# isabella232/handel

Hardware: AMD Instinct MI355X
Metric: BN254 aggregate-sig verifications/sec (batch 4096) (higher is better)
Workload: dtype u32 (26-bit-limb Fp, 64-bit accumulators)

## Files before the change

### handel_amd/_lib.py

```python

from __future__ import annotations

import ctypes
import os
import threading

from . import build as _build

_lock = threading.Lock()
_lib = None

HG_OK = 0
HG_ERR_SIG_INVALID = 1
HG_ERR_HASH_EOF = 2
HG_ERR_LEVEL = 3
HG_ERR_PK_UNMARSHAL = 4
HG_ERR_SIG_UNMARSHAL = 5
HG_ERR_EMPTY_AGG = 6
HG_ERR_CF_EXCEEDS = 7
HG_ERR_CF_MALFORMED = 8
HG_ERR_CF_SHORT = 9
HG_ERR_SIG_CF_EXCEEDS = 10
HG_ERR_SIG_CF_MALFORMED = 11
HG_ERR_SIG_CF_SHORT = 12
HG_ERR_MULTI_SIZES = 13
HG_ERR_PKT_ORIGIN = 20
HG_ERR_PKT_LEVEL = 21
HG_ERR_PKT_EOF = 22
HG_ERR_PKT_UNEXPECTED_EOF = 23
HG_ERR_PKT_BITSET_SHORT = 24
HG_ERR_PKT_TYPE_MISMATCH = 25
HG_ERR_PKT_BITSET_SIZE = 26
HG_ERR_PKT_NO_SIG = 27
HG_ERR_PKT_ID_RANGE = 28
HG_PKT_NO_IND = 29
HG_PKT_HAS_IND = 1
HG_STORE_HAS_BEST = 1
HG_STORE_BEST_SIG = 2
HG_STORE_SIG_BEST = 0xFFFFFFFF
HG_STORE_LEVEL_FULL = 0xFFFFFFFF
HG_MERGE_SKIPPED = 0
HG_MERGE_STORED = 1
HG_MERGE_DISCARDED = 2
HG_MERGE_ERR_MISSING = 3
HG_MERGE_ERR_INDIVIDUAL = 4
HG_MERGE_ERR_ROW = 5
HG_COMBINED_EMPTY = 1
HG_COMBINED_ERR_MISSING = 2
HG_ERR_ARG = 100
HG_ERR_DEVICE = 101

HG_FLAVOR_GO = 0
HG_FLAVOR_CF = 1

HG_PHASE_VERIFY = 0
HG_PHASE_AGGREGATE = 1
HG_PHASE_SUBMIT = 2

_P = ctypes.c_void_p
_SZ = ctypes.c_size_t
_I = ctypes.c_int
SIGNATURES = {
    "hg_version": (_I, []),
    "hg_context_simds": (_I, [_P]),
    "hg_context_flavor": (_I, [_P]),
    "hg_create": (_I, [_I, _I, ctypes.POINTER(_P)]),
    "hg_destroy": (None, [_P]),
    "hg_last_error": (ctypes.c_char_p, [_P]),
    "hg_code_string": (ctypes.c_char_p, [_I, _I]),
    "hg_processing_error_string": (ctypes.c_char_p, [_I, _I]),
    "hg_registry_load": (_I, [_P, _P, _SZ, _P]),
    "hg_registry_size": (_SZ, [_P]),
    "hg_prepare_aggregate": (_I, [_P]),
    "hg_aggregate_tables": (_I, [_P]),
    "hg_prepare_aggregate_msg": (_I, [_P, _P, _SZ]),
    "hg_set_aggregate_level": (_I, [_P, _I]),
    "hg_set_table_budget": (_I, [_P, _SZ]),
    "hg_set_fold_overlap": (_I, [_P, _I]),
    "hg_set_verify_split": (_I, [_P, _I]),
    "hg_registry_non_g2": (_SZ, [_P]),
    "hg_set_message": (_I, [_P, _P, _SZ]),
    "hg_verify_batch": (_I, [_P, _P, _P, _SZ, _P]),
    "hg_verify_batch_msg": (_I, [_P, _P, _SZ, _P, _P, _SZ, _P]),
    "hg_verify_batch_device": (_I, [_P, _P, _P, _SZ, _P, _P]),
    "hg_pack_verdicts_device": (_I, [_P, _P, _SZ, _P, _P]),
    "hg_verify_aggregate": (_I, [_P, _P, _SZ, _P, _SZ, _P, _P, _P]),
    "hg_verify_aggregate_device": (_I, [_P, _P, _SZ, _P, _P, _P, _P, _P]),
    "hg_verify_aggregate_device_bits": (_I, [_P, _P, _SZ, _P, _P, _P, _P, _P]),
    "hg_verify_aggregate_msg": (_I, [_P, _P, _SZ, _P, _SZ, _P, _SZ, _P, _P, _P]),
    "hg_verify_multisig": (_I, [_P, _P, _P, _SZ, _P, _SZ, _P, _P]),
    "hg_aggregate_pk": (_I, [_P, _P, _SZ, _P, _SZ, _P, _P]),
    "hg_combine_g1": (_I, [_P, _P, _P, _SZ, _P, _P]),
    "hg_combine_g2": (_I, [_P, _P, _P, _SZ, _P, _P]),
    "hg_pair": (_I, [_P, _P, _P, _SZ, _P, _P]),
    "hg_keygen": (_I, [_P, _P, _SZ, _P]),
    "hg_sign": (_I, [_P, _P, _SZ, _P]),
    "hg_sign_msg": (_I, [_P, _P, _SZ, _P, _SZ, _P]),
    "hg_debug_fp_mul": (_I, [_P, _P, _P, _SZ, _P]),
    "hg_diag_read": (_I, [_P, _P, _SZ]),
    "hg_sig_pairing_device": (_I, [_P, _P, _SZ, _P, _I, _P]),
    "hg_debug_fp12": (_I, [_P, _I, _P, _P, _SZ, _P]),
    "hg_timing_enable": (_I, [_P, _I]),
    "hg_timing_read": (_I, [_P, ctypes.POINTER(ctypes.c_double), ctypes.POINTER(_I)]),
    "hg_timing_read_phase": (_I, [_P, _I, ctypes.POINTER(ctypes.c_double), ctypes.POINTER(_I)]),
    "hg_sync": (_I, [_P]),
    "hg_context_bytes": (_SZ, [_P]),
    "hg_packet_stride_words": (_SZ, [_P]),
    "hg_parse_packets": (_I, [_P, _P, _SZ, _P, _SZ, _SZ, _P, _P, _P, _P]),
    "hg_parse_packets_device": (_I, [_P, _P, _SZ, _P, _SZ, _SZ, _P, _P, _P, _P, _P]),
    "hg_packet_error": (_I, [_P, _I, _P, ctypes.c_char_p, _SZ]),
    "hg_stores_create": (_I, [_P, _P, _SZ, _SZ, ctypes.POINTER(_P)]),
    "hg_stores_destroy": (None, [_P]),
    "hg_stores_update": (_I, [_P, _P, _SZ, _P, _SZ]),
    "hg_stores_read": (_I, [_P, ctypes.c_uint32, ctypes.c_uint32, _P, _P, ctypes.POINTER(_I)]),
    "hg_stores_evaluate_device": (_I, [_P, _P, _SZ, _SZ, _P, _P, _P, _P, _P]),
    "hg_stores_evaluate": (_I, [_P, _P, _SZ, _SZ, _P, _P, _P, _P]),
    "hg_stores_select_capacity": (_SZ, [_P, _SZ, ctypes.c_uint32]),
    "hg_stores_select_device": (_I, [_P, _P, _SZ, _P, ctypes.c_uint32, _P, _P, _P, _P, _P, _P, _P]),
    "hg_stores_enable_merge": (_I, [_P]),
    "hg_stores_update_sigs": (_I, [_P, _P, _SZ, _P, _SZ]),
    "hg_stores_read_best": (_I, [_P, ctypes.c_uint32, ctypes.c_uint32, _P, _P, ctypes.POINTER(_I)]),
    "hg_stores_merge_device": (_I, [_P, _P, _SZ, _P, _P, _SZ, _P, _SZ, _P, _P, _P, _P, _P, _P]),
    "hg_stores_combined_device": (_I, [_P, _P, _SZ, _SZ, _P, _P, _P, _P, _P]),
    "hg_stores_combined": (_I, [_P, _P, _SZ, _SZ, _P, _P, _P, _P]),
    "hg_batcher_create": (_I, [_P, _SZ, ctypes.c_uint, ctypes.POINTER(_P)]),
    "hg_batcher_destroy": (None, [_P]),
    "hg_batcher_submit": (_I, [_P, _P, _SZ, _P, _P, _P, ctypes.POINTER(_P)]),
    "hg_batcher_wait": (_I, [_P, _P, _P]),
    "hg_batcher_verify_aggregate": (_I, [_P, _P, _SZ, _P, _P, _P, _P]),
    "hg_batcher_stats": (_I, [_P, _P, _P]),
    "hg_prepare_aggregate_level": (_I, [_P, _I]),
    "hg_lane_create": (_I, [_P, _SZ, _SZ, _I, ctypes.POINTER(_P)]),
    "hg_lane_destroy": (None, [_P]),
    "hg_lane_stage": (_I, [_P, _SZ, _SZ, ctypes.POINTER(_P), ctypes.POINTER(_P), ctypes.POINTER(_P)]),
    "hg_lane_submit": (_I, [_P]),
    "hg_lane_query": (_I, [_P]),
    "hg_lane_wait": (_I, [_P]),
    "hg_lane_codes": (ctypes.POINTER(ctypes.c_int32), [_P]),
    "hg_lane_submit_device": (_I, [_P, _P, _SZ, _P, _P, _P, _P, _P]),
    "hg_lane_set_pairing_padding": (_I, [_P, _I]),
    "hg_lane_set_latency_form": (_I, [_P, _I]),
    "hg_lane_stream": (_P, [_P]),
    "hg_service_config_init": (None, [_P]),
    "hg_service_create": (_I, [_P, ctypes.c_char_p, _P, ctypes.POINTER(_P)]),
    "hg_service_create_echo": (_I, [ctypes.c_char_p, _P, ctypes.c_uint32, ctypes.c_uint32, ctypes.POINTER(_P)]),
    "hg_service_destroy": (None, [_P]),
    "hg_service_stats": (_I, [_P, _P, _P, _P]),
}


class HandelGPUError(RuntimeError):
    pass


def load(build_if_missing: bool = True):
    global _lib
    with _lock:
# ... 18 lines not shown
```

### handel_amd/csrc/bn256_gt.h

```cpp
#pragma once
#include "bn256_kernels.h"
#include "bn256_sigform.h"

namespace hg {

struct Gt {
  uint32_t w[120];
};
static constexpr int kGtChunk = 8;
static constexpr int kGtChunkTeams = 5;

struct GtReq {
  int m;
  int chunks;
  int comp;
  int k;
  int term_off;
  int chunk_off;
};
struct alignas(8) GtHdr {
  int terms, chunks;
  int big, mid;
  int nlong, nshort;
};
struct GtBlockIndex {
  int base[24];
};
struct GtWork {
  GtReq* plan;
  GtHdr* hdr;
  uint32_t* terms;
  int2* ord;
  int cap;
  Gt* partial;
  int* multi;
  int chunk_grid;
  int chunk;
  int win_bits;
};

void launch_gt_keys(const PointG2* reg, int n, const LineCoef* tab, const PointG1* h, Gt* out, hipStream_t s);
void launch_gt_windows8(const Gt* key, int nreg, Gt* w8, int nwin8, hipStream_t s);
void launch_gt_windows16(const Gt* w8, int nwin8, Gt* w16, int nwin16, hipStream_t s);
void launch_gt_blocks(const Gt* src, int stride, int nsrc, Gt* dst, int ndst, hipStream_t s);
void launch_gt_fold(const AggRequest* reqs, int n, const uint64_t* words, int32_t* codes, int nreg, int levels,
                    const Gt* win, const Gt* blk, const GtBlockIndex& bi, GtWork w, Gt* y, bool zero_hdr,
                    hipStream_t s);
void launch_verify_sig(const PointG1* sigs, int n, const LineCoef* tab, const Gt* y, int32_t* codes, hipStream_t s);
const SigEnv& sig_env();
bool launch_sig_form(SigForm f, const uint8_t* sigs, int flavor, int n, const LineCoef* tab, uint8_t* ws, Gt* fe,
                     hipStream_t s);
size_t fe12_ws_bytes(int n);
bool launch_fe12(Gt* fe, int n, uint8_t* ws, hipStream_t s);
void launch_gt_compare(const Gt* fe, const Gt* y, int n, int32_t* codes, hipStream_t s);
void launch_gt_compare_bits(const Gt* fe, const Gt* y, int n, int32_t* codes, uint8_t* bits, hipStream_t s);

}
```

### handel_amd/csrc/bn256_gt.hip

```cpp
#include <hip/hip_runtime.h>

#include <cstdlib>

#include "bn256_agg.h"
#include "bn256_decode.h"
#include "bn256_gt.h"
#include "bn256_pairing.h"
#include "bn256_sigfe.h"
#include "bn256_sigteam.h"

namespace hg {
static inline int nblk(int n, int b) { return (n + b - 1) / b; }

static constexpr int kFoldWords = kFoldTeamElems * 10;
static_assert(kFoldWords % 2 == 0, "8-byte aligned team regions");

HG_DEV void fold_regs_init(const Team& T) {
  if (T.tl == 0) {
    Fp z, o;
    fp_zero(z);
    fp_one(o);
    st_fp_a8(T.base + (kFoldRegBase + 0) * 10, z.l);
    st_fp_a8(T.base + (kFoldRegBase + 1) * 10, o.l);
  }
// ... 380 lines not shown
    gt_put(T, S_B, v, false);
    c += 4;
    if (c < g.chunks) gt_read(nx, partial + g.chunk_off + c, T);
    fold_mul(T, S);
  }
  for (int d = 1; d < (g.chunks > 2 ? 4 : 2); d <<= 1) {
    team_sync();
    lds_fp12_copy(T, slot(T, S_B), lds + (team ^ d) * kFoldWords + S_A * kFp12Words);
    fold_mul(T, S);
  }
  team_sync();
  if (team == 0) gt_store(T, S_A, y + r);
}

template <int TEAMS, bool kStore, bool kPad = (TEAMS == 4)>
__global__ __launch_bounds__(64) void k_verify_sig(const PointG1* sigs, const uint8_t* sig_bytes, int flavor, int n,
                                                   const LineCoef* tab, const Gt* y, Gt* fe, int32_t* codes) {
  __shared__ __attribute__((aligned(16))) uint32_t lds[TEAMS * kSigTeamWords];
  if (kStore) __builtin_amdgcn_s_setprio(3);
  if constexpr (kPad) asm volatile("" ::: "v255", "a0");
  Team T = make_team(lds, kSigTeamWords);
  uint32_t* F = T.base + kSigRegBase * 10;
  const int idx = blockIdx.x * TEAMS + (threadIdx.x >> 4);
  const bool valid = idx < n;
  const int ci = valid ? idx : n - 1;
  PointG1 sg;
  if (kStore) (void)decode_g1_one(sig_bytes + (size_t)ci * 64, flavor, sg);
  else sg = sigs[ci];
  XStream S = x_stream();
  team_miller_sig(T, F, sg.x, sg.y, sg.inf == 0, tab, S, SigFE<SigProgs16>::final_exp_hint_s());
  SigFE<SigProgs16>::team_final_exp_fc_s(T, S);
  if (kStore) {
    team_sync();
    if (valid) gt_store(T, S_F, fe + idx);
    return;
  }
  gt_load(T, S_A, y + ci);
  team_sync();
  const bool ok = t12_equal(T, S_F, S_A);
  if (valid && T.tl == 0 && codes[idx] == HG_OK) codes[idx] = ok ? HG_OK : HG_ERR_SIG_INVALID;
}

__global__ __launch_bounds__(64) void k_gt_compare(const Gt* fe, const Gt* y, int n, int32_t* codes) {
  const int r = blockIdx.x;
  if (r >= n) return;
  const int l = threadIdx.x;
  bool eq = true;
  if (l < 60) {
    const uint2 a = reinterpret_cast<const uint2*>(fe[r].w)[l];
    const uint2 b = reinterpret_cast<const uint2*>(y[r].w)[l];
    eq = a.x == b.x && a.y == b.y;
  }
  const bool all = __ballot(!eq) == 0;
  if (l == 0 && codes[r] == HG_OK) codes[r] = all ? HG_OK : HG_ERR_SIG_INVALID;
}

__global__ __launch_bounds__(64) void k_gt_compare_bits(const Gt* fe, const Gt* y, int n, int32_t* codes,
                                                        uint8_t* bits) {
  const int b = blockIdx.x;
  const int l = threadIdx.x;
  uint2 a[8], v[8];
#pragma unroll
  for (int j = 0; j < 8; j++) {
    const int r = min(8 * b + j, n - 1);
    a[j] = l < 60 ? reinterpret_cast<const uint2*>(fe[r].w)[l] : make_uint2(0, 0);
    v[j] = l < 60 ? reinterpret_cast<const uint2*>(y[r].w)[l] : make_uint2(0, 0);
  }
  bool mine = false;
#pragma unroll
  for (int j = 0; j < 8; j++) {
    const bool all = __ballot(a[j].x != v[j].x || a[j].y != v[j].y) == 0;
    const int r = 8 * b + j;
    if (l == j && r < n) {
      int32_t c = codes[r];
      if (c == HG_OK) c = all ? HG_OK : HG_ERR_SIG_INVALID;
      codes[r] = c;
      mine = c == HG_OK;
    }
  }
  const uint64_t m = __ballot(mine);
  if (l == 0) bits[b] = (uint8_t)(m & 0xffu);
}

void launch_gt_keys(const PointG2* reg, int n, const LineCoef* tab, const PointG1* h, Gt* out, hipStream_t s) {
  if (n > 0) k_gt_keys<4><<<nblk(n, 4), 64, 0, s>>>(reg, n, tab, h, out);
}
void launch_gt_windows8(const Gt* key, int nreg, Gt* w8, int nwin8, hipStream_t s) {
  if (nwin8 <= 0) return;
  k_gt_nib<<<nblk(2 * nwin8, 4), 64, 0, s>>>(key, nreg, nwin8, w8);
  k_gt_cross<<<nblk(15 * nwin8, 4), 64, 0, s>>>(nwin8, w8);
}
void launch_gt_windows16(const Gt* w8, int nwin8, Gt* w16, int nwin16, hipStream_t s) {
  if (nwin16 <= 0) return;
  k_gt_win16<<<nblk(256 * nwin16, kTeams12), 64, 0, s>>>(w8, nwin8, nwin16, w16);
}
void launch_gt_blocks(const Gt* src, int stride, int nsrc, Gt* dst, int ndst, hipStream_t s) {
  if (ndst > 0) k_gt_blocks<<<nblk(ndst, 4), 64, 0, s>>>(src, stride, nsrc, dst, ndst);
}
void launch_gt_fold(const AggRequest* reqs, int n, const uint64_t* words, int32_t* codes, int nreg, int levels,
                    const Gt* win, const Gt* blk, const GtBlockIndex& bi, GtWork w, Gt* y, bool zero_hdr, hipStream_t s) {
  if (n <= 0) return;
  if (zero_hdr) (void)hipMemsetAsync(w.hdr, 0, sizeof(GtHdr), s);
  if (w.win_bits == 16)
    k_gt_plan<16><<<nblk(n, kPlanWaves), 64 * kPlanWaves, 0, s>>>(reqs, n, words, codes, nreg, levels, bi, w.plan,
                                                                  w.hdr, w.terms, w.ord, w.cap, w.chunk, w.multi);
  else
    k_gt_plan<8><<<nblk(n, kPlanWaves), 64 * kPlanWaves, 0, s>>>(reqs, n, words, codes, nreg, levels, bi, w.plan,
                                                                 w.hdr, w.terms, w.ord, w.cap, w.chunk, w.multi);
  k_gt_chunks<<<w.chunk_grid, 64, 0, s>>>(win, blk, w.terms, w.ord, w.cap, w.plan, w.hdr, w.chunk, w.partial, y);
  k_gt_combine<<<n, 64, 0, s>>>(n, w.hdr, w.multi, w.plan, w.partial, y);
}
void launch_verify_sig(const PointG1* sigs, int n, const LineCoef* tab, const Gt* y, int32_t* codes, hipStream_t s) {
  if (n > 0) k_verify_sig<4, false><<<nblk(n, 4), 64, 0, s>>>(sigs, nullptr, 0, n, tab, y, nullptr, codes);
}
const SigEnv& sig_env() {
  static const SigEnv env = [] {
    auto on = [](const char* name, bool def) {
      const char* e = getenv(name);
      return e ? atoi(e) != 0 : def;
    };
    SigEnv v;
    if (getenv("HG_SIG12")) v.sig12 = on("HG_SIG12", false) ? 1 : 0;
    v.sig12_split = on("HG_SIG12_SPLIT", true);
    v.w2 = on("HG_SIG_W2", true);
    if (const char* e = getenv("HG_SIG_W2_LANE_MAX")) v.w2_lane_max = atoi(e);
    if (const char* e = getenv("HG_VERIFY_SPLIT")) v.verify_split = atoi(e) == 1;
    return v;
  }();
  return env;
}
bool launch_sig12(bool pad, bool split, const uint8_t* sigs, int flavor, int n, const LineCoef* tab, uint8_t* ws,
                  Gt* fe, hipStream_t s);
void launch_sig_w2(const uint8_t* sigs, int flavor, int n, const LineCoef* tab, Gt* fe, hipStream_t s);
bool launch_sig_form(SigForm f, const uint8_t* sigs, int flavor, int n, const LineCoef* tab, uint8_t* ws, Gt* fe,
                     hipStream_t s) {
  switch (f) {
    case SigForm::W16Pad:
      if (n > 0) k_verify_sig<4, true><<<nblk(n, 4), 64, 0, s>>>(nullptr, sigs, flavor, n, tab, nullptr, fe, nullptr);
      return true;
    case SigForm::W16:
      if (n > 0)
        k_verify_sig<4, true, false><<<nblk(n, 4), 64, 0, s>>>(nullptr, sigs, flavor, n, tab, nullptr, fe, nullptr);
      return true;
    case SigForm::T12Pad:
    case SigForm::T12:
      return launch_sig12(f == SigForm::T12Pad, sig_form_split(sig_env(), f), sigs, flavor, n, tab, ws, fe, s);
    case SigForm::W2:
      launch_sig_w2(sigs, flavor, n, tab, fe, s);
      return true;
  }
  return false;
}
void launch_gt_compare(const Gt* fe, const Gt* y, int n, int32_t* codes, hipStream_t s) {
  if (n > 0) k_gt_compare<<<n, 64, 0, s>>>(fe, y, n, codes);
}
void launch_gt_compare_bits(const Gt* fe, const Gt* y, int n, int32_t* codes, uint8_t* bits, hipStream_t s) {
  if (n > 0) k_gt_compare_bits<<<(n + 7) / 8, 64, 0, s>>>(fe, y, n, codes, bits);
}

}
```

### handel_amd/csrc/bn256_xtab.h

```cpp
#pragma once
#include <stdint.h>
namespace hg {
#define HG_P2N 0x0422599cu, 0x04ac6c5du, 0x05678616u, 0x05120b5au, 0x07b96e22u, 0x0584dc20u, 0x07fb2e17u, 0x047f9aa5u, 0x078d2a8du, 0x008fb500u
enum XProg { XP_PDBL, XP_PADD_POS, XP_PADD_NEG, XP_PADD_F1, XP_PADD_F2, XP_MDBL_1, XP_MDBL_2, XP_PDBL_1, XP_PADD_POS_1, XP_MADD_POS_2, XP_PADD_POS_3, XP_PADD_NEG_1, XP_MADD_NEG_2, XP_PADD_NEG_3, XP_PADD_F1_1, XP_MADD_F1_2, XP_PADD_F1_3, XP_PADD_F2_1, XP_MADD_F2_2, XP_PADD_F2_3, XP_SQR12, XP_LINE_PK, XP_LINE_FIX, XP_CYC_SQR, XP_MUL12, XP_CYC_SQR_X, XP_FEVAL, XP_SDBL, XP_LFEV, XP_MUL12F, XP_SQR12_12, XP_LINE_FIX_12, XP_MUL12_12, XP_CYC_SQR_X_12, XP_LINE_FIX_S, XP_MUL12_S, XP_CYC_SQR_X_S, XP_FEVAL_S, XP_SDBL_S, XP_LFEV_S, XP_SQR12_12_T, XP_LINE_FIX_12_T, XP_MUL12_12_T, XP_CYC_SQR_X_12_T, XP_MDBL_1_V, XP_MDBL_2_V, XP_PDBL_1_V, XP_PADD_POS_1_V, XP_MADD_POS_2_V, XP_PADD_POS_3_V, XP_PADD_NEG_1_V, XP_MADD_NEG_2_V, XP_PADD_NEG_3_V, XP_PADD_F1_1_V, XP_MADD_F1_2_V, XP_PADD_F1_3_V, XP_PADD_F2_1_V, XP_MADD_F2_2_V, XP_PADD_F2_3_V, XP_LINE_PK_V };
__constant__ static const uint32_t kXTab[28288] = {
  0x240616d0u, 0x19509000u, 0x90002906u, 0x28ee1bd0u, 0x16d09000u, 0x16f805c8u, 0x172006b8u, 0x16801748u, 0x24fe1680u, 0x00000f00u, 0x2a1216f8u, 0x19789000u,
  0x900028fau, 0x29fa1bf8u, 0x16d09000u, 0x177006b8u, 0x16800690u, 0x16801680u, 0x2a021680u, 0x00000ff0u, 0x2a031720u, 0x19a02b03u, 0x25032403u, 0x9000ffffu,
  0x17989000u, 0x17c00618u, 0x17e80708u, 0x16801810u, 0x28fe1680u, 0x00000fa0u, 0x2aff1748u, 0x19c82b01u, 0x250124ffu, 0x9000ffffu, 0x17989000u, 0x18380708u,
  0x168006e0u, 0x16801680u, 0x2e021680u, 0x00001090u, 0x25061770u, 0x19f09000u, 0x2b092a09u, 0x9000ffffu, 0x18609000u, 0x18880668u, 0x18b00758u, 0x168018d8u,
  0x2cfe1680u, 0x00001040u, 0x26061798u, 0x1a189000u, 0x90002afau, 0x9000ffffu, 0x19009000u, 0x19280758u, 0x19500730u, 0x19780758u, 0x26020730u, 0x00000f50u,
  0x2c1217c0u, 0x1a409000u, 0x900024fau, 0x9000ffffu, 0x19a09000u, 0x19f019c8u, 0x1a181748u, 0x168006b8u, 0x25fe1680u, 0x00000f28u, 0x2c0317e8u, 0x1a682d03u,
  0x27032603u, 0x9000ffffu, 0x17709000u, 0x1a4006b8u, 0x16800690u, 0x16801680u, 0x2b021680u, 0x00001018u, 0x2cff1810u, 0x1a902d01u, 0x270126ffu, 0x9000ffffu,
  0x1a689000u, 0x1ab81a90u, 0x1ae01810u, 0x16800708u, 0x29fe1680u, 0x00000fc8u, 0x27061838u, 0x1ab89000u, 0x2d092c09u, 0x9000ffffu, 0x18389000u, 0x1b080708u,
  0x168006e0u, 0x16801680u, 0x2f021680u, 0x000010b8u, 0x28061860u, 0x1ae09000u, 0x90002cfau, 0x9000ffffu, 0x1b309000u, 0x1b801b58u, 0x1ba818d8u, 0x16800758u,
  0x2dfe1680u, 0x00001068u, 0x2e121888u, 0x1b089000u, 0x900026fau, 0x9000ffffu, 0x19289000u, 0x1bd00758u, 0x19780730u, 0x1bf80758u, 0x27020730u, 0x00000f78u,
  0x2e0318b0u, 0x1b302f03u, 0x29032803u, 0x9000ffffu, 0x16809000u, 0x16801680u, 0x16801680u, 0x16801680u, 0x90001680u, 0x0000ffffu, 0x2eff18d8u, 0x1b582f01u,
  0x290128ffu, 0x9000ffffu, 0x16809000u, 0x16801680u, 0x16801680u, 0x16801680u, 0x90001680u, 0x0000ffffu, 0x28121900u, 0x1b809000u, 0x2f092e09u, 0x9000ffffu,
  0x16809000u, 0x16801680u, 0x16801680u, 0x16801680u, 0x90001680u, 0x0000ffffu, 0x29121928u, 0x1ba89000u, 0x90002efau, 0x9000ffffu, 0x16809000u, 0x16801680u,
  0x16801680u, 0x16801680u, 0x90001680u, 0x0000ffffu, 0x0c0616d0u, 0x19509000u, 0x0f010effu, 0x020816d0u, 0x02f816f8u, 0x17481720u, 0x01e00cfeu, 0x121216f8u,
  0x19789000u, 0x900014fau, 0x17981770u, 0x02f817c0u, 0x174817e8u, 0x02080dfeu, 0x12031720u, 0x19a01303u, 0x15091409u, 0x03981810u, 0x03701838u, 0x16801680u,
  0x02300e02u, 0x12ff1748u, 0x19c81301u, 0x90000d06u, 0x03981838u, 0x18601810u, 0x16801680u, 0x02580f02u, 0x0c031770u, 0x19f00d03u, 0x90000cfau, 0x02581888u,
  0x034818b0u, 0x190018d8u, 0x028010feu, 0x0cff1798u, 0x1a180d01u, 0x90001006u, 0x19501928u, 0x03481978u, 0x190019a0u, 0x02a811feu, 0x12fa17c0u, 0x1a409000u,
  0x90001612u, 0x02f816d0u, 0x02d019c8u, 0x16801680u, 0x02d01202u, 0x120917e8u, 0x1a681309u, 0x17031603u, 0x02f819c8u, 0x02d019f0u, 0x16801680u, 0x02f81302u,
  0x10121810u, 0x1a901106u, 0x170116ffu, 0x02a81a18u, 0x03981a40u, 0x1a901a68u, 0x032014feu, 0x10fa1838u, 0x1ab81112u, 0x11031003u, 0x1ae01ab8u, 0x03981b08u,
  0x1a901b30u, 0x034815feu, 0x16ff1860u, 0x1ae09000u, 0x110110ffu, 0x03481888u, 0x03201b58u, 0x16801680u, 0x03701602u, 0x0e061888u, 0x1b089000u, 0x900016fau,
  0x03481b58u, 0x03201b80u, 0x16801680u, 0x03981702u, 0x141218b0u, 0x1b309000u, 0x17091609u, 0x16801680u, 0x16801680u, 0x16801680u, 0xffff9000u, 0x140318d8u,
  0x1b581503u, 0x90000f06u, 0x16801680u, 0x16801680u, 0x16801680u, 0xffff9000u, 0x14ff1900u, 0x1b801501u, 0x90000efau, 0x16801680u, 0x16801680u, 0x16801680u,
  0xffff9000u, 0x0e031928u, 0xffff0f03u, 0x90009000u, 0x16801680u, 0x16801680u, 0x16801680u, 0xffff9000u, 0x0c0616d0u, 0x19509000u, 0x0f010effu, 0x020816d0u,
  0x02f816f8u, 0x17481720u, 0x03c00cfeu, 0x121216f8u, 0x19789000u, 0x900014fau, 0x17981770u, 0x02f817c0u, 0x174817e8u, 0x03e80dfeu, 0x12031720u, 0x19a01303u,
  0x15091409u, 0x03981810u, 0x03701838u, 0x16801680u, 0x04100e02u, 0x12ff1748u, 0x19c81301u, 0x90000d06u, 0x03981838u, 0x18601810u, 0x16801680u, 0x04380f02u,
  0x0c031770u, 0x19f00d03u, 0x90000cfau, 0x02581888u, 0x034818b0u, 0x190018d8u, 0x046010feu, 0x0cff1798u, 0x1a180d01u, 0x90001006u, 0x19501928u, 0x03481978u,
  0x190019a0u, 0x048811feu, 0x12fa17c0u, 0x1a409000u, 0x90001612u, 0x02f816d0u, 0x02d019c8u, 0x16801680u, 0x04b01202u, 0x120917e8u, 0x1a681309u, 0x17031603u,
  0x02f819c8u, 0x02d019f0u, 0x16801680u, 0x04d81302u, 0x10121810u, 0x1a901106u, 0x170116ffu, 0x02a81a18u, 0x03981a40u, 0x1a901a68u, 0x050014feu, 0x10fa1838u,
  0x1ab81112u, 0x11031003u, 0x1ae01ab8u, 0x03981b08u, 0x1a901b30u, 0x052815feu, 0x16ff1860u, 0x1ae09000u, 0x110110ffu, 0x03481888u, 0x03201b58u, 0x16801680u,
  0x05501602u, 0x0e061888u, 0x1b089000u, 0x900016fau, 0x03481b58u, 0x03201b80u, 0x16801680u, 0x05781702u, 0x141218b0u, 0x1b309000u, 0x17091609u, 0x16801680u,
  0x16801680u, 0x16801680u, 0xffff9000u, 0x140318d8u, 0x1b581503u, 0x90000f06u, 0x16801680u, 0x16801680u, 0x16801680u, 0xffff9000u, 0x14ff1900u, 0x1b801501u,
  0x90000efau, 0x16801680u, 0x16801680u, 0x16801680u, 0xffff9000u, 0x0e031928u, 0xffff0f03u, 0x90009000u, 0x16801680u, 0x16801680u, 0x16801680u, 0xffff9000u,
  0x0c0616d0u, 0x19509000u, 0x0f010effu, 0x020816d0u, 0x02f816f8u, 0x17481720u, 0x00000cfeu, 0x121216f8u, 0x19789000u, 0x900014fau, 0x17981770u, 0x02f817c0u,
  0x174817e8u, 0x00280dfeu, 0x12031720u, 0x19a01303u, 0x15091409u, 0x03981810u, 0x03701838u, 0x16801680u, 0x00500e02u, 0x12ff1748u, 0x19c81301u, 0x90000d06u,
  0x03981838u, 0x18601810u, 0x16801680u, 0x00780f02u, 0x0c031770u, 0x19f00d03u, 0x90000cfau, 0x02581888u, 0x034818b0u, 0x190018d8u, 0x00a010feu, 0x0cff1798u,
  0x1a180d01u, 0x90001006u, 0x19501928u, 0x03481978u, 0x190019a0u, 0x00c811feu, 0x12fa17c0u, 0x1a409000u, 0x90001612u, 0x02f816d0u, 0x02d019c8u, 0x16801680u,
  0x00f01202u, 0x120917e8u, 0x1a681309u, 0x17031603u, 0x02f819c8u, 0x02d019f0u, 0x16801680u, 0x01181302u, 0x10121810u, 0x1a901106u, 0x170116ffu, 0x02a81a18u,
  0x03981a40u, 0x1a901a68u, 0x014014feu, 0x10fa1838u, 0x1ab81112u, 0x11031003u, 0x1ae01ab8u, 0x03981b08u, 0x1a901b30u, 0x016815feu, 0x16ff1860u, 0x1ae09000u,
  0x110110ffu, 0x03481888u, 0x03201b58u, 0x16801680u, 0x01901602u, 0x0e061888u, 0x1b089000u, 0x900016fau, 0x03481b58u, 0x03201b80u, 0x16801680u, 0x01b81702u,
  0x141218b0u, 0x1b309000u, 0x17091609u, 0x16801680u, 0x16801680u, 0x16801680u, 0xffff9000u, 0x140318d8u, 0x1b581503u, 0x90000f06u, 0x16801680u, 0x16801680u,
  0x16801680u, 0xffff9000u, 0x14ff1900u, 0x1b801501u, 0x90000efau, 0x16801680u, 0x16801680u, 0x16801680u, 0xffff9000u, 0x0e031928u, 0xffff0f03u, 0x90009000u,
  0x16801680u, 0x16801680u, 0x16801680u, 0xffff9000u, 0x000616d0u, 0x19509000u, 0x030102ffu, 0x002816d0u, 0x011816f8u, 0x17481720u, 0x000000feu, 0x061216f8u,
  0x19789000u, 0x900008fau, 0x17981770u, 0x011817c0u, 0x174817e8u, 0x002801feu, 0x06031720u, 0x19a00703u, 0x09090809u, 0x01b81810u, 0x01901838u, 0x16801680u,
  0x00500202u, 0x06ff1748u, 0x19c80701u, 0x90000106u, 0x01b81838u, 0x18601810u, 0x16801680u, 0x00780302u, 0x00031770u, 0x19f00103u, 0x900000fau, 0x00781888u,
  0x016818b0u, 0x190018d8u, 0x00a004feu, 0x00ff1798u, 0x1a180101u, 0x90000406u, 0x19501928u, 0x01681978u, 0x190019a0u, 0x00c805feu, 0x06fa17c0u, 0x1a409000u,
  0x90000a12u, 0x011816d0u, 0x00f019c8u, 0x16801680u, 0x00f00602u, 0x060917e8u, 0x1a680709u, 0x0b030a03u, 0x011819c8u, 0x00f019f0u, 0x16801680u, 0x01180702u,
  0x04121810u, 0x1a900506u, 0x0b010affu, 0x00c81a18u, 0x01b81a40u, 0x1a901a68u, 0x014008feu, 0x04fa1838u, 0x1ab80512u, 0x05030403u, 0x1ae01ab8u, 0x01b81b08u,
  0x1a901b30u, 0x016809feu, 0x0aff1860u, 0x1ae09000u, 0x050104ffu, 0x01681888u, 0x01401b58u, 0x16801680u, 0x01900a02u, 0x02061888u, 0x1b089000u, 0x90000afau,
  0x01681b58u, 0x01401b80u, 0x16801680u, 0x01b80b02u, 0x081218b0u, 0x1b309000u, 0x0b090a09u, 0x16801680u, 0x16801680u, 0x16801680u, 0xffff9000u, 0x080318d8u,
  0x1b580903u, 0x90000306u, 0x16801680u, 0x16801680u, 0x16801680u, 0xffff9000u, 0x08ff1900u, 0x1b800901u, 0x900002fau, 0x16801680u, 0x16801680u, 0x16801680u,
  0xffff9000u, 0x02031928u, 0xffff0303u, 0x90009000u, 0x16801680u, 0x16801680u, 0x16801680u, 0xffff9000u, 0x6c0616d0u, 0x19509000u, 0x6f016effu, 0x110816d0u,
  0x11f816f8u, 0x17481720u, 0x00006cfeu, 0x721216f8u, 0x19789000u, 0x900074fau, 0x17981770u, 0x11f817c0u, 0x174817e8u, 0x00286dfeu, 0x72031720u, 0x19a07303u,
  0x75097409u, 0x12981810u, 0x12701838u, 0x16801680u, 0x00506e02u, 0x72ff1748u, 0x19c87301u, 0x90006d06u, 0x12981838u, 0x18601810u, 0x16801680u, 0x00786f02u,
  0x6c031770u, 0x19f06d03u, 0x90006cfau, 0x11581888u, 0x124818b0u, 0x190018d8u, 0x00a070feu, 0x6cff1798u, 0x1a186d01u, 0x90007006u, 0x19501928u, 0x12481978u,
  0x190019a0u, 0x00c871feu, 0x72fa17c0u, 0x1a409000u, 0x90007612u, 0x11f816d0u, 0x11d019c8u, 0x16801680u, 0x00f07202u, 0x720917e8u, 0x1a687309u, 0x77037603u,
  0x11f819c8u, 0x11d019f0u, 0x16801680u, 0x01187302u, 0x70121810u, 0x1a907106u, 0x770176ffu, 0x11a81a18u, 0x12981a40u, 0x1a901a68u, 0x014074feu, 0x70fa1838u,
  0x1ab87112u, 0x71037003u, 0x1ae01ab8u, 0x12981b08u, 0x1a901b30u, 0x016875feu, 0x76ff1860u, 0x1ae09000u, 0x710170ffu, 0x12481888u, 0x12201b58u, 0x16801680u,
  0x01907602u, 0x6e061888u, 0x1b089000u, 0x900076fau, 0x12481b58u, 0x12201b80u, 0x16801680u, 0x01b87702u, 0x741218b0u, 0x1b309000u, 0x77097609u, 0x16801680u,
  0x16801680u, 0x16801680u, 0xffff9000u, 0x740318d8u, 0x1b587503u, 0x90006f06u, 0x16801680u, 0x16801680u, 0x16801680u, 0xffff9000u, 0x74ff1900u, 0x1b807501u,
  0x90006efau, 0x16801680u, 0x16801680u, 0x16801680u, 0xffff9000u, 0x6e031928u, 0xffff6f03u, 0x90009000u, 0x16801680u, 0x16801680u, 0x16801680u, 0xffff9000u,
  0x600616d0u, 0x19509000u, 0x630162ffu, 0x0f2816d0u, 0x101816f8u, 0x17481720u, 0x0f0060feu, 0x661216f8u, 0x19789000u, 0x900068fau, 0x17981770u, 0x101817c0u,
  0x174817e8u, 0x0f2861feu, 0x66031720u, 0x19a06703u, 0x69096809u, 0x10b81810u, 0x10901838u, 0x16801680u, 0x0f506202u, 0x66ff1748u, 0x19c86701u, 0x90006106u,
  0x10b81838u, 0x18601810u, 0x16801680u, 0x0f786302u, 0x60031770u, 0x19f06103u, 0x900060fau, 0x0f781888u, 0x106818b0u, 0x190018d8u, 0x0fa064feu, 0x60ff1798u,
  0x1a186101u, 0x90006406u, 0x19501928u, 0x10681978u, 0x190019a0u, 0x0fc865feu, 0x66fa17c0u, 0x1a409000u, 0x90006a12u, 0x101816d0u, 0x0ff019c8u, 0x16801680u,
  0x0ff06602u, 0x660917e8u, 0x1a686709u, 0x6b036a03u, 0x101819c8u, 0x0ff019f0u, 0x16801680u, 0x10186702u, 0x64121810u, 0x1a906506u, 0x6b016affu, 0x0fc81a18u,
  0x10b81a40u, 0x1a901a68u, 0x104068feu, 0x64fa1838u, 0x1ab86512u, 0x65036403u, 0x1ae01ab8u, 0x10b81b08u, 0x1a901b30u, 0x106869feu, 0x6aff1860u, 0x1ae09000u,
  0x650164ffu, 0x10681888u, 0x10401b58u, 0x16801680u, 0x10906a02u, 0x62061888u, 0x1b089000u, 0x90006afau, 0x10681b58u, 0x10401b80u, 0x16801680u, 0x10b86b02u,
  0x681218b0u, 0x1b309000u, 0x6b096a09u, 0x16801680u, 0x16801680u, 0x16801680u, 0xffff9000u, 0x680318d8u, 0x1b586903u, 0x90006306u, 0x16801680u, 0x16801680u,
  0x16801680u, 0xffff9000u, 0x68ff1900u, 0x1b806901u, 0x900062fau, 0x16801680u, 0x16801680u, 0x16801680u, 0xffff9000u, 0x62031928u, 0xffff6303u, 0x90009000u,
  0x16801680u, 0x16801680u, 0x16801680u, 0xffff9000u, 0x6c0616d0u, 0x19509000u, 0x6f016effu, 0x110816d0u, 0x11f816f8u, 0x17481720u, 0x0f006cfeu, 0x721216f8u,
  0x19789000u, 0x900074fau, 0x17981770u, 0x11f817c0u, 0x174817e8u, 0x0f286dfeu, 0x72031720u, 0x19a07303u, 0x75097409u, 0x12981810u, 0x12701838u, 0x16801680u,
  0x0f506e02u, 0x72ff1748u, 0x19c87301u, 0x90006d06u, 0x12981838u, 0x18601810u, 0x16801680u, 0x0f786f02u, 0x6c031770u, 0x19f06d03u, 0x90006cfau, 0x11581888u,
  0x124818b0u, 0x190018d8u, 0x0fa070feu, 0x6cff1798u, 0x1a186d01u, 0x90007006u, 0x19501928u, 0x12481978u, 0x190019a0u, 0x0fc871feu, 0x72fa17c0u, 0x1a409000u,
  0x90007612u, 0x11f816d0u, 0x11d019c8u, 0x16801680u, 0x0ff07202u, 0x720917e8u, 0x1a687309u, 0x77037603u, 0x11f819c8u, 0x11d019f0u, 0x16801680u, 0x10187302u,
  0x70121810u, 0x1a907106u, 0x770176ffu, 0x11a81a18u, 0x12981a40u, 0x1a901a68u, 0x104074feu, 0x70fa1838u, 0x1ab87112u, 0x71037003u, 0x1ae01ab8u, 0x12981b08u,
  0x1a901b30u, 0x106875feu, 0x76ff1860u, 0x1ae09000u, 0x710170ffu, 0x12481888u, 0x12201b58u, 0x16801680u, 0x10907602u, 0x6e061888u, 0x1b089000u, 0x900076fau,
  0x12481b58u, 0x12201b80u, 0x16801680u, 0x10b87702u, 0x741218b0u, 0x1b309000u, 0x77097609u, 0x16801680u, 0x16801680u, 0x16801680u, 0xffff9000u, 0x740318d8u,
  0x1b587503u, 0x90006f06u, 0x16801680u, 0x16801680u, 0x16801680u, 0xffff9000u, 0x74ff1900u, 0x1b807501u, 0x90006efau, 0x16801680u, 0x16801680u, 0x16801680u,
  0xffff9000u, 0x6e031928u, 0xffff6f03u, 0x90009000u, 0x16801680u, 0x16801680u, 0x16801680u, 0xffff9000u, 0x000616d0u, 0x19509000u, 0x030102ffu, 0x002816d0u,
  0x011816f8u, 0x17481720u, 0x10e000feu, 0x061216f8u, 0x19789000u, 0x900008fau, 0x17981770u, 0x011817c0u, 0x174817e8u, 0x110801feu, 0x06031720u, 0x19a00703u,
  0x09090809u, 0x01b81810u, 0x01901838u, 0x16801680u, 0x11300202u, 0x06ff1748u, 0x19c80701u, 0x90000106u, 0x01b81838u, 0x18601810u, 0x16801680u, 0x11580302u,
  0x00031770u, 0x19f00103u, 0x900000fau, 0x00781888u, 0x016818b0u, 0x190018d8u, 0x118004feu, 0x00ff1798u, 0x1a180101u, 0x90000406u, 0x19501928u, 0x01681978u,
  0x190019a0u, 0x11a805feu, 0x06fa17c0u, 0x1a409000u, 0x90000a12u, 0x011816d0u, 0x00f019c8u, 0x16801680u, 0x11d00602u, 0x060917e8u, 0x1a680709u, 0x0b030a03u,
// ... 2190 lines not shown
  0x11d01298u, 0x09b009b0u, 0x09b009b0u, 0x09b009b0u, 0x09b009b0u, 0x00000b40u, 0x720102a8u, 0x05287301u, 0x3e0071ffu, 0x11f81298u, 0x11d00488u, 0x09b009b0u,
  0x09b009b0u, 0x09b009b0u, 0x09b009b0u, 0x00000b68u, 0x72ff02d0u, 0xffff7301u, 0x3e003e00u, 0x0a281180u, 0x09b009b0u, 0x09b009b0u, 0x09b009b0u, 0x09b009b0u,
  0x09b009b0u, 0x00000f50u, 0x76fd02f8u, 0xffff77ffu, 0x3e003e00u, 0x0a2811a8u, 0x09b009b0u, 0x09b009b0u, 0x09b009b0u, 0x09b009b0u, 0x09b009b0u, 0x00000f78u,
  0x78020320u, 0xffff3e00u, 0x3e003e00u, 0x0a0004b0u, 0x09b009b0u, 0x09b009b0u, 0x09b009b0u, 0x09b009b0u, 0x09b009b0u, 0x00000f00u, 0x73ff0348u, 0xffff7903u,
  0x3e003e00u, 0x0a0004d8u, 0x09b009b0u, 0x09b009b0u, 0x09b009b0u, 0x09b009b0u, 0x09b009b0u, 0x00000f28u, 0x72ff0370u, 0xffff7803u, 0x3e003e00u, 0x0ca81130u,
  0x0c801158u, 0x0cf80500u, 0x0cd00528u, 0x09b009b0u, 0x09b009b0u, 0x00000eb0u, 0x7cfd0398u, 0xffff7dffu, 0x3e003e00u, 0x0ca81158u, 0x0c8004b0u, 0x0cf80528u,
  0x0cd01180u, 0x09b009b0u, 0x09b009b0u, 0x00000ed8u, 0x7c0103c0u, 0xffff7dfdu, 0x3e003e00u, 0x09b009b0u, 0x09b009b0u, 0x09b009b0u, 0x09b009b0u, 0x09b009b0u,
  0x09b009b0u, 0x0000ffffu, 0x7eff03e8u, 0xffff3e00u, 0x3e003e00u, 0x09b009b0u, 0x09b009b0u, 0x09b009b0u, 0x09b009b0u, 0x09b009b0u, 0x09b009b0u, 0x0000ffffu,
  0x7fff0410u, 0xffff3e00u, 0x3e003e00u, 0x09b009b0u, 0x09b009b0u, 0x09b009b0u, 0x09b009b0u, 0x09b009b0u, 0x09b009b0u, 0x0000ffffu, 0x7aff0438u, 0xffff3e00u,
  0x3e003e00u, 0x09b009b0u, 0x09b009b0u, 0x09b009b0u, 0x09b009b0u, 0x09b009b0u, 0x09b009b0u, 0x0000ffffu, 0x4cff01e0u, 0x01e03e00u, 0x02300208u, 0x46010258u,
  0x00001130u, 0x48ff0208u, 0x02304903u, 0x0be00208u, 0x47010258u, 0x00001158u, 0x4dff0230u, 0x02803e00u, 0x02a80208u, 0x44010258u, 0x00001180u, 0x48030258u,
  0x02a84901u, 0x0d200208u, 0x45010258u, 0x000011a8u, 0x54ff0280u, 0x0d703e00u, 0x09b00a50u, 0x3e0009b0u, 0x00000e10u, 0x55ff02a8u, 0x0d983e00u, 0x09b00a50u,
  0x3e0009b0u, 0x00000e38u, 0x3e00ffffu, 0x0dc03e00u, 0x09b00a78u, 0x3e0009b0u, 0x00000e60u, 0x3e00ffffu, 0x0de83e00u, 0x09b00a78u, 0x3e0009b0u, 0x00000e88u,
  0x3e00ffffu, 0x09b03e00u, 0x09b009b0u, 0x3e0009b0u, 0x0000ffffu, 0x3e00ffffu, 0x09b03e00u, 0x09b009b0u, 0x3e0009b0u, 0x0000ffffu, 0x3e00ffffu, 0x09b03e00u,
  0x09b009b0u, 0x3e0009b0u, 0x0000ffffu, 0x3e00ffffu, 0x09b03e00u, 0x09b009b0u, 0x3e0009b0u, 0x0000ffffu, 0x3e00ffffu, 0x09b03e00u, 0x09b009b0u, 0x3e0009b0u,
  0x0000ffffu, 0x3e00ffffu, 0x09b03e00u, 0x09b009b0u, 0x3e0009b0u, 0x0000ffffu, 0x3e00ffffu, 0x09b03e00u, 0x09b009b0u, 0x3e0009b0u, 0x0000ffffu, 0x3e00ffffu,
  0x09b03e00u, 0x09b009b0u, 0x3e0009b0u, 0x0000ffffu, 0x720201e0u, 0x04603e00u, 0x7d017c03u, 0x11f801e0u, 0x12480208u, 0x12200230u, 0x11f80258u, 0x11d00280u,
  0x09b009b0u, 0x00000aa0u, 0x76030208u, 0x04887701u, 0x3e0076ffu, 0x02d002a8u, 0x12480230u, 0x122002f8u, 0x11f80280u, 0x11d00320u, 0x09b009b0u, 0x00000ac8u,
  0x76ff0230u, 0x04b07703u, 0x3e006effu, 0x03481310u, 0x03701338u, 0x12480398u, 0x122003c0u, 0x11f803e8u, 0x11d00410u, 0x00000af0u, 0x78fe0258u, 0x04d83e00u,
  0x3e006fffu, 0x03481338u, 0x03700438u, 0x124803c0u, 0x12200460u, 0x11f80410u, 0x11d013b0u, 0x00000b18u, 0x79fe0280u, 0x05003e00u, 0x3e0070ffu, 0x11f81270u,
  0x11d01298u, 0x09b009b0u, 0x09b009b0u, 0x09b009b0u, 0x09b009b0u, 0x00000b40u, 0x720102a8u, 0x05287301u, 0x3e0071ffu, 0x11f81298u, 0x11d00488u, 0x09b009b0u,
  0x09b009b0u, 0x09b009b0u, 0x09b009b0u, 0x00000b68u, 0x72ff02d0u, 0xffff7301u, 0x3e003e00u, 0x0a281180u, 0x09b009b0u, 0x09b009b0u, 0x09b009b0u, 0x09b009b0u,
  0x09b009b0u, 0x00000f50u, 0x76fd02f8u, 0xffff77ffu, 0x3e003e00u, 0x0a2811a8u, 0x09b009b0u, 0x09b009b0u, 0x09b009b0u, 0x09b009b0u, 0x09b009b0u, 0x00000f78u,
  0x78020320u, 0xffff3e00u, 0x3e003e00u, 0x0a0004b0u, 0x09b009b0u, 0x09b009b0u, 0x09b009b0u, 0x09b009b0u, 0x09b009b0u, 0x00000f00u, 0x73ff0348u, 0xffff7903u,
  0x3e003e00u, 0x0a0004d8u, 0x09b009b0u, 0x09b009b0u, 0x09b009b0u, 0x09b009b0u, 0x09b009b0u, 0x00000f28u, 0x72ff0370u, 0xffff7803u, 0x3e003e00u, 0x0d481130u,
  0x0d201158u, 0x0c080500u, 0x0be00528u, 0x09b009b0u, 0x09b009b0u, 0x00000eb0u, 0x7cfd0398u, 0xffff7dffu, 0x3e003e00u, 0x0d481158u, 0x0d2004b0u, 0x0c080528u,
  0x0be01180u, 0x09b009b0u, 0x09b009b0u, 0x00000ed8u, 0x7c0103c0u, 0xffff7dfdu, 0x3e003e00u, 0x09b009b0u, 0x09b009b0u, 0x09b009b0u, 0x09b009b0u, 0x09b009b0u,
  0x09b009b0u, 0x0000ffffu, 0x7eff03e8u, 0xffff3e00u, 0x3e003e00u, 0x09b009b0u, 0x09b009b0u, 0x09b009b0u, 0x09b009b0u, 0x09b009b0u, 0x09b009b0u, 0x0000ffffu,
  0x7fff0410u, 0xffff3e00u, 0x3e003e00u, 0x09b009b0u, 0x09b009b0u, 0x09b009b0u, 0x09b009b0u, 0x09b009b0u, 0x09b009b0u, 0x0000ffffu, 0x7aff0438u, 0xffff3e00u,
  0x3e003e00u, 0x09b009b0u, 0x09b009b0u, 0x09b009b0u, 0x09b009b0u, 0x09b009b0u, 0x09b009b0u, 0x0000ffffu, 0x5aff01e0u, 0x00005b03u, 0x00280e88u, 0x01900e60u,
  0x01b801e0u, 0x06030208u, 0x00000701u, 0x11a802a8u, 0x09b009b0u, 0x000011d0u, 0x5a030208u, 0x00285b01u, 0x00000e88u, 0x01b80230u, 0x019001e0u, 0x07030258u,
  0x002806ffu, 0x02f802d0u, 0x09b009b0u, 0x000011f8u, 0x5cff0230u, 0x00503e00u, 0x00780e88u, 0x00000e60u, 0x00280e38u, 0x08030e10u, 0x00500901u, 0x11580320u,
  0x09b009b0u, 0x00001220u, 0x5afd0258u, 0x00785bffu, 0x00500e88u, 0x00280230u, 0x00000e38u, 0x09030280u, 0x007808ffu, 0x03700348u, 0x09b009b0u, 0x00001248u,
  0x5aff0280u, 0x00a03e00u, 0x00c80e88u, 0x00500e60u, 0x00780e38u, 0x0a030e10u, 0x00a00b01u, 0x11a80b40u, 0x11800b68u, 0x00001270u, 0x700202a8u, 0x00c83e00u,
  0x00a00e88u, 0x00780230u, 0x00500e38u, 0x0b030280u, 0x00c80affu, 0x11a80b68u, 0x11800398u, 0x00001298u, 0x700102d0u, 0x00f07101u, 0x01180e88u, 0x00a00e60u,
  0x00c80e38u, 0x00010e10u, 0x00f03e00u, 0x11a80aa0u, 0x11800ac8u, 0x000012c0u, 0x70ff02f8u, 0x01187101u, 0x00f00e88u, 0x00c80230u, 0x00a00e38u, 0x01010280u,
  0x01183e00u, 0x11a80ac8u, 0x118003c0u, 0x000012e8u, 0x6e020320u, 0x01403e00u, 0x01680e88u, 0x00f00e60u, 0x01180e38u, 0x02010e10u, 0x01403e00u, 0x11a81130u,
  0x11801158u, 0x00001310u, 0x6e010348u, 0x01686f01u, 0x01400e88u, 0x01180230u, 0x00f00e38u, 0x03010280u, 0x01683e00u, 0x11a81158u, 0x118003e8u, 0x00001338u,
  0x6eff0370u, 0x01906f01u, 0x01b80e88u, 0x01400e60u, 0x01680e38u, 0x04010e10u, 0x01903e00u, 0x11580b40u, 0x11300b68u, 0x00001360u, 0x48ff0398u, 0x01b83e00u,
  0x01900e88u, 0x01680230u, 0x01400e38u, 0x05010280u, 0x01b83e00u, 0x11580b68u, 0x11300398u, 0x00001388u, 0x44ff03c0u, 0x09b03e00u, 0x09b009b0u, 0x09b009b0u,
  0x09b009b0u, 0x3e0009b0u, 0xffff3e00u, 0x11a80af0u, 0x11800b18u, 0x000013b0u, 0x6eff03e8u, 0x09b03e00u, 0x09b009b0u, 0x09b009b0u, 0x09b009b0u, 0x3e0009b0u,
  0xffff3e00u, 0x11a80b18u, 0x11800410u, 0x000013d8u, 0x46ff0410u, 0x09b03e00u, 0x09b009b0u, 0x09b009b0u, 0x09b009b0u, 0x3e0009b0u, 0xffff3e00u, 0x09b009b0u,
  0x09b009b0u, 0x0000ffffu, 0x3e00ffffu, 0x09b03e00u, 0x09b009b0u, 0x09b009b0u, 0x09b009b0u, 0x3e0009b0u, 0xffff3e00u, 0x09b009b0u, 0x09b009b0u, 0x0000ffffu,
  0x5aff01e0u, 0x00005b03u, 0x00280e88u, 0x01900e60u, 0x01b801e0u, 0x06030208u, 0x00000701u, 0x11a802a8u, 0x09b009b0u, 0x000011d0u, 0x5a030208u, 0x00285b01u,
  0x00000e88u, 0x01b80230u, 0x019001e0u, 0x07030258u, 0x002806ffu, 0x02f802d0u, 0x09b009b0u, 0x000011f8u, 0x5cff0230u, 0x00503e00u, 0x00780e88u, 0x00000e60u,
  0x00280e38u, 0x08030e10u, 0x00500901u, 0x11580320u, 0x09b009b0u, 0x00001220u, 0x5afd0258u, 0x00785bffu, 0x00500e88u, 0x00280230u, 0x00000e38u, 0x09030280u,
  0x007808ffu, 0x03700348u, 0x09b009b0u, 0x00001248u, 0x5aff0280u, 0x00a03e00u, 0x00c80e88u, 0x00500e60u, 0x00780e38u, 0x0a030e10u, 0x00a00b01u, 0x11a80b40u,
  0x11800b68u, 0x00001270u, 0x700202a8u, 0x00c83e00u, 0x00a00e88u, 0x00780230u, 0x00500e38u, 0x0b030280u, 0x00c80affu, 0x11a80b68u, 0x11800398u, 0x00001298u,
  0x700102d0u, 0x00f07101u, 0x01180e88u, 0x00a00e60u, 0x00c80e38u, 0x00010e10u, 0x00f03e00u, 0x11a80aa0u, 0x11800ac8u, 0x000012c0u, 0x70ff02f8u, 0x01187101u,
  0x00f00e88u, 0x00c80230u, 0x00a00e38u, 0x01010280u, 0x01183e00u, 0x11a80ac8u, 0x118003c0u, 0x000012e8u, 0x6e020320u, 0x01403e00u, 0x01680e88u, 0x00f00e60u,
  0x01180e38u, 0x02010e10u, 0x01403e00u, 0x11a81130u, 0x11801158u, 0x00001310u, 0x6e010348u, 0x01686f01u, 0x01400e88u, 0x01180230u, 0x00f00e38u, 0x03010280u,
  0x01683e00u, 0x11a81158u, 0x118003e8u, 0x00001338u, 0x6eff0370u, 0x01906f01u, 0x01b80e88u, 0x01400e60u, 0x01680e38u, 0x04010e10u, 0x01903e00u, 0x11580b40u,
  0x11300b68u, 0x00001360u, 0x48ff0398u, 0x01b83e00u, 0x01900e88u, 0x01680230u, 0x01400e38u, 0x05010280u, 0x01b83e00u, 0x11580b68u, 0x11300398u, 0x00001388u,
  0x44ff03c0u, 0x09b03e00u, 0x09b009b0u, 0x09b009b0u, 0x09b009b0u, 0x3e0009b0u, 0xffff3e00u, 0x11a80af0u, 0x11800b18u, 0x000013b0u, 0x6eff03e8u, 0x09b03e00u,
  0x09b009b0u, 0x09b009b0u, 0x09b009b0u, 0x3e0009b0u, 0xffff3e00u, 0x11a80b18u, 0x11800410u, 0x000013d8u, 0x46ff0410u, 0x09b03e00u, 0x09b009b0u, 0x09b009b0u,
  0x09b009b0u, 0x3e0009b0u, 0xffff3e00u, 0x09b009b0u, 0x09b009b0u, 0x0000ffffu, 0x3e00ffffu, 0x09b03e00u, 0x09b009b0u, 0x09b009b0u, 0x09b009b0u, 0x3e0009b0u,
  0xffff3e00u, 0x09b009b0u, 0x09b009b0u, 0x0000ffffu, 0x5aff01e0u, 0x00005b03u, 0x00280e88u, 0x01900e60u, 0x01b801e0u, 0x06030208u, 0x00000701u, 0x11a802a8u,
  0x09b009b0u, 0x000011d0u, 0x5a030208u, 0x00285b01u, 0x00000e88u, 0x01b80230u, 0x019001e0u, 0x07030258u, 0x002806ffu, 0x02f802d0u, 0x09b009b0u, 0x000011f8u,
  0x5cff0230u, 0x00503e00u, 0x00780e88u, 0x00000e60u, 0x00280e38u, 0x08030e10u, 0x00500901u, 0x11580320u, 0x09b009b0u, 0x00001220u, 0x5afd0258u, 0x00785bffu,
  0x00500e88u, 0x00280230u, 0x00000e38u, 0x09030280u, 0x007808ffu, 0x03700348u, 0x09b009b0u, 0x00001248u, 0x5aff0280u, 0x00a03e00u, 0x00c80e88u, 0x00500e60u,
  0x00780e38u, 0x0a030e10u, 0x00a00b01u, 0x11a80b40u, 0x11800b68u, 0x00001270u, 0x700202a8u, 0x00c83e00u, 0x00a00e88u, 0x00780230u, 0x00500e38u, 0x0b030280u,
  0x00c80affu, 0x11a80b68u, 0x11800398u, 0x00001298u, 0x700102d0u, 0x00f07101u, 0x01180e88u, 0x00a00e60u, 0x00c80e38u, 0x00010e10u, 0x00f03e00u, 0x11a80aa0u,
  0x11800ac8u, 0x000012c0u, 0x70ff02f8u, 0x01187101u, 0x00f00e88u, 0x00c80230u, 0x00a00e38u, 0x01010280u, 0x01183e00u, 0x11a80ac8u, 0x118003c0u, 0x000012e8u,
  0x6e020320u, 0x01403e00u, 0x01680e88u, 0x00f00e60u, 0x01180e38u, 0x02010e10u, 0x01403e00u, 0x11a81130u, 0x11801158u, 0x00001310u, 0x6e010348u, 0x01686f01u,
  0x01400e88u, 0x01180230u, 0x00f00e38u, 0x03010280u, 0x01683e00u, 0x11a81158u, 0x118003e8u, 0x00001338u, 0x6eff0370u, 0x01906f01u, 0x01b80e88u, 0x01400e60u,
  0x01680e38u, 0x04010e10u, 0x01903e00u, 0x11580b40u, 0x11300b68u, 0x00001360u, 0x48ff0398u, 0x01b83e00u, 0x01900e88u, 0x01680230u, 0x01400e38u, 0x05010280u,
  0x01b83e00u, 0x11580b68u, 0x11300398u, 0x00001388u, 0x44ff03c0u, 0x09b03e00u, 0x09b009b0u, 0x09b009b0u, 0x09b009b0u, 0x3e0009b0u, 0xffff3e00u, 0x11a80af0u,
  0x11800b18u, 0x000013b0u, 0x6eff03e8u, 0x09b03e00u, 0x09b009b0u, 0x09b009b0u, 0x09b009b0u, 0x3e0009b0u, 0xffff3e00u, 0x11a80b18u, 0x11800410u, 0x000013d8u,
  0x46ff0410u, 0x09b03e00u, 0x09b009b0u, 0x09b009b0u, 0x09b009b0u, 0x3e0009b0u, 0xffff3e00u, 0x09b009b0u, 0x09b009b0u, 0x0000ffffu, 0x3e00ffffu, 0x09b03e00u,
  0x09b009b0u, 0x09b009b0u, 0x09b009b0u, 0x3e0009b0u, 0xffff3e00u, 0x09b009b0u, 0x09b009b0u, 0x0000ffffu, 0x5aff01e0u, 0x00005b03u, 0x00280e88u, 0x01900e60u,
  0x01b801e0u, 0x06030208u, 0x00000701u, 0x11a802a8u, 0x09b009b0u, 0x000011d0u, 0x5a030208u, 0x00285b01u, 0x00000e88u, 0x01b80230u, 0x019001e0u, 0x07030258u,
  0x002806ffu, 0x02f802d0u, 0x09b009b0u, 0x000011f8u, 0x5cff0230u, 0x00503e00u, 0x00780e88u, 0x00000e60u, 0x00280e38u, 0x08030e10u, 0x00500901u, 0x11580320u,
  0x09b009b0u, 0x00001220u, 0x5afd0258u, 0x00785bffu, 0x00500e88u, 0x00280230u, 0x00000e38u, 0x09030280u, 0x007808ffu, 0x03700348u, 0x09b009b0u, 0x00001248u,
  0x5aff0280u, 0x00a03e00u, 0x00c80e88u, 0x00500e60u, 0x00780e38u, 0x0a030e10u, 0x00a00b01u, 0x11a80b40u, 0x11800b68u, 0x00001270u, 0x700202a8u, 0x00c83e00u,
  0x00a00e88u, 0x00780230u, 0x00500e38u, 0x0b030280u, 0x00c80affu, 0x11a80b68u, 0x11800398u, 0x00001298u, 0x700102d0u, 0x00f07101u, 0x01180e88u, 0x00a00e60u,
  0x00c80e38u, 0x00010e10u, 0x00f03e00u, 0x11a80aa0u, 0x11800ac8u, 0x000012c0u, 0x70ff02f8u, 0x01187101u, 0x00f00e88u, 0x00c80230u, 0x00a00e38u, 0x01010280u,
  0x01183e00u, 0x11a80ac8u, 0x118003c0u, 0x000012e8u, 0x6e020320u, 0x01403e00u, 0x01680e88u, 0x00f00e60u, 0x01180e38u, 0x02010e10u, 0x01403e00u, 0x11a81130u,
  0x11801158u, 0x00001310u, 0x6e010348u, 0x01686f01u, 0x01400e88u, 0x01180230u, 0x00f00e38u, 0x03010280u, 0x01683e00u, 0x11a81158u, 0x118003e8u, 0x00001338u,
  0x6eff0370u, 0x01906f01u, 0x01b80e88u, 0x01400e60u, 0x01680e38u, 0x04010e10u, 0x01903e00u, 0x11580b40u, 0x11300b68u, 0x00001360u, 0x48ff0398u, 0x01b83e00u,
  0x01900e88u, 0x01680230u, 0x01400e38u, 0x05010280u, 0x01b83e00u, 0x11580b68u, 0x11300398u, 0x00001388u, 0x44ff03c0u, 0x09b03e00u, 0x09b009b0u, 0x09b009b0u,
  0x09b009b0u, 0x3e0009b0u, 0xffff3e00u, 0x11a80af0u, 0x11800b18u, 0x000013b0u, 0x6eff03e8u, 0x09b03e00u, 0x09b009b0u, 0x09b009b0u, 0x09b009b0u, 0x3e0009b0u,
  0xffff3e00u, 0x11a80b18u, 0x11800410u, 0x000013d8u, 0x46ff0410u, 0x09b03e00u, 0x09b009b0u, 0x09b009b0u, 0x09b009b0u, 0x3e0009b0u, 0xffff3e00u, 0x09b009b0u,
  0x09b009b0u, 0x0000ffffu, 0x3e00ffffu, 0x09b03e00u, 0x09b009b0u, 0x09b009b0u, 0x09b009b0u, 0x3e0009b0u, 0xffff3e00u, 0x09b009b0u, 0x09b009b0u, 0x0000ffffu,
  0x00000000u, 0x00000000u, 0x00000000u, 0x00000000u, 0x00000000u, 0x00000000u, 0x00000000u, 0x00000000u, 0x00000000u, 0x00000000u, 0x00000000u, 0x00000000u,
  0x00000000u, 0x00000000u, 0x00000000u, 0x00000000u,
};
static constexpr int kXFetchWords = 16;
static constexpr int kFoldRegBase = 36;
static constexpr int kFoldTeamElems = 60;
static constexpr int kSigRegBase = 84;
static constexpr int kSigTeamElems = 118;
static constexpr int kSigTRegBase = 60;
static constexpr int kSigTTeamElems = 92;
static constexpr int kVRegBase = 62;
static constexpr int kVTeamElems = 128;
template <int PROG, int D = -1, int A = -1, int B = -1> struct XInst;
template <> struct XInst<XP_CYC_SQR, S_I, S_C> { static constexpr int kOff = 0, kW = 10; HG_DEV static void run(const Team& T, XStream& S, XHint h) { x_round<3, 2, 4, 1, 10, 0, 0, -1, -1, -1, 1, 0, 0, 0, 1>(T, S, 0, h); } };
template <> struct XInst<XP_CYC_SQR_X, S_A, S_A> { static constexpr int kOff = 160, kW = 7; HG_DEV static void run(const Team& T, XStream& S, XHint h) { x_round<2, 2, 3, 1, 7, 0, 0, 6, 2, 0, 0, 0, 1, 0, 1>(T, S, 160, h); } };
template <> struct XInst<XP_CYC_SQR_X, S_B, S_A> { static constexpr int kOff = 272, kW = 7; HG_DEV static void run(const Team& T, XStream& S, XHint h) { x_round<2, 2, 3, 1, 7, 0, 0, 6, 2, 0, 0, 0, 1, 0, 1>(T, S, 272, h); } };
template <> struct XInst<XP_CYC_SQR_X, S_F, S_A> { static constexpr int kOff = 384, kW = 7; HG_DEV static void run(const Team& T, XStream& S, XHint h) { x_round<2, 2, 3, 1, 7, 0, 0, 6, 2, 0, 0, 0, 1, 0, 1>(T, S, 384, h); } };
template <> struct XInst<XP_CYC_SQR_X, S_F, S_F> { static constexpr int kOff = 496, kW = 7; HG_DEV static void run(const Team& T, XStream& S, XHint h) { x_round<2, 2, 3, 1, 7, 0, 0, 6, 2, 0, 0, 0, 1, 0, 1>(T, S, 496, h); } };
template <> struct XInst<XP_CYC_SQR_X, S_F, S_J> { static constexpr int kOff = 608, kW = 7; HG_DEV static void run(const Team& T, XStream& S, XHint h) { x_round<2, 2, 3, 1, 7, 0, 0, 6, 2, 0, 0, 0, 1, 0, 1>(T, S, 608, h); } };
template <> struct XInst<XP_CYC_SQR_X, S_I, S_I> { static constexpr int kOff = 720, kW = 7; HG_DEV static void run(const Team& T, XStream& S, XHint h) { x_round<2, 2, 3, 1, 7, 0, 0, 6, 2, 0, 0, 0, 1, 0, 1>(T, S, 720, h); } };
template <> struct XInst<XP_CYC_SQR_X, S_I, S_J> { static constexpr int kOff = 832, kW = 7; HG_DEV static void run(const Team& T, XStream& S, XHint h) { x_round<2, 2, 3, 1, 7, 0, 0, 6, 2, 0, 0, 0, 1, 0, 1>(T, S, 832, h); } };
template <> struct XInst<XP_CYC_SQR_X, S_J, S_F> { static constexpr int kOff = 944, kW = 7; HG_DEV static void run(const Team& T, XStream& S, XHint h) { x_round<2, 2, 3, 1, 7, 0, 0, 6, 2, 0, 0, 0, 1, 0, 1>(T, S, 944, h); } };
template <> struct XInst<XP_CYC_SQR_X, S_J, S_I> { static constexpr int kOff = 1056, kW = 7; HG_DEV static void run(const Team& T, XStream& S, XHint h) { x_round<2, 2, 3, 1, 7, 0, 0, 6, 2, 0, 0, 0, 1, 0, 1>(T, S, 1056, h); } };
template <> struct XInst<XP_CYC_SQR_X, S_J, S_J> { static constexpr int kOff = 1168, kW = 7; HG_DEV static void run(const Team& T, XStream& S, XHint h) { x_round<2, 2, 3, 1, 7, 0, 0, 6, 2, 0, 0, 0, 1, 0, 1>(T, S, 1168, h); } };
template <> struct XInst<XP_CYC_SQR_X, S_K, S_I> { static constexpr int kOff = 1280, kW = 7; HG_DEV static void run(const Team& T, XStream& S, XHint h) { x_round<2, 2, 3, 1, 7, 0, 0, 6, 2, 0, 0, 0, 1, 0, 1>(T, S, 1280, h); } };
template <> struct XInst<XP_CYC_SQR_X, S_K, S_K> { static constexpr int kOff = 1392, kW = 7; HG_DEV static void run(const Team& T, XStream& S, XHint h) { x_round<2, 2, 3, 1, 7, 0, 0, 6, 2, 0, 0, 0, 1, 0, 1>(T, S, 1392, h); } };
template <> struct XInst<XP_LINE_FIX, S_F, S_F> { static constexpr int kOff = 1504, kW = 7; HG_DEV static void run(const Team& T, XStream& S, XHint h) { x_round<1, 2, 4, 2, 7, 0, 0, 4, 1, 0, 1, 0, 0, 1, 1>(T, S, 1504, h); } };
template <> struct XInst<XP_LINE_PK, S_A, S_A> { static constexpr int kOff = 1616, kW = 8; HG_DEV static void run(const Team& T, XStream& S, XHint h) { x_round<1, 2, 6, 0, 8, 0, 0, 4, 0, 0, 1, 0, 0, 1, 0>(T, S, 1616, h); } };
template <> struct XInst<XP_LINE_PK, S_F, S_F> { static constexpr int kOff = 1744, kW = 8; HG_DEV static void run(const Team& T, XStream& S, XHint h) { x_round<1, 2, 6, 0, 8, 0, 0, 4, 0, 0, 1, 0, 0, 1, 0>(T, S, 1744, h); } };
template <> struct XInst<XP_MADD_F1_2, S_F, S_F> { static constexpr int kOff = 1872, kW = 10; HG_DEV static void run(const Team& T, XStream& S, XHint h) { x_round<1, 2, 4, 2, 10, 2, 0, 4, 1, 0, 1, 0, 0, 0, 0>(T, S, 1872, h); } };
template <> struct XInst<XP_MADD_F2_2, S_F, S_F> { static constexpr int kOff = 2032, kW = 10; HG_DEV static void run(const Team& T, XStream& S, XHint h) { x_round<1, 2, 4, 2, 10, 2, 0, 4, 1, 0, 1, 0, 0, 0, 0>(T, S, 2032, h); } };
template <> struct XInst<XP_MADD_NEG_2, S_F, S_F> { static constexpr int kOff = 2192, kW = 10; HG_DEV static void run(const Team& T, XStream& S, XHint h) { x_round<1, 2, 4, 2, 10, 2, 0, 4, 1, 0, 1, 0, 0, 0, 0>(T, S, 2192, h); } };
template <> struct XInst<XP_MADD_POS_2, S_F, S_F> { static constexpr int kOff = 2352, kW = 10; HG_DEV static void run(const Team& T, XStream& S, XHint h) { x_round<1, 2, 4, 2, 10, 2, 0, 4, 1, 0, 1, 0, 0, 0, 0>(T, S, 2352, h); } };
template <> struct XInst<XP_MDBL_1, S_F, S_F> { static constexpr int kOff = 2512, kW = 16; HG_DEV static void run(const Team& T, XStream& S, XHint h) { x_round<4, 2, 7, 0, 16, 2, 0, -1, -1, -1, 1, 0, 0, 0, 0>(T, S, 2512, h); } };
template <> struct XInst<XP_MDBL_2, S_F, S_F> { static constexpr int kOff = 2768, kW = 14; HG_DEV static void run(const Team& T, XStream& S, XHint h) { x_round<2, 4, 4, 2, 14, 2, 2, -1, -1, -1, 1, 0, 0, 0, 0>(T, S, 2768, h); } };
template <> struct XInst<XP_MUL12, S_A, S_A, S_B> { static constexpr int kOff = 2992, kW = 16; HG_DEV static void run(const Team& T, XStream& S, XHint h) { x_round<2, 2, 12, 0, 16, 0, 0, 4, 0, 0, 1, 0, 0, 1, 1>(T, S, 2992, h); } };
template <> struct XInst<XP_MUL12, S_A, S_C, S_E> { static constexpr int kOff = 3248, kW = 16; HG_DEV static void run(const Team& T, XStream& S, XHint h) { x_round<2, 2, 12, 0, 16, 0, 0, 4, 0, 0, 1, 0, 0, 1, 1>(T, S, 3248, h); } };
template <> struct XInst<XP_MUL12, S_A, S_F, S_A> { static constexpr int kOff = 3504, kW = 16; HG_DEV static void run(const Team& T, XStream& S, XHint h) { x_round<2, 2, 12, 0, 16, 0, 0, 4, 0, 0, 1, 0, 0, 1, 1>(T, S, 3504, h); } };
template <> struct XInst<XP_MUL12, S_A, S_G, S_A> { static constexpr int kOff = 3760, kW = 16; HG_DEV static void run(const Team& T, XStream& S, XHint h) { x_round<2, 2, 12, 0, 16, 0, 0, 4, 0, 0, 1, 0, 0, 1, 1>(T, S, 3760, h); } };
template <> struct XInst<XP_MUL12, S_A, S_K, S_L> { static constexpr int kOff = 4016, kW = 16; HG_DEV static void run(const Team& T, XStream& S, XHint h) { x_round<2, 2, 12, 0, 16, 0, 0, 4, 0, 0, 1, 0, 0, 1, 1>(T, S, 4016, h); } };
template <> struct XInst<XP_MUL12, S_B, S_A, S_B> { static constexpr int kOff = 4272, kW = 16; HG_DEV static void run(const Team& T, XStream& S, XHint h) { x_round<2, 2, 12, 0, 16, 0, 0, 4, 0, 0, 1, 0, 0, 1, 1>(T, S, 4272, h); } };
template <> struct XInst<XP_MUL12, S_B, S_C, S_D> { static constexpr int kOff = 4528, kW = 16; HG_DEV static void run(const Team& T, XStream& S, XHint h) { x_round<2, 2, 12, 0, 16, 0, 0, 4, 0, 0, 1, 0, 0, 1, 1>(T, S, 4528, h); } };
template <> struct XInst<XP_MUL12, S_D, S_A, S_E> { static constexpr int kOff = 4784, kW = 16; HG_DEV static void run(const Team& T, XStream& S, XHint h) { x_round<2, 2, 12, 0, 16, 0, 0, 4, 0, 0, 1, 0, 0, 1, 1>(T, S, 4784, h); } };
template <> struct XInst<XP_MUL12, S_E, S_B, S_J> { static constexpr int kOff = 5040, kW = 16; HG_DEV static void run(const Team& T, XStream& S, XHint h) { x_round<2, 2, 12, 0, 16, 0, 0, 4, 0, 0, 1, 0, 0, 1, 1>(T, S, 5040, h); } };
template <> struct XInst<XP_MUL12, S_F, S_A, S_B> { static constexpr int kOff = 5296, kW = 16; HG_DEV static void run(const Team& T, XStream& S, XHint h) { x_round<2, 2, 12, 0, 16, 0, 0, 4, 0, 0, 1, 0, 0, 1, 1>(T, S, 5296, h); } };
template <> struct XInst<XP_MUL12, S_F, S_B, S_A> { static constexpr int kOff = 5552, kW = 16; HG_DEV static void run(const Team& T, XStream& S, XHint h) { x_round<2, 2, 12, 0, 16, 0, 0, 4, 0, 0, 1, 0, 0, 1, 1>(T, S, 5552, h); } };
template <> struct XInst<XP_MUL12, S_F, S_F, S_A> { static constexpr int kOff = 5808, kW = 16; HG_DEV static void run(const Team& T, XStream& S, XHint h) { x_round<2, 2, 12, 0, 16, 0, 0, 4, 0, 0, 1, 0, 0, 1, 1>(T, S, 5808, h); } };
template <> struct XInst<XP_MUL12, S_F, S_F, S_J> { static constexpr int kOff = 6064, kW = 16; HG_DEV static void run(const Team& T, XStream& S, XHint h) { x_round<2, 2, 12, 0, 16, 0, 0, 4, 0, 0, 1, 0, 0, 1, 1>(T, S, 6064, h); } };
template <> struct XInst<XP_MUL12, S_F, S_F, S_K> { static constexpr int kOff = 6320, kW = 16; HG_DEV static void run(const Team& T, XStream& S, XHint h) { x_round<2, 2, 12, 0, 16, 0, 0, 4, 0, 0, 1, 0, 0, 1, 1>(T, S, 6320, h); } };
template <> struct XInst<XP_MUL12, S_F, S_G, S_A> { static constexpr int kOff = 6576, kW = 16; HG_DEV static void run(const Team& T, XStream& S, XHint h) { x_round<2, 2, 12, 0, 16, 0, 0, 4, 0, 0, 1, 0, 0, 1, 1>(T, S, 6576, h); } };
template <> struct XInst<XP_MUL12, S_F, S_K, S_J> { static constexpr int kOff = 6832, kW = 16; HG_DEV static void run(const Team& T, XStream& S, XHint h) { x_round<2, 2, 12, 0, 16, 0, 0, 4, 0, 0, 1, 0, 0, 1, 1>(T, S, 6832, h); } };
template <> struct XInst<XP_MUL12, S_F, S_K, S_L> { static constexpr int kOff = 7088, kW = 16; HG_DEV static void run(const Team& T, XStream& S, XHint h) { x_round<2, 2, 12, 0, 16, 0, 0, 4, 0, 0, 1, 0, 0, 1, 1>(T, S, 7088, h); } };
template <> struct XInst<XP_MUL12, S_G, S_G, S_D> { static constexpr int kOff = 7344, kW = 16; HG_DEV static void run(const Team& T, XStream& S, XHint h) { x_round<2, 2, 12, 0, 16, 0, 0, 4, 0, 0, 1, 0, 0, 1, 1>(T, S, 7344, h); } };
template <> struct XInst<XP_MUL12, S_H, S_C, S_H> { static constexpr int kOff = 7600, kW = 16; HG_DEV static void run(const Team& T, XStream& S, XHint h) { x_round<2, 2, 12, 0, 16, 0, 0, 4, 0, 0, 1, 0, 0, 1, 1>(T, S, 7600, h); } };
template <> struct XInst<XP_MUL12, S_I, S_E, S_I> { static constexpr int kOff = 7856, kW = 16; HG_DEV static void run(const Team& T, XStream& S, XHint h) { x_round<2, 2, 12, 0, 16, 0, 0, 4, 0, 0, 1, 0, 0, 1, 1>(T, S, 7856, h); } };
template <> struct XInst<XP_MUL12, S_I, S_I, S_J> { static constexpr int kOff = 8112, kW = 16; HG_DEV static void run(const Team& T, XStream& S, XHint h) { x_round<2, 2, 12, 0, 16, 0, 0, 4, 0, 0, 1, 0, 0, 1, 1>(T, S, 8112, h); } };
template <> struct XInst<XP_MUL12, S_I, S_I, S_K> { static constexpr int kOff = 8368, kW = 16; HG_DEV static void run(const Team& T, XStream& S, XHint h) { x_round<2, 2, 12, 0, 16, 0, 0, 4, 0, 0, 1, 0, 0, 1, 1>(T, S, 8368, h); } };
template <> struct XInst<XP_MUL12, S_J, S_G, S_D> { static constexpr int kOff = 8624, kW = 16; HG_DEV static void run(const Team& T, XStream& S, XHint h) { x_round<2, 2, 12, 0, 16, 0, 0, 4, 0, 0, 1, 0, 0, 1, 1>(T, S, 8624, h); } };
template <> struct XInst<XP_MUL12, S_J, S_J, S_A> { static constexpr int kOff = 8880, kW = 16; HG_DEV static void run(const Team& T, XStream& S, XHint h) { x_round<2, 2, 12, 0, 16, 0, 0, 4, 0, 0, 1, 0, 0, 1, 1>(T, S, 8880, h); } };
template <> struct XInst<XP_MUL12, S_J, S_J, S_F> { static constexpr int kOff = 9136, kW = 16; HG_DEV static void run(const Team& T, XStream& S, XHint h) { x_round<2, 2, 12, 0, 16, 0, 0, 4, 0, 0, 1, 0, 0, 1, 1>(T, S, 9136, h); } };
template <> struct XInst<XP_MUL12, S_J, S_J, S_I> { static constexpr int kOff = 9392, kW = 16; HG_DEV static void run(const Team& T, XStream& S, XHint h) { x_round<2, 2, 12, 0, 16, 0, 0, 4, 0, 0, 1, 0, 0, 1, 1>(T, S, 9392, h); } };
template <> struct XInst<XP_MUL12, S_J, S_J, S_K> { static constexpr int kOff = 9648, kW = 16; HG_DEV static void run(const Team& T, XStream& S, XHint h) { x_round<2, 2, 12, 0, 16, 0, 0, 4, 0, 0, 1, 0, 0, 1, 1>(T, S, 9648, h); } };
template <> struct XInst<XP_MUL12, S_K, S_J, S_L> { static constexpr int kOff = 9904, kW = 16; HG_DEV static void run(const Team& T, XStream& S, XHint h) { x_round<2, 2, 12, 0, 16, 0, 0, 4, 0, 0, 1, 0, 0, 1, 1>(T, S, 9904, h); } };
template <> struct XInst<XP_MUL12, S_K, S_K, S_C> { static constexpr int kOff = 10160, kW = 16; HG_DEV static void run(const Team& T, XStream& S, XHint h) { x_round<2, 2, 12, 0, 16, 0, 0, 4, 0, 0, 1, 0, 0, 1, 1>(T, S, 10160, h); } };
template <> struct XInst<XP_MUL12, S_K, S_K, S_D> { static constexpr int kOff = 10416, kW = 16; HG_DEV static void run(const Team& T, XStream& S, XHint h) { x_round<2, 2, 12, 0, 16, 0, 0, 4, 0, 0, 1, 0, 0, 1, 1>(T, S, 10416, h); } };
template <> struct XInst<XP_MUL12, S_K, S_K, S_H> { static constexpr int kOff = 10672, kW = 16; HG_DEV static void run(const Team& T, XStream& S, XHint h) { x_round<2, 2, 12, 0, 16, 0, 0, 4, 0, 0, 1, 0, 0, 1, 1>(T, S, 10672, h); } };
template <> struct XInst<XP_MUL12, S_L, S_A, S_K> { static constexpr int kOff = 10928, kW = 16; HG_DEV static void run(const Team& T, XStream& S, XHint h) { x_round<2, 2, 12, 0, 16, 0, 0, 4, 0, 0, 1, 0, 0, 1, 1>(T, S, 10928, h); } };
template <> struct XInst<XP_MUL12, S_L, S_F, S_K> { static constexpr int kOff = 11184, kW = 16; HG_DEV static void run(const Team& T, XStream& S, XHint h) { x_round<2, 2, 12, 0, 16, 0, 0, 4, 0, 0, 1, 0, 0, 1, 1>(T, S, 11184, h); } };
template <> struct XInst<XP_MUL12F, S_A, S_A, S_B> { static constexpr int kOff = 11440, kW = 16; HG_DEV static void run(const Team& T, XStream& S, XHint h) { x_round<2, 2, 12, 0, 16, 0, 0, 4, 0, 0, 1, 0, 0, 1, 0>(T, S, 11440, h); } };
template <> struct XInst<XP_PADD_F1> { static constexpr int kOff = 11696, kW = 5; HG_DEV static void run(const Team& T, XStream& S, XHint h) { x_round<1, 2, 2, 1, 5, 0, 0, 1, 0, 0, 0, 0, 0, 0, 0>(T, S, 11696, XHint{11776, 4}); x_round<1, 2, 2, 0, 4, 0, 0, 1, 0, 0, 0, 0, 0, 0, 0>(T, S, 11776, XHint{11840, 10}); x_round<2, 2, 6, 0, 10, 0, 0, 4, 0, 0, 1, 0, 0, 0, 0>(T, S, 11840, h); } };
template <> struct XInst<XP_PADD_F1_1> { static constexpr int kOff = 12000, kW = 5; HG_DEV static void run(const Team& T, XStream& S, XHint h) { x_round<1, 2, 2, 1, 5, 0, 0, 1, 0, 0, 0, 0, 0, 0, 0>(T, S, 12000, h); } };
template <> struct XInst<XP_PADD_F1_3> { static constexpr int kOff = 12080, kW = 10; HG_DEV static void run(const Team& T, XStream& S, XHint h) { x_round<2, 2, 6, 0, 10, 0, 0, 4, 0, 0, 1, 0, 0, 0, 0>(T, S, 12080, h); } };
template <> struct XInst<XP_PADD_F2> { static constexpr int kOff = 12240, kW = 5; HG_DEV static void run(const Team& T, XStream& S, XHint h) { x_round<1, 2, 2, 1, 5, 0, 0, 1, 0, 0, 0, 0, 0, 0, 0>(T, S, 12240, XHint{12320, 4}); x_round<1, 2, 2, 0, 4, 0, 0, 1, 0, 0, 0, 0, 0, 0, 0>(T, S, 12320, XHint{12384, 10}); x_round<2, 2, 6, 0, 10, 0, 0, 4, 0, 0, 1, 0, 0, 0, 0>(T, S, 12384, h); } };
template <> struct XInst<XP_PADD_F2_1> { static constexpr int kOff = 12544, kW = 5; HG_DEV static void run(const Team& T, XStream& S, XHint h) { x_round<1, 2, 2, 1, 5, 0, 0, 1, 0, 0, 0, 0, 0, 0, 0>(T, S, 12544, h); } };
template <> struct XInst<XP_PADD_F2_3> { static constexpr int kOff = 12624, kW = 10; HG_DEV static void run(const Team& T, XStream& S, XHint h) { x_round<2, 2, 6, 0, 10, 0, 0, 4, 0, 0, 1, 0, 0, 0, 0>(T, S, 12624, h); } };
template <> struct XInst<XP_PADD_NEG> { static constexpr int kOff = 12784, kW = 5; HG_DEV static void run(const Team& T, XStream& S, XHint h) { x_round<1, 2, 2, 1, 5, 0, 0, 1, 0, 0, 0, 0, 0, 0, 0>(T, S, 12784, XHint{12864, 4}); x_round<1, 2, 2, 0, 4, 0, 0, 1, 0, 0, 0, 0, 0, 0, 0>(T, S, 12864, XHint{12928, 10}); x_round<2, 2, 6, 0, 10, 0, 0, 4, 0, 0, 1, 0, 0, 0, 0>(T, S, 12928, h); } };
template <> struct XInst<XP_PADD_NEG_1> { static constexpr int kOff = 13088, kW = 5; HG_DEV static void run(const Team& T, XStream& S, XHint h) { x_round<1, 2, 2, 1, 5, 0, 0, 1, 0, 0, 0, 0, 0, 0, 0>(T, S, 13088, h); } };
template <> struct XInst<XP_PADD_NEG_3> { static constexpr int kOff = 13168, kW = 10; HG_DEV static void run(const Team& T, XStream& S, XHint h) { x_round<2, 2, 6, 0, 10, 0, 0, 4, 0, 0, 1, 0, 0, 0, 0>(T, S, 13168, h); } };
template <> struct XInst<XP_PADD_POS> { static constexpr int kOff = 13328, kW = 5; HG_DEV static void run(const Team& T, XStream& S, XHint h) { x_round<1, 2, 2, 1, 5, 0, 0, 1, 0, 0, 0, 0, 0, 0, 0>(T, S, 13328, XHint{13408, 4}); x_round<1, 2, 2, 0, 4, 0, 0, 1, 0, 0, 0, 0, 0, 0, 0>(T, S, 13408, XHint{13472, 10}); x_round<2, 2, 6, 0, 10, 0, 0, 4, 0, 0, 1, 0, 0, 0, 0>(T, S, 13472, h); } };
template <> struct XInst<XP_PADD_POS_1> { static constexpr int kOff = 13632, kW = 5; HG_DEV static void run(const Team& T, XStream& S, XHint h) { x_round<1, 2, 2, 1, 5, 0, 0, 1, 0, 0, 0, 0, 0, 0, 0>(T, S, 13632, h); } };
template <> struct XInst<XP_PADD_POS_3> { static constexpr int kOff = 13712, kW = 10; HG_DEV static void run(const Team& T, XStream& S, XHint h) { x_round<2, 2, 6, 0, 10, 0, 0, 4, 0, 0, 1, 0, 0, 0, 0>(T, S, 13712, h); } };
template <> struct XInst<XP_PDBL> { static constexpr int kOff = 13872, kW = 4; HG_DEV static void run(const Team& T, XStream& S, XHint h) { x_round<1, 2, 2, 0, 4, 0, 0, -1, -1, -1, 0, 0, 0, 0, 0>(T, S, 13872, XHint{13936, 9}); x_round<2, 4, 2, 2, 9, 0, 0, -1, -1, -1, 0, 0, 0, 0, 0>(T, S, 13936, h); } };
template <> struct XInst<XP_PDBL_1> { static constexpr int kOff = 14080, kW = 4; HG_DEV static void run(const Team& T, XStream& S, XHint h) { x_round<1, 2, 2, 0, 4, 0, 0, -1, -1, -1, 0, 0, 0, 0, 0>(T, S, 14080, h); } };
template <> struct XInst<XP_SQR12, S_A, S_A> { static constexpr int kOff = 14144, kW = 12; HG_DEV static void run(const Team& T, XStream& S, XHint h) { x_round<3, 2, 7, 0, 12, 0, 0, 8, 0, 0, 1, 0, 0, 0, 0>(T, S, 14144, h); } };
template <> struct XInst<XP_SQR12, S_F, S_A> { static constexpr int kOff = 14336, kW = 12; HG_DEV static void run(const Team& T, XStream& S, XHint h) { x_round<3, 2, 7, 0, 12, 0, 0, 8, 0, 0, 1, 0, 0, 0, 0>(T, S, 14336, h); } };
template <> struct XInst<XP_SQR12, S_F, S_F> { static constexpr int kOff = 14528, kW = 12; HG_DEV static void run(const Team& T, XStream& S, XHint h) { x_round<3, 2, 7, 0, 12, 0, 0, 8, 0, 0, 1, 0, 0, 0, 0>(T, S, 14528, h); } };
template <> struct XInst<XP_CYC_SQR_X_S, S_A, S_A> { static constexpr int kOff = 14720, kW = 7; HG_DEV static void run(const Team& T, XStream& S, XHint h) { x_round<2, 2, 3, 1, 7, 0, 0, 6, 2, 0, 0, 0, 1, 0, 1>(T, S, 14720, h); } };
template <> struct XInst<XP_CYC_SQR_X_S, S_B, S_A> { static constexpr int kOff = 14832, kW = 7; HG_DEV static void run(const Team& T, XStream& S, XHint h) { x_round<2, 2, 3, 1, 7, 0, 0, 6, 2, 0, 0, 0, 1, 0, 1>(T, S, 14832, h); } };
template <> struct XInst<XP_CYC_SQR_X_S, S_D, S_D> { static constexpr int kOff = 14944, kW = 7; HG_DEV static void run(const Team& T, XStream& S, XHint h) { x_round<2, 2, 3, 1, 7, 0, 0, 6, 2, 0, 0, 0, 1, 0, 1>(T, S, 14944, h); } };
template <> struct XInst<XP_CYC_SQR_X_S, S_D, S_E> { static constexpr int kOff = 15056, kW = 7; HG_DEV static void run(const Team& T, XStream& S, XHint h) { x_round<2, 2, 3, 1, 7, 0, 0, 6, 2, 0, 0, 0, 1, 0, 1>(T, S, 15056, h); } };
template <> struct XInst<XP_CYC_SQR_X_S, S_E, S_D> { static constexpr int kOff = 15168, kW = 7; HG_DEV static void run(const Team& T, XStream& S, XHint h) { x_round<2, 2, 3, 1, 7, 0, 0, 6, 2, 0, 0, 0, 1, 0, 1>(T, S, 15168, h); } };
template <> struct XInst<XP_CYC_SQR_X_S, S_E, S_E> { static constexpr int kOff = 15280, kW = 7; HG_DEV static void run(const Team& T, XStream& S, XHint h) { x_round<2, 2, 3, 1, 7, 0, 0, 6, 2, 0, 0, 0, 1, 0, 1>(T, S, 15280, h); } };
template <> struct XInst<XP_FEVAL_S> { static constexpr int kOff = 15392, kW = 2; HG_DEV static void run(const Team& T, XStream& S, XHint h) { x_round<0, 0, 1, 0, 2, 0, 0, 0, 0, 0, 0, 0, 0, 1, 1>(T, S, 15392, h); } };
template <> struct XInst<XP_LFEV_S, S_F, S_F> { static constexpr int kOff = 15424, kW = 7; HG_DEV static void run(const Team& T, XStream& S, XHint h) { x_round<1, 2, 4, 2, 7, 0, 0, 4, 1, 0, 1, 0, 0, 1, 1>(T, S, 15424, h); } };
template <> struct XInst<XP_LINE_FIX_S, S_F, S_F> { static constexpr int kOff = 15536, kW = 7; HG_DEV static void run(const Team& T, XStream& S, XHint h) { x_round<1, 2, 4, 2, 7, 0, 0, 4, 1, 0, 1, 0, 0, 1, 1>(T, S, 15536, h); } };
template <> struct XInst<XP_MUL12_S, S_A, S_C, S_G> { static constexpr int kOff = 15648, kW = 16; HG_DEV static void run(const Team& T, XStream& S, XHint h) { x_round<2, 2, 12, 0, 16, 0, 0, 4, 0, 0, 1, 0, 0, 1, 1>(T, S, 15648, h); } };
template <> struct XInst<XP_MUL12_S, S_A, S_D, S_A> { static constexpr int kOff = 15904, kW = 16; HG_DEV static void run(const Team& T, XStream& S, XHint h) { x_round<2, 2, 12, 0, 16, 0, 0, 4, 0, 0, 1, 0, 0, 1, 1>(T, S, 15904, h); } };
template <> struct XInst<XP_MUL12_S, S_A, S_D, S_E> { static constexpr int kOff = 16160, kW = 16; HG_DEV static void run(const Team& T, XStream& S, XHint h) { x_round<2, 2, 12, 0, 16, 0, 0, 4, 0, 0, 1, 0, 0, 1, 1>(T, S, 16160, h); } };
template <> struct XInst<XP_MUL12_S, S_A, S_F, S_A> { static constexpr int kOff = 16416, kW = 16; HG_DEV static void run(const Team& T, XStream& S, XHint h) { x_round<2, 2, 12, 0, 16, 0, 0, 4, 0, 0, 1, 0, 0, 1, 1>(T, S, 16416, h); } };
template <> struct XInst<XP_MUL12_S, S_B, S_A, S_B> { static constexpr int kOff = 16672, kW = 16; HG_DEV static void run(const Team& T, XStream& S, XHint h) { x_round<2, 2, 12, 0, 16, 0, 0, 4, 0, 0, 1, 0, 0, 1, 1>(T, S, 16672, h); } };
template <> struct XInst<XP_MUL12_S, S_B, S_A, S_G> { static constexpr int kOff = 16928, kW = 16; HG_DEV static void run(const Team& T, XStream& S, XHint h) { x_round<2, 2, 12, 0, 16, 0, 0, 4, 0, 0, 1, 0, 0, 1, 1>(T, S, 16928, h); } };
template <> struct XInst<XP_MUL12_S, S_B, S_C, S_G> { static constexpr int kOff = 17184, kW = 16; HG_DEV static void run(const Team& T, XStream& S, XHint h) { x_round<2, 2, 12, 0, 16, 0, 0, 4, 0, 0, 1, 0, 0, 1, 1>(T, S, 17184, h); } };
template <> struct XInst<XP_MUL12_S, S_D, S_C, S_C> { static constexpr int kOff = 17440, kW = 16; HG_DEV static void run(const Team& T, XStream& S, XHint h) { x_round<2, 2, 12, 0, 16, 0, 0, 4, 0, 0, 1, 0, 0, 1, 1>(T, S, 17440, h); } };
template <> struct XInst<XP_MUL12_S, S_D, S_D, S_B> { static constexpr int kOff = 17696, kW = 16; HG_DEV static void run(const Team& T, XStream& S, XHint h) { x_round<2, 2, 12, 0, 16, 0, 0, 4, 0, 0, 1, 0, 0, 1, 1>(T, S, 17696, h); } };
template <> struct XInst<XP_MUL12_S, S_D, S_D, S_E> { static constexpr int kOff = 17952, kW = 16; HG_DEV static void run(const Team& T, XStream& S, XHint h) { x_round<2, 2, 12, 0, 16, 0, 0, 4, 0, 0, 1, 0, 0, 1, 1>(T, S, 17952, h); } };
template <> struct XInst<XP_MUL12_S, S_D, S_D, S_G> { static constexpr int kOff = 18208, kW = 16; HG_DEV static void run(const Team& T, XStream& S, XHint h) { x_round<2, 2, 12, 0, 16, 0, 0, 4, 0, 0, 1, 0, 0, 1, 1>(T, S, 18208, h); } };
template <> struct XInst<XP_MUL12_S, S_E, S_E, S_D> { static constexpr int kOff = 18464, kW = 16; HG_DEV static void run(const Team& T, XStream& S, XHint h) { x_round<2, 2, 12, 0, 16, 0, 0, 4, 0, 0, 1, 0, 0, 1, 1>(T, S, 18464, h); } };
template <> struct XInst<XP_MUL12_S, S_E, S_E, S_G> { static constexpr int kOff = 18720, kW = 16; HG_DEV static void run(const Team& T, XStream& S, XHint h) { x_round<2, 2, 12, 0, 16, 0, 0, 4, 0, 0, 1, 0, 0, 1, 1>(T, S, 18720, h); } };
template <> struct XInst<XP_MUL12_S, S_E, S_F, S_D> { static constexpr int kOff = 18976, kW = 16; HG_DEV static void run(const Team& T, XStream& S, XHint h) { x_round<2, 2, 12, 0, 16, 0, 0, 4, 0, 0, 1, 0, 0, 1, 1>(T, S, 18976, h); } };
template <> struct XInst<XP_MUL12_S, S_F, S_B, S_A> { static constexpr int kOff = 19232, kW = 16; HG_DEV static void run(const Team& T, XStream& S, XHint h) { x_round<2, 2, 12, 0, 16, 0, 0, 4, 0, 0, 1, 0, 0, 1, 1>(T, S, 19232, h); } };
template <> struct XInst<XP_MUL12_S, S_F, S_D, S_A> { static constexpr int kOff = 19488, kW = 16; HG_DEV static void run(const Team& T, XStream& S, XHint h) { x_round<2, 2, 12, 0, 16, 0, 0, 4, 0, 0, 1, 0, 0, 1, 1>(T, S, 19488, h); } };
template <> struct XInst<XP_MUL12_S, S_F, S_F, S_A> { static constexpr int kOff = 19744, kW = 16; HG_DEV static void run(const Team& T, XStream& S, XHint h) { x_round<2, 2, 12, 0, 16, 0, 0, 4, 0, 0, 1, 0, 0, 1, 1>(T, S, 19744, h); } };
template <> struct XInst<XP_MUL12_S, S_G, S_B, S_E> { static constexpr int kOff = 20000, kW = 16; HG_DEV static void run(const Team& T, XStream& S, XHint h) { x_round<2, 2, 12, 0, 16, 0, 0, 4, 0, 0, 1, 0, 0, 1, 1>(T, S, 20000, h); } };
template <> struct XInst<XP_SDBL_S, S_F, S_F> { static constexpr int kOff = 20256, kW = 12; HG_DEV static void run(const Team& T, XStream& S, XHint h) { x_round<3, 2, 7, 0, 12, 0, 0, 8, 0, 0, 1, 0, 0, 0, 1>(T, S, 20256, h); } };
template <> struct XInst<XP_CYC_SQR_X_12_T, S_A, S_A> { static constexpr int kOff = 20448, kW = 7; HG_DEV static void run(const Team& T, XStream& S, XHint h) { XQ<13>::x_round<2, 2, 3, 1, 7, 0, 0, 4, 2, 0, 1, 0, 1, 0, 0>(T, S, 20448, h); } };
template <> struct XInst<XP_CYC_SQR_X_12_T, S_B, S_A> { static constexpr int kOff = 20560, kW = 7; HG_DEV static void run(const Team& T, XStream& S, XHint h) { XQ<13>::x_round<2, 2, 3, 1, 7, 0, 0, 4, 2, 0, 1, 0, 1, 0, 0>(T, S, 20560, h); } };
template <> struct XInst<XP_CYC_SQR_X_12_T, S_C, S_B> { static constexpr int kOff = 20672, kW = 7; HG_DEV static void run(const Team& T, XStream& S, XHint h) { XQ<13>::x_round<2, 2, 3, 1, 7, 0, 0, 4, 2, 0, 1, 0, 1, 0, 0>(T, S, 20672, h); } };
template <> struct XInst<XP_CYC_SQR_X_12_T, S_C, S_C> { static constexpr int kOff = 20784, kW = 7; HG_DEV static void run(const Team& T, XStream& S, XHint h) { XQ<13>::x_round<2, 2, 3, 1, 7, 0, 0, 4, 2, 0, 1, 0, 1, 0, 0>(T, S, 20784, h); } };
template <> struct XInst<XP_CYC_SQR_X_12_T, S_C, S_D> { static constexpr int kOff = 20896, kW = 7; HG_DEV static void run(const Team& T, XStream& S, XHint h) { XQ<13>::x_round<2, 2, 3, 1, 7, 0, 0, 4, 2, 0, 1, 0, 1, 0, 0>(T, S, 20896, h); } };
template <> struct XInst<XP_CYC_SQR_X_12_T, S_C, S_F> { static constexpr int kOff = 21008, kW = 7; HG_DEV static void run(const Team& T, XStream& S, XHint h) { XQ<13>::x_round<2, 2, 3, 1, 7, 0, 0, 4, 2, 0, 1, 0, 1, 0, 0>(T, S, 21008, h); } };
template <> struct XInst<XP_CYC_SQR_X_12_T, S_D, S_C> { static constexpr int kOff = 21120, kW = 7; HG_DEV static void run(const Team& T, XStream& S, XHint h) { XQ<13>::x_round<2, 2, 3, 1, 7, 0, 0, 4, 2, 0, 1, 0, 1, 0, 0>(T, S, 21120, h); } };
template <> struct XInst<XP_CYC_SQR_X_12_T, S_D, S_D> { static constexpr int kOff = 21232, kW = 7; HG_DEV static void run(const Team& T, XStream& S, XHint h) { XQ<13>::x_round<2, 2, 3, 1, 7, 0, 0, 4, 2, 0, 1, 0, 1, 0, 0>(T, S, 21232, h); } };
template <> struct XInst<XP_LINE_FIX_12_T, S_F, S_F> { static constexpr int kOff = 21344, kW = 7; HG_DEV static void run(const Team& T, XStream& S, XHint h) { XQ<13>::x_round<1, 2, 4, 2, 7, 0, 0, 4, 1, 0, 1, 0, 0, 1, 0>(T, S, 21344, h); } };
template <> struct XInst<XP_MUL12_12_T, S_A, S_D, S_B> { static constexpr int kOff = 21456, kW = 16; HG_DEV static void run(const Team& T, XStream& S, XHint h) { x_round<2, 2, 12, 0, 16, 0, 0, 4, 0, 0, 1, 0, 0, 1, 0>(T, S, 21456, h); } };
template <> struct XInst<XP_MUL12_12_T, S_B, S_A, S_B> { static constexpr int kOff = 21712, kW = 16; HG_DEV static void run(const Team& T, XStream& S, XHint h) { x_round<2, 2, 12, 0, 16, 0, 0, 4, 0, 0, 1, 0, 0, 1, 0>(T, S, 21712, h); } };
template <> struct XInst<XP_MUL12_12_T, S_B, S_A, S_F> { static constexpr int kOff = 21968, kW = 16; HG_DEV static void run(const Team& T, XStream& S, XHint h) { x_round<2, 2, 12, 0, 16, 0, 0, 4, 0, 0, 1, 0, 0, 1, 0>(T, S, 21968, h); } };
template <> struct XInst<XP_MUL12_12_T, S_B, S_F, S_D> { static constexpr int kOff = 22224, kW = 16; HG_DEV static void run(const Team& T, XStream& S, XHint h) { x_round<2, 2, 12, 0, 16, 0, 0, 4, 0, 0, 1, 0, 0, 1, 0>(T, S, 22224, h); } };
template <> struct XInst<XP_MUL12_12_T, S_C, S_C, S_B> { static constexpr int kOff = 22480, kW = 16; HG_DEV static void run(const Team& T, XStream& S, XHint h) { x_round<2, 2, 12, 0, 16, 0, 0, 4, 0, 0, 1, 0, 0, 1, 0>(T, S, 22480, h); } };
template <> struct XInst<XP_MUL12_12_T, S_C, S_C, S_D> { static constexpr int kOff = 22736, kW = 16; HG_DEV static void run(const Team& T, XStream& S, XHint h) { x_round<2, 2, 12, 0, 16, 0, 0, 4, 0, 0, 1, 0, 0, 1, 0>(T, S, 22736, h); } };
template <> struct XInst<XP_MUL12_12_T, S_C, S_C, S_F> { static constexpr int kOff = 22992, kW = 16; HG_DEV static void run(const Team& T, XStream& S, XHint h) { x_round<2, 2, 12, 0, 16, 0, 0, 4, 0, 0, 1, 0, 0, 1, 0>(T, S, 22992, h); } };
template <> struct XInst<XP_MUL12_12_T, S_D, S_A, S_A> { static constexpr int kOff = 23248, kW = 16; HG_DEV static void run(const Team& T, XStream& S, XHint h) { x_round<2, 2, 12, 0, 16, 0, 0, 4, 0, 0, 1, 0, 0, 1, 0>(T, S, 23248, h); } };
template <> struct XInst<XP_MUL12_12_T, S_D, S_B, S_C> { static constexpr int kOff = 23504, kW = 16; HG_DEV static void run(const Team& T, XStream& S, XHint h) { x_round<2, 2, 12, 0, 16, 0, 0, 4, 0, 0, 1, 0, 0, 1, 0>(T, S, 23504, h); } };
template <> struct XInst<XP_MUL12_12_T, S_D, S_D, S_B> { static constexpr int kOff = 23760, kW = 16; HG_DEV static void run(const Team& T, XStream& S, XHint h) { x_round<2, 2, 12, 0, 16, 0, 0, 4, 0, 0, 1, 0, 0, 1, 0>(T, S, 23760, h); } };
template <> struct XInst<XP_MUL12_12_T, S_D, S_D, S_C> { static constexpr int kOff = 24016, kW = 16; HG_DEV static void run(const Team& T, XStream& S, XHint h) { x_round<2, 2, 12, 0, 16, 0, 0, 4, 0, 0, 1, 0, 0, 1, 0>(T, S, 24016, h); } };
template <> struct XInst<XP_MUL12_12_T, S_D, S_D, S_F> { static constexpr int kOff = 24272, kW = 16; HG_DEV static void run(const Team& T, XStream& S, XHint h) { x_round<2, 2, 12, 0, 16, 0, 0, 4, 0, 0, 1, 0, 0, 1, 0>(T, S, 24272, h); } };
template <> struct XInst<XP_MUL12_12_T, S_F, S_A, S_D> { static constexpr int kOff = 24528, kW = 16; HG_DEV static void run(const Team& T, XStream& S, XHint h) { x_round<2, 2, 12, 0, 16, 0, 0, 4, 0, 0, 1, 0, 0, 1, 0>(T, S, 24528, h); } };
template <> struct XInst<XP_MUL12_12_T, S_F, S_A, S_F> { static constexpr int kOff = 24784, kW = 16; HG_DEV static void run(const Team& T, XStream& S, XHint h) { x_round<2, 2, 12, 0, 16, 0, 0, 4, 0, 0, 1, 0, 0, 1, 0>(T, S, 24784, h); } };
template <> struct XInst<XP_MUL12_12_T, S_F, S_B, S_A> { static constexpr int kOff = 25040, kW = 16; HG_DEV static void run(const Team& T, XStream& S, XHint h) { x_round<2, 2, 12, 0, 16, 0, 0, 4, 0, 0, 1, 0, 0, 1, 0>(T, S, 25040, h); } };
template <> struct XInst<XP_MUL12_12_T, S_F, S_C, S_F> { static constexpr int kOff = 25296, kW = 16; HG_DEV static void run(const Team& T, XStream& S, XHint h) { x_round<2, 2, 12, 0, 16, 0, 0, 4, 0, 0, 1, 0, 0, 1, 0>(T, S, 25296, h); } };
template <> struct XInst<XP_MUL12_12_T, S_F, S_F, S_A> { static constexpr int kOff = 25552, kW = 16; HG_DEV static void run(const Team& T, XStream& S, XHint h) { x_round<2, 2, 12, 0, 16, 0, 0, 4, 0, 0, 1, 0, 0, 1, 0>(T, S, 25552, h); } };
template <> struct XInst<XP_SQR12_12_T, S_F, S_F> { static constexpr int kOff = 25808, kW = 12; HG_DEV static void run(const Team& T, XStream& S, XHint h) { x_round<3, 2, 7, 0, 12, 0, 0, 8, 0, 0, 1, 0, 0, 0, 0>(T, S, 25808, h); } };
template <> struct XInst<XP_MDBL_1_V, S_F, S_F> { static constexpr int kOff = 26000, kW = 16; HG_DEV static void run(const Team& T, XStream& S, XHint h) { x_round<4, 2, 7, 0, 16, 2, 0, -1, -1, -1, 1, 0, 0, 0, 0>(T, S, 26000, h); } };
template <> struct XInst<XP_MDBL_2_V, S_F, S_F> { static constexpr int kOff = 26256, kW = 14; HG_DEV static void run(const Team& T, XStream& S, XHint h) { x_round<2, 4, 4, 2, 14, 2, 2, -1, -1, -1, 1, 0, 0, 0, 0>(T, S, 26256, h); } };
template <> struct XInst<XP_PDBL_1_V> { static constexpr int kOff = 26480, kW = 4; HG_DEV static void run(const Team& T, XStream& S, XHint h) { x_round<1, 2, 2, 0, 4, 0, 0, -1, -1, -1, 0, 0, 0, 0, 0>(T, S, 26480, h); } };
template <> struct XInst<XP_LINE_PK_V, S_F, S_F> { static constexpr int kOff = 26544, kW = 8; HG_DEV static void run(const Team& T, XStream& S, XHint h) { x_round<1, 2, 6, 0, 8, 0, 0, 4, 0, 0, 1, 0, 0, 1, 0>(T, S, 26544, h); } };
template <> struct XInst<XP_PADD_POS_1_V> { static constexpr int kOff = 26672, kW = 5; HG_DEV static void run(const Team& T, XStream& S, XHint h) { x_round<1, 2, 2, 1, 5, 0, 0, 1, 0, 0, 0, 0, 0, 0, 0>(T, S, 26672, h); } };
template <> struct XInst<XP_PADD_POS_3_V> { static constexpr int kOff = 26752, kW = 10; HG_DEV static void run(const Team& T, XStream& S, XHint h) { x_round<2, 2, 6, 0, 10, 0, 0, 4, 0, 0, 1, 0, 0, 0, 0>(T, S, 26752, h); } };
template <> struct XInst<XP_PADD_NEG_1_V> { static constexpr int kOff = 26912, kW = 5; HG_DEV static void run(const Team& T, XStream& S, XHint h) { x_round<1, 2, 2, 1, 5, 0, 0, 1, 0, 0, 0, 0, 0, 0, 0>(T, S, 26912, h); } };
template <> struct XInst<XP_PADD_NEG_3_V> { static constexpr int kOff = 26992, kW = 10; HG_DEV static void run(const Team& T, XStream& S, XHint h) { x_round<2, 2, 6, 0, 10, 0, 0, 4, 0, 0, 1, 0, 0, 0, 0>(T, S, 26992, h); } };
template <> struct XInst<XP_PADD_F1_1_V> { static constexpr int kOff = 27152, kW = 5; HG_DEV static void run(const Team& T, XStream& S, XHint h) { x_round<1, 2, 2, 1, 5, 0, 0, 1, 0, 0, 0, 0, 0, 0, 0>(T, S, 27152, h); } };
template <> struct XInst<XP_PADD_F1_3_V> { static constexpr int kOff = 27232, kW = 10; HG_DEV static void run(const Team& T, XStream& S, XHint h) { x_round<2, 2, 6, 0, 10, 0, 0, 4, 0, 0, 1, 0, 0, 0, 0>(T, S, 27232, h); } };
template <> struct XInst<XP_PADD_F2_1_V> { static constexpr int kOff = 27392, kW = 5; HG_DEV static void run(const Team& T, XStream& S, XHint h) { x_round<1, 2, 2, 1, 5, 0, 0, 1, 0, 0, 0, 0, 0, 0, 0>(T, S, 27392, h); } };
template <> struct XInst<XP_PADD_F2_3_V> { static constexpr int kOff = 27472, kW = 10; HG_DEV static void run(const Team& T, XStream& S, XHint h) { x_round<2, 2, 6, 0, 10, 0, 0, 4, 0, 0, 1, 0, 0, 0, 0>(T, S, 27472, h); } };
template <> struct XInst<XP_MADD_POS_2_V, S_F, S_F> { static constexpr int kOff = 27632, kW = 10; HG_DEV static void run(const Team& T, XStream& S, XHint h) { x_round<1, 2, 4, 2, 10, 2, 0, 4, 1, 0, 1, 0, 0, 0, 0>(T, S, 27632, h); } };
template <> struct XInst<XP_MADD_NEG_2_V, S_F, S_F> { static constexpr int kOff = 27792, kW = 10; HG_DEV static void run(const Team& T, XStream& S, XHint h) { x_round<1, 2, 4, 2, 10, 2, 0, 4, 1, 0, 1, 0, 0, 0, 0>(T, S, 27792, h); } };
template <> struct XInst<XP_MADD_F1_2_V, S_F, S_F> { static constexpr int kOff = 27952, kW = 10; HG_DEV static void run(const Team& T, XStream& S, XHint h) { x_round<1, 2, 4, 2, 10, 2, 0, 4, 1, 0, 1, 0, 0, 0, 0>(T, S, 27952, h); } };
template <> struct XInst<XP_MADD_F2_2_V, S_F, S_F> { static constexpr int kOff = 28112, kW = 10; HG_DEV static void run(const Team& T, XStream& S, XHint h) { x_round<1, 2, 4, 2, 10, 2, 0, 4, 1, 0, 1, 0, 0, 0, 0>(T, S, 28112, h); } };
}
```

### handel_amd/csrc/hg_aggregate.cpp

```cpp
#include <cstring>

#include "hg_ctx.h"

namespace {

__global__ void k_agg_codes(const int32_t* sig_codes, const int32_t* lvl_codes, int hash_eof, int n, int32_t* out) {
  int i = blockIdx.x * blockDim.x + threadIdx.x;
  if (i >= n) return;
  int32_t c = sig_codes[i];
  if (c == HG_OK && lvl_codes[i] == HG_ERR_LEVEL) c = HG_ERR_LEVEL;
  if (c == HG_OK && hash_eof) c = HG_ERR_HASH_EOF;
  if (c == HG_OK) c = lvl_codes[i];
  out[i] = c;
}
}

static void level_codes(hg_ctx* c, const hg_request* reqs, size_t n, std::vector<int32_t>& out) {
  out.resize(n);
  for (size_t i = 0; i < n; i++) {
    const hg_request& r = reqs[i];
    bool ok = r.bitlen == r.level_size && (size_t)r.offset + r.bitlen <= c->nreg;
    out[i] = ok ? HG_OK : HG_ERR_LEVEL;
  }
}

static constexpr size_t kGtMaxRegistry = 16384;
static constexpr size_t kGtLevel1Requests = 16384;
static constexpr size_t kGtLevel2Requests = (size_t)1 << 20;
static constexpr int kNoMem = -1;
static constexpr int kOverBudget = -2;
int gt_forced_level() {
  static const int lvl = [] {
    const char* p = getenv("HG_AGG_PATH");
    if (p && strcmp(p, "g2") == 0) return 0;
    const char* e = getenv("HG_GT_LEVEL");
    if (!e) return -1;
    const int v = atoi(e);
    return v >= 0 && v <= 2 ? v : -1;
  }();
  return lvl;
}
static int resolve_subgroup(hg_ctx* c) {
  if (!c->sub_pending) return HG_OK;
  int cnt = 0;
  HG_CHECK(c, hipEventSynchronize(c->ev_sub));
  HG_CHECK(c, hipMemcpy(&cnt, c->sub_count.p, sizeof cnt, hipMemcpyDeviceToHost));
  c->reg_non_g2 = (size_t)cnt;
  c->sub_pending = false;
  return HG_OK;
}
static int gt_max_level(const hg_ctx* c) {
  if (c->reg_non_g2 || c->sub_pending) return 0;
  const int top = c->nreg <= kGtMaxRegistry ? 2 : 1;
  return top < c->gt_cap ? top : c->gt_cap;
}

#define HG_GT_ALLOC(ctx, expr)                                                     \
  do {                                                                             \
    hipError_t e_ = (expr);                                                        \
    if (e_ == hipErrorOutOfMemory) {                                               \
      (void)hipGetLastError();        \
      return kNoMem;                                                               \
    }                                                                              \
    if (e_ != hipSuccess) {                                                        \
      (ctx)->err = std::string(#expr) + ": " + hipGetErrorString(e_);              \
      return HG_ERR_DEVICE;                                                        \
    }                                                                              \
  } while (0)

static size_t gt_block_count(const hg_ctx* c, int* cnt) {
  size_t total = 0;
  for (int k = 4; k <= c->block_levels && k < 24; k++) {
    const size_t v = (c->nreg + ((size_t)1 << k) - 1) >> k;
    if (cnt) cnt[k] = (int)v;
    total += v;
  }
  return total;
}
static size_t gt_table_bytes(const hg_ctx* c, int level) {
  const size_t n = c->nreg, nwin8 = (n + 7) / 8, nwin16 = (n + 15) / 16;
  size_t b = 0;
  if (level >= 1) b += (n + nwin8 * 256 + gt_block_count(c, nullptr)) * sizeof(Gt);
  if (level >= 2) b += nwin16 * 65536 * sizeof(Gt);
  return b;
}

static int build_gt_locked(hg_ctx* c, hipStream_t s, int level) {
  const int n = (int)c->nreg;
  const int nwin8 = (n + 7) / 8, nwin16 = (n + 15) / 16;
  if (c->cur.gt_level < 1 && level >= 1) {
    if (gt_table_bytes(c, 1) + c->alt.table_bytes() > c->table_budget) return kOverBudget;
    int cnt[24] = {0};
    const size_t total = gt_block_count(c, cnt);
    int base = 0;
    for (int k = 4; k <= c->block_levels && k < 24; k++) {
      c->gt_bi.base[k] = base;
      base += cnt[k];
    }
    HG_GT_ALLOC(c, c->cur.gt_key.ensure(n));
    HG_GT_ALLOC(c, c->cur.gt_w8.ensure((size_t)nwin8 * 256));
    if (total) HG_GT_ALLOC(c, c->cur.gt_blk.ensure(total));
    launch_gt_keys(c->reg.p, n, c->d_lines.p, c->cur.d_h.p, c->cur.gt_key.p, s);
    launch_gt_windows8(c->cur.gt_key.p, n, c->cur.gt_w8.p, nwin8, s);
    for (int k = 4; k <= c->block_levels && k < 24; k++) {
      if (k == 4) launch_gt_blocks(c->cur.gt_w8.p + 255, 256, nwin8, c->cur.gt_blk.p + c->gt_bi.base[4], cnt[4], s);
      else launch_gt_blocks(c->cur.gt_blk.p + c->gt_bi.base[k - 1], 1, cnt[k - 1], c->cur.gt_blk.p + c->gt_bi.base[k], cnt[k], s);
    }
    int rc = check_launch(c);
    if (rc) return rc;
    c->cur.gt_level = 1;
  }
  if (c->cur.gt_level < 2 && level >= 2) {
    if (gt_table_bytes(c, 2) + c->alt.table_bytes() > c->table_budget) return kOverBudget;
    HG_GT_ALLOC(c, c->cur.gt_win.ensure((size_t)nwin16 * 65536));
    launch_gt_windows16(c->cur.gt_w8.p, nwin8, c->cur.gt_win.p, nwin16, s);
    int rc = check_launch(c);
    if (rc) return rc;
    c->cur.gt_level = 2;
  }
  return HG_OK;
}

static void gt_lower_cap(hg_ctx* c, int cap, bool oom) {
  if (cap < 0) cap = 0;
  if (cap < c->gt_cap) c->gt_cap = cap;
  if (oom && cap < c->oom_cap) c->oom_cap = cap;
  if (c->gt_cap < 2) c->cur.gt_win.reset();
  if (c->gt_cap < 1) c->cur.drop_tables();
  if (c->cur.gt_level > c->gt_cap) c->cur.gt_level = c->gt_cap;
}

static int build_fitting_locked(hg_ctx* c, hipStream_t s, int& level) {
  while (level > c->cur.gt_level) {
    int rc = build_gt_locked(c, s, level);
    if (rc == kNoMem || rc == kOverBudget) {
      if (c->alt.drop_tables()) continue;
      gt_lower_cap(c, c->cur.gt_level < level ? c->cur.gt_level : level - 1, rc == kNoMem);
      level = level < c->gt_cap ? level : c->gt_cap;
      continue;
    }
    if (rc) return rc;
  }
  return HG_OK;
}

static int gt_submission_level(hg_ctx* c, size_t n) {
  if (c->cur.hash_eof || c->nreg == 0) return 0;
  const bool wants_gt = c->pinned_level > 0 || c->cur.gt_level > 0 || c->cur.gt_requests + n >= kGtLevel1Requests;
  if (wants_gt && resolve_subgroup(c) != HG_OK) return 0;
  const int top = gt_max_level(c);
  if (c->pinned_level >= 0) return c->pinned_level < top ? c->pinned_level : top;
  c->cur.gt_requests += n;
  int want = c->cur.gt_requests >= kGtLevel2Requests ? 2 : (c->cur.gt_requests >= kGtLevel1Requests ? 1 : 0);
  if (want < c->cur.gt_level) want = c->cur.gt_level;
  return want < top ? want : top;
}

static int gt_chunk() {
  static const int chunk = env_int("HG_GT_CHUNK", kGtChunk, 1, 64);
  return chunk;
}
static size_t fold_terms_bound(size_t bitlen) { return 8 * ((bitlen + 7 + 63) / 64) + 1; }
struct FoldCaps {
  size_t terms = 0, chunks = 0;
  void add(size_t bitlen) {
    const size_t m = fold_terms_bound(bitlen);
    terms += m;
    chunks += (m + gt_chunk() - 1) / gt_chunk();
  }
};
static FoldCaps fold_caps_worst(const hg_ctx* c, size_t n) {
  FoldCaps one;
  one.add(c->nreg);
  return FoldCaps{one.terms * n, one.chunks * n};
}
static FoldCaps fold_caps_lane(size_t n, size_t max_words) {
  const size_t terms = 8 * (max_words + n) + n;
  return FoldCaps{terms, terms / (size_t)gt_chunk() + n};
}

enum : unsigned { kWsVerify = 1, kWsLevel = 2, kWsG2Fold = 4, kWsAggOut = 8, kWsGtFold = 16, kWsPairing = 32, kWsSide = 64 };
static hipError_t ws_ensure(Ws& ws, size_t n, unsigned parts, const FoldCaps& caps = {}, size_t sig_bytes = 0) {
  hipError_t e = hipSuccess;
  auto grow = [&e](auto& buf, size_t count) {
    if (e == hipSuccess) e = buf.ensure(count);
  };
  if (parts & kWsVerify) grow(ws.pts1, n), grow(ws.codes_b, n);
  if (parts & kWsLevel) grow(ws.codes_c, n);
  if (parts & kWsG2Fold) grow(ws.checks, n), grow(ws.order, n), grow(ws.agg_ws, n * agg_partial_bytes() + agg_fixed_bytes());
  if (parts & kWsAggOut) grow(ws.pts2, n);
  if (parts & kWsGtFold) {
    grow(ws.gt_plan, n), grow(ws.gt_hdr, 1), grow(ws.gt_terms, caps.terms), grow(ws.gt_ord, caps.chunks);
    grow(ws.gt_multi, 2 * n), grow(ws.gt_partial, caps.chunks), grow(ws.gt_y, n);
  }
  if (parts & kWsPairing) grow(ws.gt_fe, n), grow(ws.sig_lines, sig_bytes);
  if ((parts & kWsSide) && e == hipSuccess) e = ensure_side(ws);
  return e;
}

static int ensure_gt_fold(hg_ctx* c, Ws& ws, size_t n, const FoldCaps& caps, GtWork& w) {
  static const int grid = env_int("HG_GT_GRID", 4096, 64, 65536);
  if (caps.chunks > (size_t)INT32_MAX || caps.terms > (size_t)INT32_MAX) return kNoMem;
  HG_GT_ALLOC(c, ws_ensure(ws, n, kWsGtFold, caps));
  w.plan = ws.gt_plan.p;
  w.hdr = ws.gt_hdr.p;
  w.terms = ws.gt_terms.p;
  w.ord = ws.gt_ord.p;
  w.cap = (int)caps.chunks;
  w.multi = ws.gt_multi.p;
  w.partial = ws.gt_partial.p;
  const size_t per_wg = kGtChunkTeams;
  const size_t need = (caps.chunks + per_wg - 1) / per_wg;
  w.chunk_grid = (int)(need < (size_t)grid ? (need ? need : 1) : (size_t)grid);
  w.chunk = gt_chunk();
  return HG_OK;
}

static int gt_acquire(hg_ctx* c, Ws& ws, hipStream_t s, size_t n, const FoldCaps& caps, int& level, GtWork& w,
                      bool may_build = true) {
  if (!may_build && level > c->cur.gt_level) level = c->cur.gt_level;
  if (level > 0 && c->cur.gt_level < level) {
    int rc = build_fitting_locked(c, s, level);
    if (rc) return rc;
  }
  if (level > 0) {
    int rc = ensure_gt_fold(c, ws, n, caps, w);
    if (rc == kNoMem) level = 0;
    else if (rc) return rc;
  }
  return HG_OK;
}

bool gt_overlap() {
  static const bool on = env_int("HG_GT_OVERLAP", 1, 0, 1) != 0;
  return on;
}

__global__ void k_level_codes(const hg_request* r, int n, uint32_t nreg, int32_t* out) {
  int i = blockIdx.x * blockDim.x + threadIdx.x;
  if (i >= n) return;
  bool ok = r[i].bitlen == r[i].level_size && (uint64_t)r[i].offset + r[i].bitlen <= nreg;
  out[i] = ok ? HG_OK : HG_ERR_LEVEL;
}

struct AggBatch {
  const hg_request* reqs;
  size_t n;
  const uint64_t* words;
  const uint8_t* sigs;
  int32_t* codes;
  uint8_t* agg = nullptr;
  int32_t* lvl = nullptr;
  uint8_t* bits = nullptr;
  const FoldCaps* caps = nullptr;
};

static void gt_prologue(hg_ctx* c, const AggBatch& b, Ws& ws, const GtWork& gw, hipStream_t s) {
  launch_agg_prologue(b.reqs, (int)b.n, (uint32_t)c->nreg, b.sigs, c->flavor, ws.pts1.p, b.codes, (int*)gw.hdr,
                      (int)(sizeof(GtHdr) / sizeof(int)), s);
}
static void gt_fold(hg_ctx* c, const AggBatch& b, Ws& ws, const GtWork& gw, int32_t* codes, bool zero_hdr,
                    hipStream_t s) {
  launch_gt_fold(b.reqs, (int)b.n, b.words, codes, (int)c->nreg, c->block_levels,
                 gw.win_bits == 16 ? c->cur.gt_win.p : c->cur.gt_w8.p, c->cur.gt_blk.p, c->gt_bi, gw, ws.gt_y.p, zero_hdr,
                 s);
}

static int flow_gt_beside(hg_ctx* c, const AggBatch& b, Ws& ws, SigForm form, const GtWork& gw, hipStream_t s) {
  const int n = (int)b.n;
  HG_CHECK(c, hipEventRecord(ws.ev_fork, s));
  PhaseTimer t(c, HG_PHASE_VERIFY, s);
  const bool ran = launch_sig_form(form, b.sigs, c->flavor, n, c->d_lines.p, ws.sig_lines.p, ws.gt_fe.p, s);
  t.stop();
  if (!ran) {
    c->err = "aggregate batch too large for its pairing form";
    return HG_ERR_ARG;
  }
  HG_CHECK(c, hipStreamWaitEvent(ws.side, ws.ev_fork, 0));
  gt_prologue(c, b, ws, gw, ws.side);
  PhaseTimer fold(c, HG_PHASE_AGGREGATE, ws.side);
  gt_fold(c, b, ws, gw, b.codes, false, ws.side);
  fold.stop();
  HG_CHECK(c, hipEventRecord(ws.ev_join, ws.side));
  HG_CHECK(c, hipStreamWaitEvent(s, ws.ev_join, 0));
  if (b.bits) launch_gt_compare_bits(ws.gt_fe.p, ws.gt_y.p, n, b.codes, b.bits, s);
  else launch_gt_compare(ws.gt_fe.p, ws.gt_y.p, n, b.codes, s);
  return HG_OK;
}

static int flow_gt_sequence(hg_ctx* c, const AggBatch& b, Ws& ws, const GtWork& gw, hipStream_t s) {
  const int n = (int)b.n;
  gt_prologue(c, b, ws, gw, s);
  PhaseTimer fold(c, HG_PHASE_AGGREGATE, s);
  gt_fold(c, b, ws, gw, b.codes, false, s);
  fold.stop();
  PhaseTimer t(c, HG_PHASE_VERIFY, s);
  launch_verify_sig(ws.pts1.p, n, c->d_lines.p, ws.gt_y.p, b.codes, s);
  t.stop();
  if (b.bits) launch_pack_verdicts(b.codes, n, b.bits, s);
  return HG_OK;
}

static int flow_g2_or_mixed(hg_ctx* c, const AggBatch& b, Ws& ws, bool verify, bool use_gt, bool g2_fold,
                            const GtWork& gw, hipStream_t s) {
  const int n = (int)b.n;
  int32_t* d_lvl = b.lvl;
  if (!d_lvl) {
    d_lvl = ws.codes_c.p;
    k_level_codes<<<nb(b.n), 256, 0, s>>>(b.reqs, n, (uint32_t)c->nreg, d_lvl);
  }
  PhaseTimer fold(c, HG_PHASE_AGGREGATE, s);
  if (g2_fold)
    launch_aggregate(c->wsum.p, (int)c->nreg, c->blocks.p, c->block_base.data(), c->block_levels, b.reqs, n, b.words,
                     ws.order.p, ws.agg_ws.p, ws.checks.p, d_lvl, s);
  if (use_gt) gt_fold(c, b, ws, gw, d_lvl, true, s);
  fold.stop();
  if (b.agg) {
    launch_extract_pk(ws.checks.p, n, ws.pts2.p, s);
    launch_encode_g2(ws.pts2.p, n, b.agg, s);
  }
  if (verify) {
    launch_decode_g1(b.sigs, n, c->flavor, ws.pts1.p, ws.codes_b.p, s);
    k_agg_codes<<<nb(b.n), 256, 0, s>>>(ws.codes_b.p, d_lvl, c->cur.hash_eof ? 1 : 0, n, b.codes);
    if (use_gt) {
      PhaseTimer t(c, HG_PHASE_VERIFY, s);
      launch_verify_sig(ws.pts1.p, n, c->d_lines.p, ws.gt_y.p, b.codes, s);
      t.stop();
    } else if (!c->cur.hash_eof) {
      launch_sig_into_checks(ws.pts1.p, n, ws.checks.p, s);
      PhaseTimer t(c, HG_PHASE_VERIFY, s);
      launch_verify(ws.checks.p, n, c->d_lines.p, c->cur.d_h.p, b.codes, s);
      t.stop();
    }
  }
  if (b.bits) launch_pack_verdicts(b.codes, n, b.bits, s);
  return HG_OK;
}

static int aggregate_device_locked(hg_ctx* c, const AggBatch& b, bool verify, hipStream_t s, Ws& ws,
                                   const SigPolicy& pol, bool is_lane) {
  if (verify && !c->cur.has_msg) {
    c->err = "hg_set_message was not called";
    return HG_ERR_ARG;
  }
  const size_t n = b.n;
  Submission sub(c, s);
  if (!is_lane) HG_CHECK(c, sub.start());
  int level = verify ? gt_submission_level(c, n) : 0;
  GtWork gw{};
  if (level > 0) {
    int rc = gt_acquire(c, ws, s, n, b.caps ? *b.caps : fold_caps_worst(c, n), level, gw, !is_lane);
    if (rc) return rc;
  }
  gw.win_bits = level == 2 ? 16 : 8;
  const bool use_gt = level > 0;
  const bool g2_fold = !use_gt || b.agg;
  const bool beside = use_gt && !g2_fold && pol.overlap;
  const SigForm form = sig_form(sig_env(), pol, n);
  const unsigned parts = (g2_fold ? kWsG2Fold : 0) | (b.agg ? kWsAggOut : 0) | (b.lvl ? 0 : kWsLevel) |
                         (verify ? kWsVerify : 0) | (beside ? kWsPairing | kWsSide : 0);
  HG_CHECK(c, ws_ensure(ws, n, parts, {}, sig_form_ws_bytes(form, (int)n)));
  PhaseTimer all(c, HG_PHASE_SUBMIT, s);
  int rc;
  if (beside) rc = flow_gt_beside(c, b, ws, form, gw, s);
  else if (use_gt && !g2_fold) rc = flow_gt_sequence(c, b, ws, gw, s);
  else rc = flow_g2_or_mixed(c, b, ws, verify, use_gt, g2_fold, gw, s);
  if (rc) return rc;
  all.stop();
  rc = check_launch(c);
  if (rc) return rc;
  if (!is_lane) HG_CHECK(c, sub.finish());
  return HG_OK;
}

static int aggregate_host_locked(hg_ctx* c, const hg_request* reqs, size_t n, const uint64_t* words, size_t nwords,
                                 const uint8_t* sigs, int32_t* codes, uint8_t* agg_out, bool verify) {
  HG_CHECK(c, hipSetDevice(c->device));
  std::vector<int32_t> lvl;
  level_codes(c, reqs, n, lvl);
  FoldCaps caps;
  for (size_t i = 0; i < n; i++) {
    if (lvl[i] != HG_OK) continue;
    if ((size_t)reqs[i].word_offset + (reqs[i].bitlen + 63) / 64 > nwords) {
      c->err = "request words out of range";
      return HG_ERR_ARG;
    }
    caps.add(reqs[i].bitlen);
  }
  HG_CHECK(c, c->reqs.ensure(n));
  HG_CHECK(c, c->words.ensure(nwords ? nwords : 1));
  HG_CHECK(c, c->codes_a.ensure(n));
  HG_CHECK(c, c->ws.codes_c.ensure(n));
  uint8_t* d_agg = nullptr;
  if (agg_out) {
    HG_CHECK(c, c->bytes_a.ensure(n * 128));
    d_agg = c->bytes_a.p;
  }
  if (verify) HG_CHECK(c, c->bytes_b.ensure(n * 64));
  Submission sub(c, c->stream);
  HG_CHECK(c, sub.start());
  HG_CHECK(c, hipMemcpyAsync(c->reqs.p, reqs, n * sizeof(hg_request), hipMemcpyHostToDevice, c->stream));
  if (nwords) HG_CHECK(c, hipMemcpyAsync(c->words.p, words, nwords * 8, hipMemcpyHostToDevice, c->stream));
  HG_CHECK(c, hipMemcpyAsync(c->ws.codes_c.p, lvl.data(), n * 4, hipMemcpyHostToDevice, c->stream));
  if (verify) HG_CHECK(c, hipMemcpyAsync(c->bytes_b.p, sigs, n * 64, hipMemcpyHostToDevice, c->stream));
  const AggBatch b{c->reqs.p, n, c->words.p, verify ? c->bytes_b.p : nullptr, c->codes_a.p, d_agg, c->ws.codes_c.p,
                   nullptr, &caps};
  int rc = aggregate_device_locked(c, b, verify, c->stream, c->ws, c->pol, false);
  if (rc) return rc;
  if (agg_out) HG_CHECK(c, hipMemcpyAsync(agg_out, d_agg, n * 128, hipMemcpyDeviceToHost, c->stream));
  HG_CHECK(c, hipMemcpyAsync(codes, verify ? c->codes_a.p : c->ws.codes_c.p, n * 4, hipMemcpyDeviceToHost, c->stream));
  HG_CHECK(c, sub.finish());
  HG_CHECK(c, hipStreamSynchronize(c->stream));
  if (agg_out) {
    for (size_t i = 0; i < n; i++)
      if (lvl[i] != HG_OK || codes[i] == HG_ERR_EMPTY_AGG) memset(agg_out + 128 * i, 0, 128);
  }
  return HG_OK;
}

static int prepare_aggregate_locked(hg_ctx* c, int want = -1) {
  if (!c->cur.has_msg || c->nreg == 0) {
    c->err = "hg_prepare_aggregate: needs a message and a registry";
    return HG_ERR_ARG;
  }
  if (c->cur.hash_eof) return HG_ERR_HASH_EOF;
  int src = resolve_subgroup(c);
  if (src) return src;
  int level = gt_max_level(c);
  if (c->pinned_level >= 0 && c->pinned_level < level) level = c->pinned_level;
  if (want >= 0 && want < level) level = want;
  if (c->cur.gt_level >= level) return HG_OK;
  HG_CHECK(c, hipSetDevice(c->device));
  Submission sub(c, c->stream);
  HG_CHECK(c, sub.start());
  int rc = build_fitting_locked(c, c->stream, level);
  if (rc) return rc;
  HG_CHECK(c, sub.finish());
  HG_CHECK(c, hipStreamSynchronize(c->stream));
  return HG_OK;
}

extern "C" {

int hg_prepare_aggregate(hg_ctx* c) {
  if (!c) return HG_ERR_ARG;
  std::lock_guard<std::mutex> g(c->mu);
  return prepare_aggregate_locked(c);
}

int hg_prepare_aggregate_msg(hg_ctx* c, const uint8_t* msg, size_t len) {
  if (!c || (!msg && len)) return HG_ERR_ARG;
  std::lock_guard<std::mutex> g(c->mu);
  int rc = set_message_locked(c, msg, len);
  if (rc) return rc;
  return prepare_aggregate_locked(c);
}

int hg_set_aggregate_level(hg_ctx* c, int level) {
  if (!c || level < -1 || level > 2) return HG_ERR_ARG;
  std::lock_guard<std::mutex> g(c->mu);
  c->pinned_level = level;
  return HG_OK;
}

int hg_set_fold_overlap(hg_ctx* c, int on) {
  if (!c) return HG_ERR_ARG;
  std::lock_guard<std::mutex> g(c->mu);
  c->pol.overlap = on != 0;
  return HG_OK;
}

int hg_set_verify_split(hg_ctx* c, int on) {
  if (!c) return HG_ERR_ARG;
  std::lock_guard<std::mutex> g(c->mu);
  c->verify_split = on != 0;
  return HG_OK;
}

int hg_set_table_budget(hg_ctx* c, size_t bytes) {
  if (!c) return HG_ERR_ARG;
  std::lock_guard<std::mutex> g(c->mu);
  c->table_budget = bytes;
  if (gt_table_bytes(c, c->cur.gt_level) + c->alt.table_bytes() > bytes) c->alt.drop_tables();
  if (c->cur.gt_level >= 1 && gt_table_bytes(c, c->cur.gt_level) > bytes)
    gt_lower_cap(c, gt_table_bytes(c, 1) <= bytes ? 1 : 0, false);
  c->gt_cap = c->oom_cap;
  return HG_OK;
}

size_t hg_registry_non_g2(hg_ctx* c) {
  if (!c) return 0;
  std::lock_guard<std::mutex> g(c->mu);
  if (resolve_subgroup(c) != HG_OK) return 0;
  return c->reg_non_g2;
}

int hg_aggregate_tables(hg_ctx* c) {
  if (!c) return 0;
  std::lock_guard<std::mutex> g(c->mu);
  return c->cur.gt_level;
}

int hg_verify_aggregate_device(hg_ctx* c, const hg_request* d_reqs, size_t n, const uint64_t* d_words,
                               const uint8_t* d_sigs, int32_t* d_codes, uint8_t* d_agg_pk_out, void* stream) {
  if (!c || (n && (!d_reqs || !d_sigs || !d_codes)) || n > (size_t)INT32_MAX) return HG_ERR_ARG;
  if (n == 0) return HG_OK;
  std::lock_guard<std::mutex> g(c->mu);
  HG_CHECK(c, hipSetDevice(c->device));
  hipStream_t s = stream ? (hipStream_t)stream : c->stream;
  return aggregate_device_locked(c, AggBatch{d_reqs, n, d_words, d_sigs, d_codes, d_agg_pk_out}, true, s, c->ws, c->pol,
                                 false);
}

int hg_verify_aggregate_device_bits(hg_ctx* c, const hg_request* d_reqs, size_t n, const uint64_t* d_words,
                                    const uint8_t* d_sigs, int32_t* d_codes, uint8_t* d_bits, void* stream) {
  if (!c || (n && (!d_reqs || !d_sigs || !d_codes || !d_bits)) || n > (size_t)INT32_MAX) return HG_ERR_ARG;
  if (n == 0) return HG_OK;
  std::lock_guard<std::mutex> g(c->mu);
  HG_CHECK(c, hipSetDevice(c->device));
  hipStream_t s = stream ? (hipStream_t)stream : c->stream;
  return aggregate_device_locked(c, AggBatch{d_reqs, n, d_words, d_sigs, d_codes, nullptr, nullptr, d_bits}, true, s,
                                 c->ws, c->pol, false);
}

int hg_verify_aggregate(hg_ctx* c, const hg_request* reqs, size_t n, const uint64_t* words, size_t nwords,
                        const uint8_t* sigs, int32_t* codes, uint8_t* agg_pk_out) {
  if (!c || (n && (!reqs || !sigs || !codes)) || n > (size_t)INT32_MAX) return HG_ERR_ARG;
  if (n == 0) return HG_OK;
  std::lock_guard<std::mutex> g(c->mu);
  return aggregate_host_locked(c, reqs, n, words, nwords, sigs, codes, agg_pk_out, true);
}

int hg_verify_aggregate_msg(hg_ctx* c, const uint8_t* msg, size_t len, const hg_request* reqs, size_t n,
                            const uint64_t* words, size_t nwords, const uint8_t* sigs, int32_t* codes,
                            uint8_t* agg_pk_out) {
  if (!c || (!msg && len) || (n && (!reqs || !sigs || !codes)) || n > (size_t)INT32_MAX) return HG_ERR_ARG;
  std::lock_guard<std::mutex> g(c->mu);
  int rc = set_message_locked(c, msg, len);
  if (rc != HG_OK && rc != HG_ERR_HASH_EOF) return rc;
  if (n == 0) return HG_OK;
  return aggregate_host_locked(c, reqs, n, words, nwords, sigs, codes, agg_pk_out, true);
}

int hg_verify_multisig(hg_ctx* c, const uint32_t* bitlens, const uint32_t* word_offsets, size_t n,
                       const uint64_t* words, size_t nwords, const uint8_t* sigs, int32_t* codes) {
  if (!c || (n && (!bitlens || !word_offsets || !sigs || !codes)) || n > (size_t)INT32_MAX) return HG_ERR_ARG;
  if (n == 0) return HG_OK;
  std::lock_guard<std::mutex> g(c->mu);
  std::vector<hg_request> reqs(n);
  for (size_t i = 0; i < n; i++) reqs[i] = hg_request{0u, bitlens[i], (uint32_t)c->nreg, word_offsets[i]};
  int rc = aggregate_host_locked(c, reqs.data(), n, words, nwords, sigs, codes, nullptr, true);
  if (rc) return rc;
  for (size_t i = 0; i < n; i++)
    if (bitlens[i] != c->nreg) codes[i] = HG_ERR_MULTI_SIZES;
  return HG_OK;
}

int hg_aggregate_pk(hg_ctx* c, const hg_request* reqs, size_t n, const uint64_t* words, size_t nwords,
                    uint8_t* agg_pk_out, int32_t* codes) {
  if (!c || (n && (!reqs || !agg_pk_out || !codes)) || n > (size_t)INT32_MAX) return HG_ERR_ARG;
  if (n == 0) return HG_OK;
  std::lock_guard<std::mutex> g(c->mu);
  return aggregate_host_locked(c, reqs, n, words, nwords, nullptr, codes, agg_pk_out, false);
}

int hg_prepare_aggregate_level(hg_ctx* c, int level) {
  if (!c || level < 0 || level > 2) return HG_ERR_ARG;
  std::lock_guard<std::mutex> g(c->mu);
  return prepare_aggregate_locked(c, level);
}

int hg_lane_create(hg_ctx* c, size_t max_batch, size_t max_words, int overlap, hg_lane** out) {
  if (!c || !out || max_batch == 0 || max_batch > (size_t)INT32_MAX || max_words > ((size_t)1 << 40))
    return HG_ERR_ARG;
  *out = nullptr;
  std::lock_guard<std::mutex> g(c->mu);
  HG_CHECK(c, hipSetDevice(c->device));
  hg_lane* l = new hg_lane();
  l->c = c;
  l->pol.overlap = overlap != 0;
  l->max_batch = max_batch;
  l->max_words = max_words;
  const size_t bytes = ((max_batch * sizeof(hg_request) + 255) & ~(size_t)255) +
// ... 142 lines not shown
```

### handel_amd/csrc/hg_ctx.h

```cpp
#pragma once
#include <hip/hip_runtime.h>

#include <cstdint>
#include <cstdlib>
#include <mutex>
#include <string>
#include <utility>
#include <vector>

#include "bn256_gt.h"
#include "bn256_kernels.h"
#include "hg_codes.h"
#include "hg_dev.h"
#include "hg_packets.h"
#include "hg_stores.h"

namespace hg {

struct Ws {
  DevBuf<PointG2> pts2;
  DevBuf<PointG1> pts1;
  DevBuf<CheckIn> checks;
  DevBuf<int32_t> codes_b, codes_c;
  DevBuf<int> order;
  DevBuf<uint8_t> agg_ws;
  DevBuf<GtReq> gt_plan;
  DevBuf<GtHdr> gt_hdr;
  DevBuf<uint32_t> gt_terms;
  DevBuf<int2> gt_ord;
  DevBuf<int> gt_multi;
  DevBuf<Gt> gt_partial, gt_y;
  Stream side;
  Event ev_fork, ev_join;
  DevBuf<Gt> gt_fe;
  DevBuf<uint8_t> sig_lines;
  size_t bytes() const {
    return pts2.bytes() + pts1.bytes() + checks.bytes() + codes_b.bytes() + codes_c.bytes() + order.bytes() +
           agg_ws.bytes() + gt_plan.bytes() + gt_hdr.bytes() + gt_terms.bytes() + gt_ord.bytes() + gt_multi.bytes() +
           gt_partial.bytes() + gt_y.bytes() + gt_fe.bytes() + sig_lines.bytes();
  }
};

struct TableSet {
  std::vector<uint8_t> msg;
  bool has_msg = false, hash_eof = false;
  DevBuf<PointG1> d_h;
  DevBuf<Gt> gt_key, gt_w8, gt_win, gt_blk;
  int gt_level = 0;
  size_t gt_requests = 0;
  size_t table_bytes() const { return gt_key.bytes() + gt_w8.bytes() + gt_win.bytes() + gt_blk.bytes(); }
  bool drop_tables() {
    if (table_bytes() == 0) return false;
    gt_key.reset();
    gt_w8.reset();
    gt_win.reset();
    gt_blk.reset();
    gt_level = 0;
    return true;
  }
};

}

using namespace hg;

struct hg_ctx {
  int device = 0;
  int flavor = HG_FLAVOR_GO;
  Stream stream;
  std::mutex mu;
  std::string err;
  DevBuf<LineCoef> d_lines;
  DevBuf<uint32_t> d_k;
  TableSet cur, alt;
  DevBuf<PointG2> reg;
  size_t nreg = 0;
  uint64_t reg_gen = 0;
  DevBuf<PointG2> blocks;
  DevBuf<PointG2> wsum;
  std::vector<int> block_base = std::vector<int>(24, 0);
  int block_levels = 0;
  Ws ws;
  DevBuf<uint8_t> bytes_a, bytes_b;
  DevBuf<PointG1> pts1b;
  DevBuf<int32_t> codes_a;
  DevBuf<hg_request> reqs;
  DevBuf<hg_packet> pkts;
  DevBuf<uint64_t> words;
  int pinned_level = -1;
  int gt_cap = 2;
  size_t table_budget = SIZE_MAX;
  size_t reg_non_g2 = 0;
  bool sub_pending = false;
  Event ev_sub;
  DevBuf<int> sub_count;
  GtBlockIndex gt_bi{};
  int oom_cap = 2;
  SigPolicy pol;
  bool verify_split = false;
  Event last_ev;
  hipStream_t last_s = nullptr;
  std::vector<hg_lane*> lanes;
  bool timing = false;
  std::vector<std::pair<Event, Event>> events[HG_NUM_PHASES];
};

struct hg_lane {
  hg_ctx* c = nullptr;
  Ws ws;
  Stream s;
  Event done;
  bool recorded = false;
  SigPolicy pol{true, sig_env().w2_lane_max, true};
  Event ev_in;
  size_t max_batch = 0, max_words = 0;
  HostBuf<uint8_t> h_in;
  HostBuf<int32_t> h_codes;
  DevBuf<uint8_t> d_in;
  DevBuf<int32_t> d_codes;
  size_t n = 0, nwords = 0, off_sigs = 0, off_words = 0, in_bytes = 0;
  size_t bytes() const { return ws.bytes() + d_in.bytes() + d_codes.bytes(); }
};

struct hg_stores {
  hg_ctx* c = nullptr;
  uint64_t reg_gen = 0;
  size_t nreg = 0, max_packets = 0;
  int levels = 0, stride = 0;
  std::vector<uint32_t> receivers;
  std::vector<int32_t> map;
  DevBuf<uint64_t> tab;
  DevBuf<uint32_t> flags;
  DevBuf<int32_t> d_map;
  DevBuf<hg_store_update> ups;
  DevBuf<uint64_t> up_words;
  DevBuf<hg_packet> pkts;
  DevBuf<uint64_t> words;
  DevBuf<int32_t> codes, scores;
  DevBuf<uint8_t> live;
  DevBuf<uint64_t> keys_a, keys_b;
// ... 115 lines not shown
```

### handel_amd/engine.py

```python

from __future__ import annotations

import ctypes
import weakref
from typing import Optional, Sequence, Tuple

import numpy as np

from . import _lib
from ._lib import HandelGPUError

FLAVORS = {"go": _lib.HG_FLAVOR_GO, "bn256/go": _lib.HG_FLAVOR_GO,
           "cf": _lib.HG_FLAVOR_CF, "bn256/cf": _lib.HG_FLAVOR_CF, "bn256": _lib.HG_FLAVOR_CF}

REQ_DTYPE = np.dtype([("offset", "<u4"), ("bitlen", "<u4"), ("level_size", "<u4"), ("word_offset", "<u4")])
PACKET_DTYPE = np.dtype([("origin", "<i4"), ("receiver", "<u4"), ("level", "<u4"), ("flags", "<u4"),
                         ("ms_off", "<u4"), ("ms_len", "<u4"), ("ind_off", "<u4"), ("ind_len", "<u4")])
STORE_UPDATE_DTYPE = np.dtype([("receiver", "<u4"), ("level", "<u4"), ("flags", "<u4"), ("best_off", "<u4"),
                               ("indiv_off", "<u4")])
STORE_SIG_DTYPE = np.dtype([("receiver", "<u4"), ("level", "<u4"), ("index", "<u4"), ("sig_off", "<u4")])
STORE_QUERY_DTYPE = np.dtype([("receiver", "<u4"), ("level", "<u4")])


def _ptr(a) -> Optional[int]:
# ... 4 lines not shown
    return a.ctypes.data


def _u8(b) -> np.ndarray:
    if isinstance(b, np.ndarray):
        return np.ascontiguousarray(b, dtype=np.uint8)
    return np.frombuffer(bytes(b), dtype=np.uint8).copy()


class Engine:

    def __init__(self, device: int = 0, flavor: str = "go"):
        self.L = _lib.load()
        self.flavor_name = flavor
        self.flavor = FLAVORS[flavor]
        h = ctypes.c_void_p()
        rc = self.L.hg_create(device, self.flavor, ctypes.byref(h))
        if rc != 0:
            raise HandelGPUError(f"hg_create failed: code {rc}")
        self.ctx = h
        self.device = device

    def close(self):
        if getattr(self, "ctx", None):
            for ref in getattr(self, "_stores", []):
                st = ref()
                if st is not None:
                    st.close()
            self.L.hg_destroy(self.ctx)
            self.ctx = None

    def __del__(self):
        try:
            self.close()
        except Exception:
            pass

    def _check(self, rc: int, what: str, ok=(0,)):
        if rc not in ok:
            err = self.L.hg_last_error(self.ctx)
            raise HandelGPUError(f"{what}: code {rc}: {err.decode() if err else ''}")
        return rc

    def code_string(self, code: int) -> str:
        return self.L.hg_code_string(int(code), self.flavor).decode()

    def processing_error_string(self, code: int) -> str:
        return self.L.hg_processing_error_string(int(code), self.flavor).decode()

    def set_message(self, msg: bytes) -> int:
        m = _u8(msg)
        return self._check(self.L.hg_set_message(self.ctx, _ptr(m) if len(m) else None, len(m)),
                           "hg_set_message", ok=(0, _lib.HG_ERR_HASH_EOF))

    def prepare_aggregate(self) -> int:
        return self._check(self.L.hg_prepare_aggregate(self.ctx), "hg_prepare_aggregate",
                           ok=(0, _lib.HG_ERR_HASH_EOF))

    def prepare_aggregate_msg(self, msg: bytes) -> int:
        m = _u8(msg)
        return self._check(self.L.hg_prepare_aggregate_msg(self.ctx, _ptr(m) if len(m) else None, len(m)),
                           "hg_prepare_aggregate_msg", ok=(0, _lib.HG_ERR_HASH_EOF))

    def set_aggregate_level(self, level: int) -> None:
        self._check(self.L.hg_set_aggregate_level(self.ctx, int(level)), "hg_set_aggregate_level")

    def set_fold_overlap(self, on: bool) -> None:
        self._check(self.L.hg_set_fold_overlap(self.ctx, int(bool(on))), "hg_set_fold_overlap")

    def set_verify_split(self, on: bool) -> None:
        self._check(self.L.hg_set_verify_split(self.ctx, int(bool(on))), "hg_set_verify_split")

    def set_table_budget(self, nbytes: int) -> None:
        self._check(self.L.hg_set_table_budget(self.ctx, int(nbytes)), "hg_set_table_budget")

    def registry_non_g2(self) -> int:
        return int(self.L.hg_registry_non_g2(self.ctx))

    def context_bytes(self) -> int:
        return int(self.L.hg_context_bytes(self.ctx))

    def aggregate_tables(self) -> int:
        return int(self.L.hg_aggregate_tables(self.ctx))

    def registry_load(self, pks: bytes) -> np.ndarray:
        a = _u8(pks)
        n = len(a) // 128
        codes = np.zeros(n, dtype=np.int32)
        rc = self.L.hg_registry_load(self.ctx, _ptr(a), n, _ptr(codes))
        self._check(rc, "hg_registry_load", ok=(0, _lib.HG_ERR_PK_UNMARSHAL))
        return codes

    def verify_batch(self, pks: bytes, sigs: bytes) -> np.ndarray:
        a, b = _u8(pks), _u8(sigs)
        n = len(b) // 64
        if len(a) != 128 * n:
            raise ValueError("pks must hold 128 bytes per signature")
        codes = np.zeros(n, dtype=np.int32)
        self._check(self.L.hg_verify_batch(self.ctx, _ptr(a), _ptr(b), n, _ptr(codes)), "hg_verify_batch")
        return codes

    def verify_batch_msg(self, msg: bytes, pks: bytes, sigs: bytes) -> np.ndarray:
        m, a, b = _u8(msg), _u8(pks), _u8(sigs)
        n = len(b) // 64
        if len(a) != 128 * n:
            raise ValueError("pks must hold 128 bytes per signature")
        codes = np.zeros(n, dtype=np.int32)
        rc = self.L.hg_verify_batch_msg(self.ctx, _ptr(m) if len(m) else None, len(m), _ptr(a) if n else None,
                                        _ptr(b) if n else None, n, _ptr(codes) if n else None)
        self._check(rc, "hg_verify_batch_msg")
        return codes

    def verify_batch_device(self, d_pks: int, d_sigs: int, n: int, d_codes: int, stream: int = 0):
        self._check(self.L.hg_verify_batch_device(self.ctx, d_pks, d_sigs, n, d_codes, stream or None),
                    "hg_verify_batch_device")

    def pack_verdicts_device(self, d_codes: int, n: int, d_bits: int, stream: int = 0):
        self._check(self.L.hg_pack_verdicts_device(self.ctx, d_codes, n, d_bits, stream or None),
                    "hg_pack_verdicts_device")

    SIG_K16_PAD, SIG_K16, SIG_K12_PAD, SIG_K12, SIG_W2 = 0, 1, 2, 3, 4

    def sig_pairing_device(self, d_sigs: int, n: int, d_fe: int, kernel: int, stream: int = 0):
        self._check(self.L.hg_sig_pairing_device(self.ctx, d_sigs, n, d_fe, int(kernel), stream or None),
                    "hg_sig_pairing_device")

    def verify_aggregate(self, reqs: np.ndarray, words: np.ndarray, sigs: bytes, want_agg: bool = False):
        reqs = np.ascontiguousarray(reqs, dtype=REQ_DTYPE)
        words = np.ascontiguousarray(words, dtype=np.uint64)
        s = _u8(sigs)
        n = len(reqs)
        codes = np.zeros(n, dtype=np.int32)
        agg = np.zeros(n * 128, dtype=np.uint8) if want_agg else None
        self._check(self.L.hg_verify_aggregate(self.ctx, _ptr(reqs), n, _ptr(words) if len(words) else None,
                                               len(words), _ptr(s), _ptr(codes), _ptr(agg)),
                    "hg_verify_aggregate")
        return (codes, agg.tobytes()) if want_agg else codes

    def packet_stride_words(self) -> int:
        return int(self.L.hg_packet_stride_words(self.ctx))

    def parse_packets(self, pool, pkts: np.ndarray, stride: Optional[int] = None):
        pkts = np.ascontiguousarray(pkts, dtype=PACKET_DTYPE)
        pool = _u8(pool)
        n = len(pkts)
        stride = self.packet_stride_words() if stride is None else int(stride)
        reqs, words, sigs, codes = _parse_outputs(n, stride)
        self._check(self.L.hg_parse_packets(self.ctx, _ptr(pool) if len(pool) else None, len(pool), _ptr(pkts), n,
                                            stride, _ptr(reqs), _ptr(words), _ptr(sigs), _ptr(codes)),
                    "hg_parse_packets")
        return reqs, words, sigs.tobytes(), codes

    def parse_packets_device(self, d_pool: int, pool_len: int, d_pkts: int, n: int, stride: int, d_reqs: int,
                             d_words: int, d_sigs: int, d_codes: int, stream: int = 0) -> None:
        self._check(self.L.hg_parse_packets_device(self.ctx, d_pool or None, pool_len, d_pkts, n, stride, d_reqs,
                                                   d_words, d_sigs, d_codes, stream or None),
                    "hg_parse_packets_device")

    def packet_error(self, code: int, pkt) -> str:
        p = np.ascontiguousarray(np.asarray(pkt, dtype=PACKET_DTYPE).reshape(1))
        buf = ctypes.create_string_buffer(256)
        self.L.hg_packet_error(self.ctx, int(code), _ptr(p), buf, 256)
        return buf.value.decode()

    def verify_aggregate_msg(self, msg: bytes, reqs: np.ndarray, words: np.ndarray, sigs: bytes):
        reqs = np.ascontiguousarray(reqs, dtype=REQ_DTYPE)
# ... 353 lines not shown
```

### include/handel_gpu.h

```cpp
#ifndef HANDEL_GPU_H
#define HANDEL_GPU_H

#include <stddef.h>
#include <stdint.h>

#ifdef __cplusplus
extern "C" {
#endif

enum hg_code {
  HG_OK = 0,
  HG_ERR_SIG_INVALID = 1,
  HG_ERR_HASH_EOF = 2,
  HG_ERR_LEVEL = 3,
  HG_ERR_PK_UNMARSHAL = 4,
  HG_ERR_SIG_UNMARSHAL = 5,
  HG_ERR_EMPTY_AGG = 6,
  HG_ERR_CF_EXCEEDS = 7,
  HG_ERR_CF_MALFORMED = 8,
  HG_ERR_CF_SHORT = 9,
  HG_ERR_SIG_CF_EXCEEDS = 10,
  HG_ERR_SIG_CF_MALFORMED = 11,
  HG_ERR_SIG_CF_SHORT = 12,
  HG_ERR_MULTI_SIZES = 13,
  HG_ERR_PKT_ORIGIN = 20,
  HG_ERR_PKT_LEVEL = 21,
  HG_ERR_PKT_EOF = 22,
  HG_ERR_PKT_UNEXPECTED_EOF = 23,
  HG_ERR_PKT_BITSET_SHORT = 24,
  HG_ERR_PKT_TYPE_MISMATCH = 25,
  HG_ERR_PKT_BITSET_SIZE = 26,
  HG_ERR_PKT_NO_SIG = 27,
  HG_ERR_PKT_ID_RANGE = 28,
  HG_PKT_NO_IND = 29,
  HG_ERR_ARG = 100,
  HG_ERR_DEVICE = 101
};

enum hg_flavor {
  HG_FLAVOR_GO = 0,
  HG_FLAVOR_CF = 1
};

typedef struct hg_ctx hg_ctx;

typedef struct {
  uint32_t offset;
  uint32_t bitlen;
  uint32_t level_size;
  uint32_t word_offset;
} hg_request;

int hg_create(int device, int flavor, hg_ctx** out);
void hg_destroy(hg_ctx* ctx);
const char* hg_last_error(hg_ctx* ctx);
const char* hg_code_string(int code, int flavor);
const char* hg_processing_error_string(int code, int flavor);
int hg_version(void);
int hg_context_flavor(hg_ctx* ctx);
int hg_context_simds(hg_ctx* ctx);

int hg_registry_load(hg_ctx* ctx, const uint8_t* pks, size_t n, int32_t* codes);
size_t hg_registry_size(hg_ctx* ctx);

int hg_set_message(hg_ctx* ctx, const uint8_t* msg, size_t len);

int hg_verify_batch_msg(hg_ctx* ctx, const uint8_t* msg, size_t len, const uint8_t* pks, const uint8_t* sigs,
                        size_t n, int32_t* codes);

int hg_verify_batch(hg_ctx* ctx, const uint8_t* pks, const uint8_t* sigs, size_t n, int32_t* codes);

int hg_verify_batch_device(hg_ctx* ctx, const uint8_t* d_pks, const uint8_t* d_sigs, size_t n, int32_t* d_codes,
                           void* stream);

int hg_pack_verdicts_device(hg_ctx* ctx, const int32_t* d_codes, size_t n, uint8_t* d_bits, void* stream);

int hg_verify_aggregate(hg_ctx* ctx, const hg_request* reqs, size_t n, const uint64_t* words, size_t nwords,
                        const uint8_t* sigs, int32_t* codes, uint8_t* agg_pk_out);

int hg_verify_aggregate_msg(hg_ctx* ctx, const uint8_t* msg, size_t len, const hg_request* reqs, size_t n,
                            const uint64_t* words, size_t nwords, const uint8_t* sigs, int32_t* codes,
                            uint8_t* agg_pk_out);

int hg_verify_multisig(hg_ctx* ctx, const uint32_t* bitlens, const uint32_t* word_offsets, size_t n,
                       const uint64_t* words, size_t nwords, const uint8_t* sigs, int32_t* codes);

int hg_prepare_aggregate(hg_ctx* ctx);
int hg_prepare_aggregate_msg(hg_ctx* ctx, const uint8_t* msg, size_t len);
int hg_aggregate_tables(hg_ctx* ctx);
int hg_set_aggregate_level(hg_ctx* ctx, int level);
int hg_set_fold_overlap(hg_ctx* ctx, int on);
int hg_set_verify_split(hg_ctx* ctx, int on);
int hg_set_table_budget(hg_ctx* ctx, size_t bytes);
size_t hg_registry_non_g2(hg_ctx* ctx);

int hg_verify_aggregate_device(hg_ctx* ctx, const hg_request* d_reqs, size_t n, const uint64_t* d_words,
                               const uint8_t* d_sigs, int32_t* d_codes, uint8_t* d_agg_pk_out, void* stream);

int hg_verify_aggregate_device_bits(hg_ctx* ctx, const hg_request* d_reqs, size_t n, const uint64_t* d_words,
                                    const uint8_t* d_sigs, int32_t* d_codes, uint8_t* d_bits, void* stream);

int hg_aggregate_pk(hg_ctx* ctx, const hg_request* reqs, size_t n, const uint64_t* words, size_t nwords,
                    uint8_t* agg_pk_out, int32_t* codes);

int hg_combine_g1(hg_ctx* ctx, const uint8_t* a, const uint8_t* b, size_t n, uint8_t* out, int32_t* codes);

int hg_combine_g2(hg_ctx* ctx, const uint8_t* a, const uint8_t* b, size_t n, uint8_t* out, int32_t* codes);

int hg_pair(hg_ctx* ctx, const uint8_t* g1s, const uint8_t* g2s, size_t n, uint8_t* gt_out, int32_t* codes);

int hg_keygen(hg_ctx* ctx, const uint8_t* scalars_be, size_t n, uint8_t* pks_out);
int hg_sign(hg_ctx* ctx, const uint8_t* scalars_be, size_t n, uint8_t* sigs_out);
int hg_sign_msg(hg_ctx* ctx, const uint8_t* msg, size_t len, const uint8_t* scalars_be, size_t n,
                uint8_t* sigs_out);

int hg_debug_fp_mul(hg_ctx* ctx, const uint32_t* a, const uint32_t* b, size_t n, uint32_t* out);

enum hg_phase { HG_PHASE_VERIFY = 0, HG_PHASE_AGGREGATE = 1, HG_PHASE_SUBMIT = 2, HG_NUM_PHASES = 3 };
int hg_timing_enable(hg_ctx* ctx, int on);
int hg_timing_read(hg_ctx* ctx, double* total_ms, int* launches);
int hg_timing_read_phase(hg_ctx* ctx, int phase, double* total_ms, int* launches);

int hg_debug_fp12(hg_ctx* ctx, int op, const uint8_t* a, const uint8_t* b, size_t n, uint8_t* out);

int hg_sig_pairing_device(hg_ctx* ctx, const uint8_t* d_sigs, size_t n, uint8_t* d_fe, int kernel, void* stream);

int hg_diag_read(hg_ctx* ctx, uint64_t* out, size_t n);

int hg_sync(hg_ctx* ctx);

size_t hg_context_bytes(hg_ctx* ctx);

typedef struct {
  int32_t origin;
  uint32_t receiver;
  uint32_t level;
  uint32_t flags;
  uint32_t ms_off, ms_len;
  uint32_t ind_off, ind_len;
} hg_packet;
#define HG_PKT_HAS_IND 1u
size_t hg_packet_stride_words(hg_ctx* ctx);
int hg_parse_packets(hg_ctx* ctx, const uint8_t* pool, size_t pool_len, const hg_packet* pkts, size_t n,
                     size_t stride_words, hg_request* reqs, uint64_t* words, uint8_t* sigs, int32_t* codes);
int hg_parse_packets_device(hg_ctx* ctx, const uint8_t* d_pool, size_t pool_len, const hg_packet* d_pkts, size_t n,
                            size_t stride_words, hg_request* d_reqs, uint64_t* d_words, uint8_t* d_sigs,
                            int32_t* d_codes, void* stream);
int hg_packet_error(hg_ctx* ctx, int code, const hg_packet* p, char* buf, size_t cap);

typedef struct hg_stores hg_stores;
typedef struct {
  uint32_t receiver;
  uint32_t level;
  uint32_t flags;
  uint32_t best_off, indiv_off;
} hg_store_update;
#define HG_STORE_HAS_BEST 1u
int hg_stores_create(hg_ctx* ctx, const uint32_t* receivers, size_t n_receivers, size_t max_packets, hg_stores** out);
void hg_stores_destroy(hg_stores* st);
int hg_stores_update(hg_stores* st, const hg_store_update* ups, size_t n, const uint64_t* words, size_t nwords);
int hg_stores_read(hg_stores* st, uint32_t receiver, uint32_t level, uint64_t* best, uint64_t* indiv, int* has_best);
int hg_stores_evaluate_device(hg_stores* st, const hg_packet* d_pkts, size_t n, size_t stride_words,
                              const uint64_t* d_words, const int32_t* d_codes, const uint8_t* d_live,
                              int32_t* d_scores, void* stream);
int hg_stores_evaluate(hg_stores* st, const hg_packet* pkts, size_t n, size_t stride_words, const uint64_t* words,
                       const int32_t* codes, const uint8_t* live, int32_t* scores);
size_t hg_stores_select_capacity(hg_stores* st, size_t n, uint32_t k);
int hg_stores_select_device(hg_stores* st, const hg_packet* d_pkts, size_t n, const int32_t* d_scores, uint32_t k,
                            const hg_request* d_reqs, const uint8_t* d_sigs, uint32_t* d_sel, uint32_t* d_count,
                            hg_request* d_out_reqs, uint8_t* d_out_sigs, void* stream);

#define HG_STORE_BEST_SIG 2u
// ... 86 lines not shown
```

Baseline: 6.735 million.

## Store level-2 GT tables in compressed torus form and fold with cheaper multiply

After building the 16-bit window GT tables, a one-time pass converts each Fp12 entry into a compressed torus (Fp6-ratio) representation using batched Montgomery-style inversion, zeroing the upper half. The fold kernel then reads only half the words per term and uses a new cheaper torus multiply program, and the final check compares the pairing output against the torus element via a dedicated compare kernel. This is meant to cut memory traffic and multiply cost in the aggregate fold. In exchange it adds a host sync at table build, a degenerate-entry scan fallback, and a different verification path that always runs the full pairing form.

Result: faster. 6.812 million (median of 6 runs) (+1.1%).

```diff
diff --git a/handel_amd/_lib.py b/handel_amd/_lib.py
--- a/handel_amd/_lib.py
+++ b/handel_amd/_lib.py
@@ -73,6 +73,7 @@
     "hg_registry_size": (_SZ, [_P]),
     "hg_prepare_aggregate": (_I, [_P]),
     "hg_aggregate_tables": (_I, [_P]),
+    "hg_aggregate_tables_torus": (_I, [_P]),
     "hg_prepare_aggregate_msg": (_I, [_P, _P, _SZ]),
     "hg_set_aggregate_level": (_I, [_P, _I]),
     "hg_set_table_budget": (_I, [_P, _SZ]),
diff --git a/handel_amd/csrc/bn256_gt.h b/handel_amd/csrc/bn256_gt.h
--- a/handel_amd/csrc/bn256_gt.h
+++ b/handel_amd/csrc/bn256_gt.h
@@ -37,6 +37,7 @@
   int chunk_grid;
   int chunk;
   int win_bits;
+  bool torus;
 };
 
 void launch_gt_keys(const PointG2* reg, int n, const LineCoef* tab, const PointG1* h, Gt* out, hipStream_t s);
@@ -52,6 +53,9 @@
                      hipStream_t s);
 size_t fe12_ws_bytes(int n);
 bool launch_fe12(Gt* fe, int n, uint8_t* ws, hipStream_t s);
+void launch_tor_scan(Gt* win, size_t nwin, Gt* blk, size_t nblk, int nreg, int* flag, hipStream_t s);
+void launch_tor_convert(Gt* win, size_t nwin, Gt* blk, size_t nblk, int nreg, hipStream_t s);
+void launch_tor_compare(const Gt* fe, const Gt* x, int n, int32_t* codes, uint8_t* bits, hipStream_t s);
 void launch_gt_compare(const Gt* fe, const Gt* y, int n, int32_t* codes, hipStream_t s);
 void launch_gt_compare_bits(const Gt* fe, const Gt* y, int n, int32_t* codes, uint8_t* bits, hipStream_t s);
 
diff --git a/handel_amd/csrc/bn256_gt.hip b/handel_amd/csrc/bn256_gt.hip
--- a/handel_amd/csrc/bn256_gt.hip
+++ b/handel_amd/csrc/bn256_gt.hip
@@ -486,6 +486,286 @@
   if (l == 0) bits[b] = (uint8_t)(m & 0xffu);
 }
 
+struct Fp6 {
+  Fp2 c[3];
+};
+HG_DEV void f6_mul(Fp6& r, const Fp6& a, const Fp6& b) {
+  Fp2 t0, t1, t2, s, u, w;
+  Fp6 o;
+  f2_mul(t0, a.c[0], b.c[0]);
+  f2_mul(t1, a.c[1], b.c[1]);
+  f2_mul(t2, a.c[2], b.c[2]);
+  f2_add(s, a.c[1], a.c[2]);
+  f2_add(u, b.c[1], b.c[2]);
+  f2_mul(w, s, u);
+  f2_sub(w, w, t1);
+  f2_sub(w, w, t2);
+  f2_mul_xi(w, w);
+  f2_add(o.c[0], t0, w);
+  f2_add(s, a.c[0], a.c[1]);
+  f2_add(u, b.c[0], b.c[1]);
+  f2_mul(w, s, u);
+  f2_sub(w, w, t0);
+  f2_sub(w, w, t1);
+  f2_mul_xi(s, t2);
+  f2_add(o.c[1], w, s);
+  f2_add(s, a.c[0], a.c[2]);
+  f2_add(u, b.c[0], b.c[2]);
+  f2_mul(w, s, u);
+  f2_sub(w, w, t0);
+  f2_sub(w, w, t2);
+  f2_add(o.c[2], w, t1);
+  r = o;
+}
+HG_DEV void f6_adj_norm(Fp6& adj, Fp2& n, const Fp6& a) {
+  Fp2 A, B, C, t;
+  f2_sqr(A, a.c[0]);
+  f2_mul(t, a.c[1], a.c[2]);
+  f2_mul_xi(t, t);
+  f2_sub(A, A, t);
+  f2_sqr(B, a.c[2]);
+  f2_mul_xi(B, B);
+  f2_mul(t, a.c[0], a.c[1]);
+  f2_sub(B, B, t);
+  f2_sqr(C, a.c[1]);
+  f2_mul(t, a.c[0], a.c[2]);
+  f2_sub(C, C, t);
+  f2_mul(n, a.c[2], B);
+  f2_mul(t, a.c[1], C);
+  f2_add(n, n, t);
+  f2_mul_xi(n, n);
+  f2_mul(t, a.c[0], A);
+  f2_add(n, n, t);
+  adj.c[0] = A;
+  adj.c[1] = B;
+  adj.c[2] = C;
+}
+HG_DEV void tor_ld(Fp& v, const uint32_t* p) {
+  const uint2* src = (const uint2*)__builtin_assume_aligned(p, 8);
+#pragma unroll
+  for (int i = 0; i < 5; i++) {
+    const uint2 x = src[i];
+    v.l[2 * i] = x.x;
+    v.l[2 * i + 1] = x.y;
+  }
+}
+HG_DEV void tor_st(uint32_t* p, const Fp& v) {
+  uint2* dst = (uint2*)__builtin_assume_aligned(p, 8);
+#pragma unroll
+  for (int i = 0; i < 5; i++) dst[i] = make_uint2(v.l[2 * i], v.l[2 * i + 1]);
+}
+HG_DEV void tor_load_half(Fp6& r, const Gt* g, int odd) {
+#pragma unroll
+  for (int m = 0; m < 3; m++) {
+    tor_ld(r.c[m].x, g->w + 20 * (2 * m + odd));
+    tor_ld(r.c[m].y, g->w + 20 * (2 * m + odd) + 10);
+  }
+}
+struct TorTables {
+  Gt* win;
+  Gt* blk;
+  size_t nwin, nblk;
+  int nreg;
+};
+HG_DEV Gt* tor_entry(const TorTables& t, size_t idx) {
+  if (idx < t.nwin) {
+    const int w = (int)(idx >> 16), have = min(16, t.nreg - 16 * w);
+    return ((uint32_t)idx & ((1u << have) - 1u) & 0xffffu) ? t.win + idx : nullptr;
+  }
+  return idx < t.nwin + t.nblk ? t.blk + (idx - t.nwin) : nullptr;
+}
+__global__ __launch_bounds__(256) void k_tor_scan(TorTables t, int* flag) {
+  const size_t idx = (size_t)blockIdx.x * 256 + threadIdx.x;
+  const Gt* g = tor_entry(t, idx);
+  if (!g) return;
+  uint32_t any = 0;
+#pragma unroll
+  for (int m = 0; m < 3; m++) {
+    const uint4* p = reinterpret_cast<const uint4*>(g->w + 20 * (2 * m + 1));
+#pragma unroll
+    for (int i = 0; i < 5; i++) {
+      const uint4 v = p[i];
+      any |= v.x | v.y | v.z | v.w;
+    }
+  }
+  if (any == 0) atomicOr(flag, 1);
+}
+static constexpr int kTorRun = 16;
+__global__ __launch_bounds__(64) void k_tor_convert(TorTables t) {
+  const size_t first = ((size_t)blockIdx.x * 64 + threadIdx.x) * kTorRun;
+  Fp2 acc;
+  f2_one(acc);
+#pragma unroll 1
+  for (int i = 0; i < kTorRun; i++) {
+    Gt* g = tor_entry(t, first + i);
+    if (!g) continue;
+    Fp6 a, b, adj;
+    Fp2 n;
+    tor_load_half(b, g, 1);
+    f6_adj_norm(adj, n, b);
+    tor_load_half(a, g, 0);
+    Fp one;
+    fp_one(one);
+    fp_add(a.c[0].y, a.c[0].y, one);
+    f6_mul(a, a, adj);
+#pragma unroll
+    for (int m = 0; m < 3; m++) {
+      tor_st(g->w + 20 * m, a.c[m].x);
+      tor_st(g->w + 20 * m + 10, a.c[m].y);
+    }
+    tor_st(g->w + 60, n.x);
+    tor_st(g->w + 70, n.y);
+    tor_st(g->w + 80, acc.x);
+    tor_st(g->w + 90, acc.y);
+    f2_mul(acc, acc, n);
+  }
+  Fp2 inv;
+  f2_inv(inv, acc);
+  Fp zero;
+  fp_zero(zero);
+#pragma unroll 1
+  for (int i = kTorRun - 1; i >= 0; i--) {
+    Gt* g = tor_entry(t, first + i);
+    if (!g) continue;
+    Fp2 n, pre, ni;
+    tor_ld(n.x, g->w + 60);
+    tor_ld(n.y, g->w + 70);
+    tor_ld(pre.x, g->w + 80);
+    tor_ld(pre.y, g->w + 90);
+    f2_mul(ni, inv, pre);
+    f2_mul(inv, inv, n);
+#pragma unroll
+    for (int m = 0; m < 3; m++) {
+      Fp2 c;
+      tor_ld(c.x, g->w + 20 * m);
+      tor_ld(c.y, g->w + 20 * m + 10);
+      f2_mul(c, c, ni);
+      tor_st(g->w + 20 * m, c.x);
+      tor_st(g->w + 20 * m + 10, c.y);
+    }
+#pragma unroll
+    for (int e = 6; e < 12; e++) tor_st(g->w + 10 * e, zero);
+  }
+}
+
+using ITorF = XInst<XP_TORMULF, S_A, S_A, S_B>;
+HG_DEV void tor_mul(const Team& T, XStream& S) {
+  team_sync();
+  ITorF::run(T, S, xh<ITorF>());
+}
+HG_DEV void tor_read(Fp& v, const Gt* g, int e) { tor_ld(v, g->w + 10 * e); }
+HG_DEV void tor_put(const Team& T, const Fp& v0, bool conj) {
+  Fp v = v0, n;
+  fp_neg(n, v);
+  fp_sel(v, conj, n, v);
+  if (T.tl < 6) st_fp_a8(slot(T, S_B) + T.tl * 10, v.l);
+}
+
+__global__ __launch_bounds__(64, HG_CHUNK_WAVES) void k_tor_chunks(const Gt* win, const Gt* blk, const uint32_t* terms,
+                                                   const int2* ord, int cap, const GtReq* plan, const GtHdr* hdr,
+                                                   int chunk, Gt* partial, Gt* y) {
+  __shared__ __attribute__((aligned(16))) uint32_t lds[kTeams12 * kFoldWords];
+  Team T = make_team12(lds, kFoldWords);
+  fold_regs_init(T);
+  const int team = team12_index();
+  const int total = hdr->chunks, nlong = hdr->nlong;
+  const bool rd = T.tl < 6;
+  XStream S = x_stream();
+  for (int base = blockIdx.x * kTeams12; base < total; base += gridDim.x * kTeams12) {
+    const int k = base + team;
+    const bool valid = k < total && T.active;
+    int first = 0, cnt = 0, r = 0, c = 0;
+    bool single = false;
+    if (valid) {
+      const int2 e = k < nlong ? ord[k] : ord[cap - 1 - (k - nlong)];
+      c = e.x;
+      r = e.y;
+      const GtReq g = plan[r];
+      first = g.term_off + (c - g.chunk_off) * chunk;
+      cnt = min(chunk, g.term_off + g.m - first);
+      single = g.chunks == 1;
+    }
+    int maxc = cnt;
+#pragma unroll
+    for (int d = 1; d < 64; d <<= 1) maxc = max(maxc, __shfl_xor(maxc, d));
+    const uint32_t my_t = T.tl < cnt ? terms[first + T.tl] : 0u;
+    const int tbase = 12 * team;
+    auto term = [&](int i) -> uint32_t {
+      const uint32_t v = (uint32_t)__shfl((int)my_t, tbase + (i < 12 ? i : 0), 64);
+      return i < 12 ? v : (i < cnt ? terms[first + i] : 0u);
+    };
+    Fp cur, n1, n2, one;
+    fp_one(one);
+    fp_zero(cur);
+    fp_zero(n1);
+    fp_zero(n2);
+    const uint32_t t0 = term(0);
+    const bool even = (T.k & 1) == 0;
+    if (valid && even) tor_read(cur, term_ptr(t0, win, blk), T.k + T.comp);
+    {
+      Fp n;
+      fp_neg(n, cur);
+      fp_sel(cur, (t0 & kTermConj) != 0, n, cur);
+      fp_sel(cur, T.e == 3, one, cur);
+    }
+    if (T.active) st_fp_a8(slot(T, S_A) + T.e * 10, cur.l);
+    uint32_t t1 = term(1), t2 = term(2);
+    if (1 < cnt && rd) tor_read(n1, term_ptr(t1, win, blk), T.tl);
+    if (2 < cnt && rd) tor_read(n2, term_ptr(t2, win, blk), T.tl);
+#pragma unroll 1
+    for (int i = 1; i < maxc; i++) {
+      const bool pad = i >= cnt;
+      tor_put(T, n1, (t1 & kTermConj) != 0);
+      n1 = n2;
+      t1 = t2;
+      t2 = term(i + 2);
+      if (i + 2 < cnt && rd) tor_read(n2, term_ptr(t2, win, blk), T.tl);
+      if (pad) lds_fp12_copy(T, slot(T, S_F), slot(T, S_A));
+      tor_mul(T, S);
+      team_sync();
+      if (pad) lds_fp12_copy(T, slot(T, S_A), slot(T, S_F));
+    }
+    team_sync();
+    if (valid) gt_store(T, S_A, single ? y + r : partial + c);
+    team_sync();
+  }
+}
+
+__global__ __launch_bounds__(64) void k_tor_compare_bits(const Gt* fe, const Gt* x, int n, int32_t* codes,
+                                                         uint8_t* bits) {
+  __shared__ __attribute__((aligned(16))) uint32_t lds[4 * kFoldWords];
+  Team T = make_team(lds, kFoldWords);
+  fold_regs_init(T);
+  const int team = (threadIdx.x & 63) >> 4;
+  const int b = blockIdx.x;
+  XStream S = x_stream();
+  uint32_t m = 0;
+#pragma unroll 1
+  for (int j = 0; j < 2; j++) {
+    const int r = 8 * b + 4 * j + team;
+    const int ci = min(r, n - 1);
+    team_sync();
+    gt_load(T, S_A, fe + ci);
+    gt_load(T, S_B, x + ci, true);
+    fold_mul(T, S);
+    team_sync();
+    gt_load(T, S_B, x + ci);
+    team_sync();
+    const bool eq = t12_equal(T, S_A, S_B);
+    bool mine = false;
+    if (T.tl == 0 && r < n) {
+      int32_t c = codes[r];
+      if (c == HG_OK) c = eq ? HG_OK : HG_ERR_SIG_INVALID;
+      codes[r] = c;
+      mine = c == HG_OK;
+    }
+    const uint64_t bal = __ballot(mine);
+#pragma unroll
+    for (int q = 0; q < 4; q++) m |= (uint32_t)((bal >> (16 * q)) & 1u) << (4 * j + q);
+  }
+  if (bits && threadIdx.x == 0) bits[b] = (uint8_t)m;
+}
+
 void launch_gt_keys(const PointG2* reg, int n, const LineCoef* tab, const PointG1* h, Gt* out, hipStream_t s) {
   if (n > 0) k_gt_keys<4><<<nblk(n, 4), 64, 0, s>>>(reg, n, tab, h, out);
 }
@@ -504,6 +784,7 @@
 void launch_gt_fold(const AggRequest* reqs, int n, const uint64_t* words, int32_t* codes, int nreg, int levels,
                     const Gt* win, const Gt* blk, const GtBlockIndex& bi, GtWork w, Gt* y, bool zero_hdr, hipStream_t s) {
   if (n <= 0) return;
+  if (w.torus && w.win_bits != 16) abort();
   if (zero_hdr) (void)hipMemsetAsync(w.hdr, 0, sizeof(GtHdr), s);
   if (w.win_bits == 16)
     k_gt_plan<16><<<nblk(n, kPlanWaves), 64 * kPlanWaves, 0, s>>>(reqs, n, words, codes, nreg, levels, bi, w.plan,
@@ -511,8 +792,23 @@
   else
     k_gt_plan<8><<<nblk(n, kPlanWaves), 64 * kPlanWaves, 0, s>>>(reqs, n, words, codes, nreg, levels, bi, w.plan,
                                                                  w.hdr, w.terms, w.ord, w.cap, w.chunk, w.multi);
-  k_gt_chunks<<<w.chunk_grid, 64, 0, s>>>(win, blk, w.terms, w.ord, w.cap, w.plan, w.hdr, w.chunk, w.partial, y);
+  if (w.torus)
+    k_tor_chunks<<<w.chunk_grid, 64, 0, s>>>(win, blk, w.terms, w.ord, w.cap, w.plan, w.hdr, w.chunk, w.partial, y);
+  else
+    k_gt_chunks<<<w.chunk_grid, 64, 0, s>>>(win, blk, w.terms, w.ord, w.cap, w.plan, w.hdr, w.chunk, w.partial, y);
   k_gt_combine<<<n, 64, 0, s>>>(n, w.hdr, w.multi, w.plan, w.partial, y);
+}
+void launch_tor_scan(Gt* win, size_t nwin, Gt* blk, size_t nblk_, int nreg, int* flag, hipStream_t s) {
+  const size_t total = nwin + nblk_;
+  (void)hipMemsetAsync(flag, 0, sizeof(int), s);
+  if (total) k_tor_scan<<<(unsigned)((total + 255) / 256), 256, 0, s>>>(TorTables{win, blk, nwin, nblk_, nreg}, flag);
+}
+void launch_tor_convert(Gt* win, size_t nwin, Gt* blk, size_t nblk_, int nreg, hipStream_t s) {
+  const size_t total = nwin + nblk_, per = 64 * kTorRun;
+  if (total) k_tor_convert<<<(unsigned)((total + per - 1) / per), 64, 0, s>>>(TorTables{win, blk, nwin, nblk_, nreg});
+}
+void launch_tor_compare(const Gt* fe, const Gt* x, int n, int32_t* codes, uint8_t* bits, hipStream_t s) {
+  if (n > 0) k_tor_compare_bits<<<(n + 7) / 8, 64, 0, s>>>(fe, x, n, codes, bits);
 }
 void launch_verify_sig(const PointG1* sigs, int n, const LineCoef* tab, const Gt* y, int32_t* codes, hipStream_t s) {
   if (n > 0) k_verify_sig<4, false><<<nblk(n, 4), 64, 0, s>>>(sigs, nullptr, 0, n, tab, y, nullptr, codes);
diff --git a/handel_amd/csrc/bn256_xtab.h b/handel_amd/csrc/bn256_xtab.h
--- a/handel_amd/csrc/bn256_xtab.h
+++ b/handel_amd/csrc/bn256_xtab.h
@@ -2,8 +2,8 @@
 #include <stdint.h>
 namespace hg {
 #define HG_P2N 0x0422599cu, 0x04ac6c5du, 0x05678616u, 0x05120b5au, 0x07b96e22u, 0x0584dc20u, 0x07fb2e17u, 0x047f9aa5u, 0x078d2a8du, 0x008fb500u
-enum XProg { XP_PDBL, XP_PADD_POS, XP_PADD_NEG, XP_PADD_F1, XP_PADD_F2, XP_MDBL_1, XP_MDBL_2, XP_PDBL_1, XP_PADD_POS_1, XP_MADD_POS_2, XP_PADD_POS_3, XP_PADD_NEG_1, XP_MADD_NEG_2, XP_PADD_NEG_3, XP_PADD_F1_1, XP_MADD_F1_2, XP_PADD_F1_3, XP_PADD_F2_1, XP_MADD_F2_2, XP_PADD_F2_3, XP_SQR12, XP_LINE_PK, XP_LINE_FIX, XP_CYC_SQR, XP_MUL12, XP_CYC_SQR_X, XP_FEVAL, XP_SDBL, XP_LFEV, XP_MUL12F, XP_SQR12_12, XP_LINE_FIX_12, XP_MUL12_12, XP_CYC_SQR_X_12, XP_LINE_FIX_S, XP_MUL12_S, XP_CYC_SQR_X_S, XP_FEVAL_S, XP_SDBL_S, XP_LFEV_S, XP_SQR12_12_T, XP_LINE_FIX_12_T, XP_MUL12_12_T, XP_CYC_SQR_X_12_T, XP_MDBL_1_V, XP_MDBL_2_V, XP_PDBL_1_V, XP_PADD_POS_1_V, XP_MADD_POS_2_V, XP_PADD_POS_3_V, XP_PADD_NEG_1_V, XP_MADD_NEG_2_V, XP_PADD_NEG_3_V, XP_PADD_F1_1_V, XP_MADD_F1_2_V, XP_PADD_F1_3_V, XP_PADD_F2_1_V, XP_MADD_F2_2_V, XP_PADD_F2_3_V, XP_LINE_PK_V };
-__constant__ static const uint32_t kXTab[28288] = {
+enum XProg { XP_PDBL, XP_PADD_POS, XP_PADD_NEG, XP_PADD_F1, XP_PADD_F2, XP_MDBL_1, XP_MDBL_2, XP_PDBL_1, XP_PADD_POS_1, XP_MADD_POS_2, XP_PADD_POS_3, XP_PADD_NEG_1, XP_MADD_NEG_2, XP_PADD_NEG_3, XP_PADD_F1_1, XP_MADD_F1_2, XP_PADD_F1_3, XP_PADD_F2_1, XP_MADD_F2_2, XP_PADD_F2_3, XP_SQR12, XP_LINE_PK, XP_LINE_FIX, XP_CYC_SQR, XP_MUL12, XP_CYC_SQR_X, XP_FEVAL, XP_SDBL, XP_LFEV, XP_MUL12F, XP_SQR12_12, XP_LINE_FIX_12, XP_MUL12_12, XP_CYC_SQR_X_12, XP_TORMULF, XP_LINE_FIX_S, XP_MUL12_S, XP_CYC_SQR_X_S, XP_FEVAL_S, XP_SDBL_S, XP_LFEV_S, XP_SQR12_12_T, XP_LINE_FIX_12_T, XP_MUL12_12_T, XP_CYC_SQR_X_12_T, XP_MDBL_1_V, XP_MDBL_2_V, XP_PDBL_1_V, XP_PADD_POS_1_V, XP_MADD_POS_2_V, XP_PADD_POS_3_V, XP_PADD_NEG_1_V, XP_MADD_NEG_2_V, XP_PADD_NEG_3_V, XP_PADD_F1_1_V, XP_MADD_F1_2_V, XP_PADD_F1_3_V, XP_PADD_F2_1_V, XP_MADD_F2_2_V, XP_PADD_F2_3_V, XP_LINE_PK_V };
+__constant__ static const uint32_t kXTab[28432] = {
   0x240616d0u, 0x19509000u, 0x90002906u, 0x28ee1bd0u, 0x16d09000u, 0x16f805c8u, 0x172006b8u, 0x16801748u, 0x24fe1680u, 0x00000f00u, 0x2a1216f8u, 0x19789000u,
   0x900028fau, 0x29fa1bf8u, 0x16d09000u, 0x177006b8u, 0x16800690u, 0x16801680u, 0x2a021680u, 0x00000ff0u, 0x2a031720u, 0x19a02b03u, 0x25032403u, 0x9000ffffu,
   0x17989000u, 0x17c00618u, 0x17e80708u, 0x16801810u, 0x28fe1680u, 0x00000fa0u, 0x2aff1748u, 0x19c82b01u, 0x250124ffu, 0x9000ffffu, 0x17989000u, 0x18380708u,
@@ -2360,6 +2360,18 @@
   0x09b009b0u, 0x3e0009b0u, 0xffff3e00u, 0x11a80af0u, 0x11800b18u, 0x000013b0u, 0x6eff03e8u, 0x09b03e00u, 0x09b009b0u, 0x09b009b0u, 0x09b009b0u, 0x3e0009b0u,
   0xffff3e00u, 0x11a80b18u, 0x11800410u, 0x000013d8u, 0x46ff0410u, 0x09b03e00u, 0x09b009b0u, 0x09b009b0u, 0x09b009b0u, 0x3e0009b0u, 0xffff3e00u, 0x09b009b0u,
   0x09b009b0u, 0x0000ffffu, 0x3e00ffffu, 0x09b03e00u, 0x09b009b0u, 0x09b009b0u, 0x09b009b0u, 0x3e0009b0u, 0xffff3e00u, 0x09b009b0u, 0x09b009b0u, 0x0000ffffu,
+  0x1cff05f0u, 0x01e01d03u, 0x020803e8u, 0x028003c0u, 0x02a805f0u, 0x03200618u, 0x03480640u, 0x16030668u, 0x01e01701u, 0x1c030618u, 0x02081d01u, 0x01e003e8u,
+  0x02a80690u, 0x028005f0u, 0x034806b8u, 0x03200640u, 0x170306e0u, 0x020816ffu, 0x1aff0640u, 0x02301b03u, 0x025803e8u, 0x02d003c0u, 0x02f805f0u, 0x03700618u,
+  0x03980640u, 0x0c010668u, 0x02302400u, 0x1a030668u, 0x02581b01u, 0x023003e8u, 0x02f80690u, 0x02d005f0u, 0x039806b8u, 0x03700640u, 0x0d0106e0u, 0x02582400u,
+  0x18ff0690u, 0x01e02400u, 0x02080438u, 0x02800410u, 0x02a803e8u, 0x032003c0u, 0x034805f0u, 0x0e010618u, 0x02802400u, 0x1cfd06b8u, 0x02081dffu, 0x01e00438u,
+  0x02a80708u, 0x028003e8u, 0x03480690u, 0x032005f0u, 0x0f0106b8u, 0x02a82400u, 0x1afd06e0u, 0x02301bffu, 0x02580438u, 0x02d00410u, 0x02f803e8u, 0x037003c0u,
+  0x039805f0u, 0x10010618u, 0x02d02400u, 0x1aff0708u, 0x02582400u, 0x02300438u, 0x02f80708u, 0x02d003e8u, 0x03980690u, 0x037005f0u, 0x110106b8u, 0x02f82400u,
+  0x1cff0730u, 0x01e02400u, 0x02080488u, 0x02800460u, 0x02a80438u, 0x03200410u, 0x034803e8u, 0x120103c0u, 0x03202400u, 0x2400ffffu, 0x02082400u, 0x01e00488u,
+  0x02a80730u, 0x02800438u, 0x03480708u, 0x032003e8u, 0x13010690u, 0x03482400u, 0x2400ffffu, 0x02302400u, 0x02580488u, 0x02d00460u, 0x02f80438u, 0x03700410u,
+  0x039803e8u, 0x140103c0u, 0x03702400u, 0x2400ffffu, 0x02582400u, 0x02300488u, 0x02f80730u, 0x02d00438u, 0x03980708u, 0x037003e8u, 0x15010690u, 0x03982400u,
+  0x2400ffffu, 0x05a02400u, 0x05a005a0u, 0x05a005a0u, 0x05a005a0u, 0x05a005a0u, 0x05a005a0u, 0x240005a0u, 0xffff2400u, 0x2400ffffu, 0x05a02400u, 0x05a005a0u,
+  0x05a005a0u, 0x05a005a0u, 0x05a005a0u, 0x05a005a0u, 0x240005a0u, 0xffff2400u, 0x2400ffffu, 0x05a02400u, 0x05a005a0u, 0x05a005a0u, 0x05a005a0u, 0x05a005a0u,
+  0x05a005a0u, 0x240005a0u, 0xffff2400u, 0x2400ffffu, 0x05a02400u, 0x05a005a0u, 0x05a005a0u, 0x05a005a0u, 0x05a005a0u, 0x05a005a0u, 0x240005a0u, 0xffff2400u,
   0x00000000u, 0x00000000u, 0x00000000u, 0x00000000u, 0x00000000u, 0x00000000u, 0x00000000u, 0x00000000u, 0x00000000u, 0x00000000u, 0x00000000u, 0x00000000u,
   0x00000000u, 0x00000000u, 0x00000000u, 0x00000000u,
 };
@@ -2517,4 +2529,5 @@
 template <> struct XInst<XP_MADD_NEG_2_V, S_F, S_F> { static constexpr int kOff = 27792, kW = 10; HG_DEV static void run(const Team& T, XStream& S, XHint h) { x_round<1, 2, 4, 2, 10, 2, 0, 4, 1, 0, 1, 0, 0, 0, 0>(T, S, 27792, h); } };
 template <> struct XInst<XP_MADD_F1_2_V, S_F, S_F> { static constexpr int kOff = 27952, kW = 10; HG_DEV static void run(const Team& T, XStream& S, XHint h) { x_round<1, 2, 4, 2, 10, 2, 0, 4, 1, 0, 1, 0, 0, 0, 0>(T, S, 27952, h); } };
 template <> struct XInst<XP_MADD_F2_2_V, S_F, S_F> { static constexpr int kOff = 28112, kW = 10; HG_DEV static void run(const Team& T, XStream& S, XHint h) { x_round<1, 2, 4, 2, 10, 2, 0, 4, 1, 0, 1, 0, 0, 0, 0>(T, S, 28112, h); } };
+template <> struct XInst<XP_TORMULF, S_A, S_A, S_B> { static constexpr int kOff = 28272, kW = 9; HG_DEV static void run(const Team& T, XStream& S, XHint h) { x_round<1, 2, 6, 2, 9, 0, 0, 4, 1, 0, 1, 0, 0, 1, 0>(T, S, 28272, h); } };
 }
diff --git a/handel_amd/csrc/hg_aggregate.cpp b/handel_amd/csrc/hg_aggregate.cpp
--- a/handel_amd/csrc/hg_aggregate.cpp
+++ b/handel_amd/csrc/hg_aggregate.cpp
@@ -83,6 +83,27 @@
   if (level >= 1) b += (n + nwin8 * 256 + gt_block_count(c, nullptr)) * sizeof(Gt);
   if (level >= 2) b += nwin16 * 65536 * sizeof(Gt);
   return b;
+}
+
+static bool gt_torus_enabled() {
+  static const bool on = env_int("HG_GT_TORUS", 1, 0, 1) != 0;
+  return on;
+}
+static int convert_torus_locked(hg_ctx* c, hipStream_t s, size_t nwin) {
+  c->cur.torus = false;
+  if (!gt_torus_enabled()) return HG_OK;
+  const size_t nblk = gt_block_count(c, nullptr);
+  HG_CHECK(c, c->sub_count.ensure(1));
+  int degenerate = 0;
+  launch_tor_scan(c->cur.gt_win.p, nwin, c->cur.gt_blk.p, nblk, (int)c->nreg, c->sub_count.p, s);
+  HG_CHECK(c, hipMemcpyAsync(&degenerate, c->sub_count.p, sizeof degenerate, hipMemcpyDeviceToHost, s));
+  HG_CHECK(c, hipStreamSynchronize(s));
+  if (degenerate) return HG_OK;
+  launch_tor_convert(c->cur.gt_win.p, nwin, c->cur.gt_blk.p, nblk, (int)c->nreg, s);
+  int rc = check_launch(c);
+  if (rc) return rc;
+  c->cur.torus = true;
+  return HG_OK;
 }
 
 static int build_gt_locked(hg_ctx* c, hipStream_t s, int level) {
@@ -116,6 +137,8 @@
     launch_gt_windows16(c->cur.gt_w8.p, nwin8, c->cur.gt_win.p, nwin16, s);
     int rc = check_launch(c);
     if (rc) return rc;
+    rc = convert_torus_locked(c, s, (size_t)nwin16 * 65536);
+    if (rc) return rc;
     c->cur.gt_level = 2;
   }
   return HG_OK;
@@ -125,6 +148,7 @@
   if (cap < 0) cap = 0;
   if (cap < c->gt_cap) c->gt_cap = cap;
   if (oom && cap < c->oom_cap) c->oom_cap = cap;
+  if (c->gt_cap < 2 && c->cur.gt_level == 2 && c->cur.torus) c->cur.drop_tables();
   if (c->gt_cap < 2) c->cur.gt_win.reset();
   if (c->gt_cap < 1) c->cur.drop_tables();
   if (c->cur.gt_level > c->gt_cap) c->cur.gt_level = c->gt_cap;
@@ -265,6 +289,18 @@
                  gw.win_bits == 16 ? c->cur.gt_win.p : c->cur.gt_w8.p, c->cur.gt_blk.p, c->gt_bi, gw, ws.gt_y.p, zero_hdr,
                  s);
 }
+static int pair_and_compare(hg_ctx* c, const AggBatch& b, Ws& ws, SigForm form, hipStream_t s) {
+  const int n = (int)b.n;
+  PhaseTimer t(c, HG_PHASE_VERIFY, s);
+  const bool ran = launch_sig_form(form, b.sigs, c->flavor, n, c->d_lines.p, ws.sig_lines.p, ws.gt_fe.p, s);
+  t.stop();
+  if (!ran) {
+    c->err = "aggregate batch too large for its pairing form";
+    return HG_ERR_ARG;
+  }
+  launch_tor_compare(ws.gt_fe.p, ws.gt_y.p, n, b.codes, b.bits, s);
+  return HG_OK;
+}
 
 static int flow_gt_beside(hg_ctx* c, const AggBatch& b, Ws& ws, SigForm form, const GtWork& gw, hipStream_t s) {
   const int n = (int)b.n;
@@ -283,17 +319,19 @@
   fold.stop();
   HG_CHECK(c, hipEventRecord(ws.ev_join, ws.side));
   HG_CHECK(c, hipStreamWaitEvent(s, ws.ev_join, 0));
-  if (b.bits) launch_gt_compare_bits(ws.gt_fe.p, ws.gt_y.p, n, b.codes, b.bits, s);
+  if (gw.torus) launch_tor_compare(ws.gt_fe.p, ws.gt_y.p, n, b.codes, b.bits, s);
+  else if (b.bits) launch_gt_compare_bits(ws.gt_fe.p, ws.gt_y.p, n, b.codes, b.bits, s);
   else launch_gt_compare(ws.gt_fe.p, ws.gt_y.p, n, b.codes, s);
   return HG_OK;
 }
 
-static int flow_gt_sequence(hg_ctx* c, const AggBatch& b, Ws& ws, const GtWork& gw, hipStream_t s) {
+static int flow_gt_sequence(hg_ctx* c, const AggBatch& b, Ws& ws, SigForm form, const GtWork& gw, hipStream_t s) {
   const int n = (int)b.n;
   gt_prologue(c, b, ws, gw, s);
   PhaseTimer fold(c, HG_PHASE_AGGREGATE, s);
   gt_fold(c, b, ws, gw, b.codes, false, s);
   fold.stop();
+  if (gw.torus) return pair_and_compare(c, b, ws, form, s);
   PhaseTimer t(c, HG_PHASE_VERIFY, s);
   launch_verify_sig(ws.pts1.p, n, c->d_lines.p, ws.gt_y.p, b.codes, s);
   t.stop();
@@ -301,7 +339,7 @@
   return HG_OK;
 }
 
-static int flow_g2_or_mixed(hg_ctx* c, const AggBatch& b, Ws& ws, bool verify, bool use_gt, bool g2_fold,
+static int flow_g2_or_mixed(hg_ctx* c, const AggBatch& b, Ws& ws, bool verify, bool use_gt, bool g2_fold, SigForm form,
                             const GtWork& gw, hipStream_t s) {
   const int n = (int)b.n;
   int32_t* d_lvl = b.lvl;
@@ -322,7 +360,9 @@
   if (verify) {
     launch_decode_g1(b.sigs, n, c->flavor, ws.pts1.p, ws.codes_b.p, s);
     k_agg_codes<<<nb(b.n), 256, 0, s>>>(ws.codes_b.p, d_lvl, c->cur.hash_eof ? 1 : 0, n, b.codes);
-    if (use_gt) {
+    if (use_gt && gw.torus) {
+      return pair_and_compare(c, b, ws, form, s);
+    } else if (use_gt) {
       PhaseTimer t(c, HG_PHASE_VERIFY, s);
       launch_verify_sig(ws.pts1.p, n, c->d_lines.p, ws.gt_y.p, b.codes, s);
       t.stop();
@@ -352,19 +392,21 @@
     int rc = gt_acquire(c, ws, s, n, b.caps ? *b.caps : fold_caps_worst(c, n), level, gw, !is_lane);
     if (rc) return rc;
   }
+  if (level > 0 && c->cur.gt_level == 2 && c->cur.torus) level = 2;
   gw.win_bits = level == 2 ? 16 : 8;
+  gw.torus = level == 2 && c->cur.torus;
   const bool use_gt = level > 0;
   const bool g2_fold = !use_gt || b.agg;
   const bool beside = use_gt && !g2_fold && pol.overlap;
   const SigForm form = sig_form(sig_env(), pol, n);
   const unsigned parts = (g2_fold ? kWsG2Fold : 0) | (b.agg ? kWsAggOut : 0) | (b.lvl ? 0 : kWsLevel) |
-                         (verify ? kWsVerify : 0) | (beside ? kWsPairing | kWsSide : 0);
+                         (verify ? kWsVerify : 0) | (beside ? kWsPairing | kWsSide : 0) | (gw.torus ? kWsPairing : 0);
   HG_CHECK(c, ws_ensure(ws, n, parts, {}, sig_form_ws_bytes(form, (int)n)));
   PhaseTimer all(c, HG_PHASE_SUBMIT, s);
   int rc;
   if (beside) rc = flow_gt_beside(c, b, ws, form, gw, s);
-  else if (use_gt && !g2_fold) rc = flow_gt_sequence(c, b, ws, gw, s);
-  else rc = flow_g2_or_mixed(c, b, ws, verify, use_gt, g2_fold, gw, s);
+  else if (use_gt && !g2_fold) rc = flow_gt_sequence(c, b, ws, form, gw, s);
+  else rc = flow_g2_or_mixed(c, b, ws, verify, use_gt, g2_fold, form, gw, s);
   if (rc) return rc;
   all.stop();
   rc = check_launch(c);
@@ -499,6 +541,12 @@
   if (!c) return 0;
   std::lock_guard<std::mutex> g(c->mu);
   return c->cur.gt_level;
+}
+
+int hg_aggregate_tables_torus(hg_ctx* c) {
+  if (!c) return 0;
+  std::lock_guard<std::mutex> g(c->mu);
+  return c->cur.gt_level == 2 && c->cur.torus ? 1 : 0;
 }
 
 int hg_verify_aggregate_device(hg_ctx* c, const hg_request* d_reqs, size_t n, const uint64_t* d_words,
diff --git a/handel_amd/csrc/hg_ctx.h b/handel_amd/csrc/hg_ctx.h
--- a/handel_amd/csrc/hg_ctx.h
+++ b/handel_amd/csrc/hg_ctx.h
@@ -47,6 +47,7 @@
   DevBuf<PointG1> d_h;
   DevBuf<Gt> gt_key, gt_w8, gt_win, gt_blk;
   int gt_level = 0;
+  bool torus = false;
   size_t gt_requests = 0;
   size_t table_bytes() const { return gt_key.bytes() + gt_w8.bytes() + gt_win.bytes() + gt_blk.bytes(); }
   bool drop_tables() {
@@ -56,6 +57,7 @@
     gt_win.reset();
     gt_blk.reset();
     gt_level = 0;
+    torus = false;
     return true;
   }
 };
diff --git a/handel_amd/engine.py b/handel_amd/engine.py
--- a/handel_amd/engine.py
+++ b/handel_amd/engine.py
@@ -110,6 +110,9 @@
 
     def aggregate_tables(self) -> int:
         return int(self.L.hg_aggregate_tables(self.ctx))
+
+    def aggregate_tables_torus(self) -> bool:
+        return bool(self.L.hg_aggregate_tables_torus(self.ctx))
 
     def registry_load(self, pks: bytes) -> np.ndarray:
         a = _u8(pks)
diff --git a/include/handel_gpu.h b/include/handel_gpu.h
--- a/include/handel_gpu.h
+++ b/include/handel_gpu.h
@@ -88,6 +88,7 @@
 int hg_prepare_aggregate(hg_ctx* ctx);
 int hg_prepare_aggregate_msg(hg_ctx* ctx, const uint8_t* msg, size_t len);
 int hg_aggregate_tables(hg_ctx* ctx);
+int hg_aggregate_tables_torus(hg_ctx* ctx);
 int hg_set_aggregate_level(hg_ctx* ctx, int level);
 int hg_set_fold_overlap(hg_ctx* ctx, int on);
 int hg_set_verify_split(hg_ctx* ctx, int on);
```
